# SamSweere/xmm-superres-denoise

Hardware: NVIDIA B200
Metric: RRDB SR-2x inference images/sec (F=32, nb=4, 416x416 -> 832x832, batch 64 per GPU) (higher is better)
Workload: dtype bf16

## Files before the change

### include/xmm_b200.h

```cpp
#ifndef XMM_B200_H_
#define XMM_B200_H_

#include <stddef.h>
#include <stdint.h>

#ifdef __cplusplus
extern "C" {
#endif

#define XMM_OK 0
#define XMM_ERR_INVALID_ARGUMENT 1
#define XMM_ERR_UNSUPPORTED_DEVICE 2
#define XMM_ERR_CUDA 3
#define XMM_ERR_UNSUPPORTED_SHAPE 4

const char* xmm_last_error(void);
int xmm_version(void);
int xmm_check_device(void);
int xmm_set_sm_reserve(int sms);

typedef struct {
  const float* src;
  int src_cin;
  int o_off, i_off;
  int transpose;
  int k_off, k_count;
  float scale;
  int n_off, n_count;
  int part;
} xmm_pack_segment;

typedef struct {
  void* dst;
  const float* bias;
  int nt;
  int kc;
  int nchunks;
  int nseg;
  int perm;
  int n_valid;
  int bias_n;
  xmm_pack_segment seg[5];
  int tap_order;
} xmm_pack_job;

size_t xmm_pack_blob_bytes(int nt, int kc, int nchunks);
int xmm_pack_weights(const xmm_pack_job* jobs_dev, int njobs, void* stream);

typedef struct {
  const void* in;
  int in_ctot, in_coff, cin;
  const void* wblob;
  int kc;
  int cout;
  int batch, height, width;
  float lrelu_slope;
  const void* mask; int mask_ctot, mask_coff; float mask_slope;
  float s0;
  const void* r1; int r1_ctot, r1_coff; float s1;
  const void* r2; int r2_ctot, r2_coff; float s2;
  void* out; int out_ctot, out_coff;
  int pixel_shuffle;
  int tap_mode;
  float* colsum;
  float colsum_scale;
  int shuffle_stride;
  const void* wblob_row;
} xmm_conv3x3_params;

int xmm_conv3x3_bf16(const xmm_conv3x3_params* p, void* stream);

#define XMM_CHAIN_SKIP_DEAD_STORES 0x100
size_t xmm_conv3x3_chain_workspace_bytes(int nlayers, int batch, int height);
int xmm_conv3x3_chain_bf16(const xmm_conv3x3_params* layers, int nlayers, int mode_flags, void* workspace,
                           size_t workspace_bytes, void* stream);
int xmm_last_chain_launches(void);

#define XMM_STRETCH_LINEAR 0
#define XMM_STRETCH_SQRT 1
#define XMM_STRETCH_ASINH 2
#define XMM_STRETCH_LOG 3

typedef struct {
  const void* in;
  int in_is_int32;
  const uint8_t* mask;
  size_t mask_n;
  float* out;
  size_t n;
  float pre_scale;
  float max_val;
  int stretch_mode;
  float* scratch;
} xmm_normalize_params;
int xmm_normalize(const xmm_normalize_params* p, void* stream);

int xmm_denormalize(const float* in, float* out, size_t n, size_t per_image, const float* max_vals_dev,
                    int max_n, int stretch_mode, void* stream);

int xmm_restretch(const float* in, float* out, size_t n, int from_mode, int to_mode, void* stream);

typedef struct {
  const void* src[3];
  int nsrc;
  int src_is_int32;
  const unsigned char* mask;
  int batch, h, w;
  int up;
  int res_h, res_w;
  float pre_scale;
  const float* pre_scale_dev;
  float max_val;
  int stretch_mode;
  float* out;
} xmm_prepare_counts_params;
int xmm_prepare_counts(const xmm_prepare_counts_params* p, void* stream);

int xmm_image_upsample(const float* in, float* out, int n_img, int h, int w, int scale, void* stream);

typedef struct {
  const float* in;
  const float* weight;
  const float* bias;
  int batch, cin, height, width, filters;
  void* out; int out_ctot, out_coff;
  void* out2; int out2_ctot, out2_coff;
  const float* gate;
  const void* mask; int mask_ctot, mask_coff; float mask_slope;
} xmm_conv_first_params;
int xmm_conv_first(const xmm_conv_first_params* p, void* stream);

typedef struct {
  const void* in; int in_ctot, in_coff;
  const float* weight;
  const float* bias;
  const float* residual;
  float* out;
  float* pre;
  int batch, cout, height, width, filters;
  int clamp;
  const void* wblob;
} xmm_conv_last_params;
int xmm_conv_last(const xmm_conv_last_params* p, void* stream);

typedef struct {
  int tap_begin, tap_count;
  int x_c0, x_boxes;
  int y_c0, n;
  int mode;
} xmm_wgrad_role;

typedef struct {
  float* dw;
  int o_count, i_total;
  int i_begin, i_end;
  int role;
  int lane0;
  int col0;
  float scale;
  int accumulate;
  int perm;
  int o_begin, o_total;
} xmm_wgrad_dst;

typedef struct {
  const void* x; int x_ctot;
  const void* dy; int dy_ctot;
  int batch, height, width;
  int nroles; xmm_wgrad_role roles[4];
  int ndst; xmm_wgrad_dst dst[16];
  float* workspace;
} xmm_wgrad_params;

size_t xmm_wgrad_workspace_bytes(void);
int xmm_conv3x3_wgrad(const xmm_wgrad_params* p, void* stream);

int xmm_colsum_bf16(const void* in, int ctot, int c0, int n, size_t npix, float* out, float scale,
                    int accumulate, void* stream);

typedef struct {
  int c0, n;
  float* out;
  float scale;
  int accumulate;
} xmm_colsum_segment;
int xmm_colsum_multi_bf16(const void* in, int ctot, size_t npix, const xmm_colsum_segment* segs, int nseg,
                          void* stream);

typedef struct {
  const float* s; const float* gate;
  const void* v; int v_ctot, v_coff;
  const void* v2; int v2_ctot, v2_coff;
  float* r;
  float* ssum;
  int batch, ns, height, width, channels;
} xmm_edge_wgrad_params;
int xmm_edge_wgrad(const xmm_edge_wgrad_params* p, void* stream);

typedef struct {
  float minp, maxp, mint, maxt;
  float nmaxp, nminp;
  float dr, c1, c2;
  float use_p;
  float d_dr;
  float pad;
} xmm_scale_stats;

size_t xmm_loss_workspace_floats(void);
int xmm_loss_reduce(const float* preds, const float* target, size_t n, float* sums_dev,
                    xmm_scale_stats* stats_dev, float* workspace, void* stream);
int xmm_loss_grad(const float* preds, const float* target, size_t n, const float* coef_dev,
                  const float* gl_dev, float* grad, int accumulate, void* stream);
int xmm_avgpool2_pair(const float* preds, const float* target, float* preds_out, float* target_out,
                      int nimg, int h, int w, void* stream);
int xmm_ssim_prepare(const float* preds, size_t n, xmm_scale_stats* stats_dev, float k1, float k2,
                     void* stream);

typedef struct {
  const float* preds; const float* target;
  int nimg, h, w;
  const xmm_scale_stats* stats_dev;
  float window[19];
  int use_sim;
  float* acc;
  const float* kimg;
  float* ga; float* gb; float* gc;
} xmm_ssim_stats_params;
int xmm_ssim_tiles(int h, int w);
int xmm_ssim_stats(const xmm_ssim_stats_params* p, void* stream);

typedef struct {
  const float* preds; const float* target;
  int nimg, h, w;
  const xmm_scale_stats* stats_dev;
  float window[19];
  const float* ga; const float* gb; const float* gc;
  const float* coarse;
  float* grad;
  int accumulate;
} xmm_ssim_grad_params;
int xmm_ssim_grad(const xmm_ssim_grad_params* p, void* stream);

typedef struct {
  const float* acc[5];
  int tiles[5];
  int nvalid[5];
  int nscales;
  int batch, channels;
  float betas[5];
  float k1, k2;
  xmm_scale_stats* stats_dev;
  float* value;
  float* img_val;
  float* kimg;
  const float* gl_dev;
  float weight;
} xmm_msssim_finalize_params;
int xmm_msssim_finalize(const xmm_msssim_finalize_params* p, void* stream);

int xmm_adam_step(float* params, const float* grads, float* exp_avg, float* exp_avg_sq, size_t n, float lr,
                  float beta1, float beta2, float eps, int step, float grad_scale, void* stream);

#ifdef __cplusplus
}
#endif
#endif
```

### xmm_superres_denoise_b200/csrc/conv3x3_rdb.cuh

```cuda
#pragma once
#include <cstdio>

#include "conv3x3_tc.cuh"

namespace xmm {

constexpr int kRdbP = 63;
constexpr int kRdbBoxPx = kRdbP + 2;
constexpr int kRdbTileData = 2 * kRdbBoxPx * 64;
constexpr int kRdbTileBytes = 17 * 512;
constexpr int kRdbThreads = 512;
constexpr int kRdbSlots = 5;
constexpr int kRdbSlotCols = kRdbSlots * 32;
constexpr int kRdbMaxRing = 8;
constexpr int kRdbMaxStages = 8;
constexpr int kRdbTapBytes = 32 * 64;

struct RdbLayerArgs {
  const void* wblob;
  uint32_t w_bytes;
  uint32_t smem_off;
  float lrelu_slope;
  int store;
  __nv_bfloat16* out;
  int out_ctot, out_coff;
};

struct RdbArgs {
  RdbLayerArgs layer[3];
  int cin_off;
  int batch, height, width, band_h, tiles_x;
  long long total_rows;
  int stages, ring0, ring1;
  uint32_t w_total;
  float s0, s1, s2;
  const __nv_bfloat16* r1;
  int r1_ctot, r1_coff;
  const __nv_bfloat16* r2;
  int r2_ctot, r2_coff;
  int backoff_ns;
  int prefetch_rows;
  int split_producers;
  long long* prof;
};

template <int NL>
__host__ __device__ inline int rdb_tile_origin(int t) {
  return t == 0 ? 0 : (kRdbP - (NL - 1)) + (t - 1) * (kRdbP - 2 * (NL - 1));
}
template <int NL>
__host__ __device__ inline int rdb_tiles_x(int width) {
  int n = 1;
  while ((n == 1 ? 0 : rdb_tile_origin<NL>(n - 1) - (NL - 1)) + kRdbP < width) ++n;
  return n;
}

struct RdbPiece {
  int b, x0;
  int own_lo, own_hi;
  int ra, rb;
};

template <int NL>
struct RdbSched {
  int band_h, tiles_x, width, c0, npieces;
  long long t0, t1;
  __device__ __forceinline__ void init(const RdbArgs& a) {
    band_h = a.band_h;
    tiles_x = a.tiles_x;
    width = a.width;
    t0 = a.total_rows * blockIdx.x / gridDim.x;
    t1 = a.total_rows * (blockIdx.x + 1) / gridDim.x;
    c0 = int(t0 / band_h);
    npieces = t1 > t0 ? int((t1 - 1) / band_h) - c0 + 1 : 0;
  }
  __device__ __forceinline__ RdbPiece get(int i) const {
    RdbPiece p;
    const int col = c0 + i;
    const long long base = (long long)col * band_h;
    p.ra = t0 > base ? int(t0 - base) : 0;
    p.rb = t1 < base + band_h ? int(t1 - base) : band_h;
    p.b = col / tiles_x;
    const int t = col - p.b * tiles_x;
    p.own_lo = rdb_tile_origin<NL>(t);
    p.x0 = t == 0 ? 0 : p.own_lo - (NL - 1);
    p.own_hi = t == tiles_x - 1 ? width : rdb_tile_origin<NL>(t + 1);
    return p;
  }
};

template <int NL, class F>
__device__ __forceinline__ void rdb_walk(const RdbSched<NL>& s, F&& f) {
  int piece[NL], r[NL], hi[NL], n[NL], seq[NL][NL];
  RdbPiece pc[NL];
  bool done[NL];
#pragma unroll
  for (int l = 0; l < NL; ++l) {
    piece[l] = 0;
    n[l] = 0;
    done[l] = s.npieces == 0;
#pragma unroll
    for (int m = 0; m < NL; ++m) seq[l][m] = 0;
    pc[l] = s.get(0);
    r[l] = pc[l].ra - (NL - 1 - l) - 1;
    hi[l] = pc[l].rb + (NL - 1 - l) + 2;
  }
  while (!done[NL - 1]) {
    uint32_t go = done[0] ? 0u : 1u;
    bool steady = !done[0];
    int reps = pc[0].rb + (NL - 1) - r[0] + 1;
#pragma unroll
    for (int l = 1; l < NL; ++l) {
      const bool ready = !done[l] && (done[l - 1] || piece[l - 1] > piece[l] || (piece[l - 1] == piece[l] && r[l - 1] > r[l] + 1));
      go |= ready ? (1u << l) : 0u;
      steady = steady && ready && piece[l] == piece[0];
      const int kl = pc[l].rb + (NL - 1 - l) - r[l] + 1;
      reps = kl < reps ? kl : reps;
    }
    if (!steady || reps < 1) reps = 1;
    for (int i = 0; i < reps; ++i) {
#pragma unroll
      for (int l = 0; l < NL; ++l) {
        if ((go >> l) & 1u) {
          const int e = NL - 1 - l;
          f(l, pc[l], r[l], r[l] > pc[l].rb + e, n[l], seq[l]);
          ++n[l];
          if (++r[l] > hi[l]) {
#pragma unroll
            for (int m = 0; m < NL; ++m) seq[l][m] += (pc[l].rb - pc[l].ra) + 2 * (NL - 1 - m);
            if (++piece[l] >= s.npieces) {
              done[l] = true;
            } else {
              pc[l] = s.get(piece[l]);
              r[l] = pc[l].ra - e - 1;
              hi[l] = pc[l].rb + e + 2;
            }
          }
        }
      }
    }
  }
}

__device__ __noinline__ void rdb_wait_timeout(int tag, int a, int b2, int c) {
  printf("conv3x3_rdb: CTA %d thread %d stuck in wait %d (layer/map %d, index %d, parity %d)\n", int(blockIdx.x),
         int(threadIdx.x), tag, a, b2, c);
  __trap();
}
__device__ __forceinline__ void rdb_wait(uint64_t* bar, uint32_t parity, int tag, int a, int b2) {
  uint32_t spins = 0;
  while (!ptx::mbar_try_wait(bar, parity)) {
    if (++spins > (1u << 26)) rdb_wait_timeout(tag, a, b2, int(parity));
  }
}

__device__ __forceinline__ void rdb_wait_backoff(uint64_t* bar, uint32_t parity, int tag, int a, int b2, uint32_t ns) {
  uint32_t spins = 0;
  while (!ptx::mbar_try_wait(bar, parity)) {
    if (ns) __nanosleep(ns);
    if (++spins > (1u << 24)) rdb_wait_timeout(tag, a, b2, int(parity));
  }
}
#ifndef XMM_RDB_PROFILE
#define XMM_RDB_PROFILE 0
#endif
__device__ __forceinline__ void rdb_wait_p(uint64_t* bar, uint32_t parity, int tag, int a, int b2, bool prof, long long& acc) {
  if (XMM_RDB_PROFILE && prof) {
    const long long t0 = clock64();
    rdb_wait(bar, parity, tag, a, b2);
    acc += clock64() - t0;
  } else {
    rdb_wait(bar, parity, tag, a, b2);
  }
}

__device__ __forceinline__ int rdb_phi(int row) { return (row + 30) % 3; }

__device__ __forceinline__ void tmem_st_zero32(uint32_t taddr) {
  const uint32_t z = 0;
  asm volatile(
      "tcgen05.st.sync.aligned.32x32b.x32.b32 [%0], "
      "{%1, %1, %1, %1, %1, %1, %1, %1, %1, %1, %1, %1, %1, %1, %1, %1, "
      "%1, %1, %1, %1, %1, %1, %1, %1, %1, %1, %1, %1, %1, %1, %1, %1};" ::"r"(taddr),
      "r"(z)
      : "memory");
}
__device__ __forceinline__ void tmem_st_32x32(uint32_t taddr, const uint32_t (&r)[32]) {
  asm volatile(
      "tcgen05.st.sync.aligned.32x32b.x32.b32 [%0], "
      "{%1, %2, %3, %4, %5, %6, %7, %8, %9, %10, %11, %12, %13, %14, %15, %16, "
      "%17, %18, %19, %20, %21, %22, %23, %24, %25, %26, %27, %28, %29, %30, %31, %32};" ::"r"(taddr),
      "r"(r[0]), "r"(r[1]), "r"(r[2]), "r"(r[3]), "r"(r[4]), "r"(r[5]), "r"(r[6]), "r"(r[7]), "r"(r[8]), "r"(r[9]), "r"(r[10]),
      "r"(r[11]), "r"(r[12]), "r"(r[13]), "r"(r[14]), "r"(r[15]), "r"(r[16]), "r"(r[17]), "r"(r[18]), "r"(r[19]), "r"(r[20]),
      "r"(r[21]), "r"(r[22]), "r"(r[23]), "r"(r[24]), "r"(r[25]), "r"(r[26]), "r"(r[27]), "r"(r[28]), "r"(r[29]), "r"(r[30]),
      "r"(r[31])
      : "memory");
}
__device__ __forceinline__ void st_global_256(void* p, const uint4& a, const uint4& b) {
  asm volatile("st.global.v8.b32 [%0], {%1, %2, %3, %4, %5, %6, %7, %8};" ::"l"(p), "r"(a.x), "r"(a.y), "r"(a.z), "r"(a.w),
               "r"(b.x), "r"(b.y), "r"(b.z), "r"(b.w)
               : "memory");
}
__device__ __forceinline__ void ld_global_nc_256(const void* p, uint4& a, uint4& b) {
  asm volatile("ld.global.nc.v8.b32 {%0, %1, %2, %3, %4, %5, %6, %7}, [%8];"
               : "=r"(a.x), "=r"(a.y), "=r"(a.z), "=r"(a.w), "=r"(b.x), "=r"(b.y), "=r"(b.z), "=r"(b.w)
               : "l"(p));
}
__device__ __forceinline__ void tmem_st_wait() { asm volatile("tcgen05.wait::st.sync.aligned;" ::: "memory"); }

struct RdbCtx {
  uint8_t* w_s;
  uint8_t* stage_s;
  uint8_t* map_s[2];
  uint64_t* lfull;
  uint64_t* empty;
  uint64_t* tfull;
  uint64_t* tdrain;
  uint64_t* mfull;
  uint64_t* mempty;
  uint64_t* w_bar;
  volatile int* lstage;
  uint32_t tmem_base;
};

template <int G, int NL, int L>
__device__ __forceinline__ void rdb_issuer(const RdbArgs& args, const RdbCtx& c, const RdbSched<NL>& sched) {
  constexpr int NM = NL - 1;
  constexpr int e = NL - 1 - L;
  constexpr int ring[2] = {NL == 3 ? 5 : 2, 3};
  rdb_wait(c.w_bar, 0, 7, L, 0);
  ptx::tc_fence_after();
  const uint64_t bdesc0 = ptx::umma_smem_desc(ptx::smem_u32(c.w_s), 16, 512, ptx::UMMA_SW64);
  const uint64_t adesc0 = ptx::umma_smem_desc(ptx::smem_u32(c.stage_s), 16, 512, ptx::UMMA_SW64);
  const uint32_t a_hi = uint32_t(adesc0 >> 32), b_hi = uint32_t(bdesc0 >> 32);
  const uint32_t a_lo0 = uint32_t(adesc0);
  const uint32_t b_l = uint32_t(bdesc0) + (args.layer[L].smem_off >> 4);
  const uint32_t a_map0[2] = {a_lo0 + uint32_t((c.map_s[0] - c.stage_s) >> 4), a_lo0 + uint32_t((c.map_s[1] - c.stage_s) >> 4)};
  constexpr uint32_t kTile16 = uint32_t(kRdbTileBytes) >> 4;
  constexpr uint32_t kTap16 = uint32_t(kRdbTapBytes) >> 4;
  constexpr uint32_t kIdesc = ptx::umma_idesc_bf16_f32(128, 96, 0, 0);
  auto issue6 = [&](uint32_t d, uint32_t a, uint32_t b) {
#pragma unroll
    for (int dx = 0; dx < 3; ++dx)
#pragma unroll
      for (int ks = 0; ks < 2; ++ks)
        ptx::umma_ss_lh<true>(d, a + uint32_t((dx * 64 + ks * 32) >> 4), a_hi, b + uint32_t(dx * 3) * kTap16 + uint32_t((ks * 32) >> 4),
                              b_hi, kIdesc);
  };
  const bool prof = XMM_RDB_PROFILE && args.prof != nullptr && L == 0;
  long long pw[3] = {0, 0, 0};
  const long long t_begin = XMM_RDB_PROFILE ? clock64() : 0;
  uint32_t fills = 0;
  uint32_t n = 0;
  int seq[2] = {0, 0};
  for (int pi = 0; pi < sched.npieces; ++pi) {
    const RdbPiece pc = sched.get(pi);
    const int r_last = pc.rb + e;
    for (int r = pc.ra - e - 1; r <= r_last + 2; ++r, ++n) {
      if (n > 0) rdb_wait_p(&c.tdrain[L], (n - 1u) & 1u, 2, L, int(n), prof, pw[0]);
      ptx::tc_fence_after();
      if (r <= r_last) {
        const uint32_t d = c.tmem_base + uint32_t(L * kRdbSlotCols + rdb_phi(r - 1) * 32);
        auto global_chunks = [&]() {
#pragma unroll
          for (int g = 0; g < G; ++g) {
            const int k = int(fills & 7u);
            rdb_wait_p(&c.lfull[L * 8 + k], (fills >> 3) & 1u, 3, L, k, prof, pw[1]);
            const int stage = c.lstage[L * 8 + k];
            ++fills;
            ptx::tc_fence_after();
            issue6(d, a_lo0 + uint32_t(stage) * kTile16, b_l + uint32_t(g * 9) * kTap16);
            ptx::umma_commit(&c.empty[stage]);
          }
        };
        auto map_chunks = [&]() {
#pragma unroll
          for (int m = 0; m < NM; ++m)
            if (m < L) {
              const int sq = seq[m] + (r - (pc.ra - (NL - 1 - m)));
              const int slot = sq % ring[m];
              rdb_wait_p(&c.mfull[m * 8 + slot], uint32_t(sq / ring[m]) & 1u, 4, L * 10 + m, sq, prof, pw[2]);
              ptx::tc_fence_after();
              issue6(d, a_map0[m] + uint32_t(slot) * kTile16, b_l + uint32_t((G + m) * 9) * kTap16);
              if (L == NL - 1 || r < pc.ra - e || r > pc.rb + e - 1) ptx::umma_commit(&c.mempty[m * 8 + slot]);
            }
        };
        if (NL == 2) {
          map_chunks();
          global_chunks();
        } else {
          global_chunks();
          map_chunks();
        }
      }
      ptx::umma_commit(&c.tfull[L]);
    }
#pragma unroll
    for (int m = 0; m < NM; ++m) seq[m] += (pc.rb - pc.ra) + 2 * (NL - 1 - m);
  }
  if (XMM_RDB_PROFILE && prof) {
    long long* o = args.prof + size_t(blockIdx.x) * 16;
    o[0] = clock64() - t_begin;
    o[1] = pw[0];
    o[2] = pw[1];
    o[3] = pw[2];
  }
}

template <int G, int NL, int L>
__device__ __forceinline__ void rdb_epilogue(const RdbArgs& args, const RdbCtx& c, const RdbSched<NL>& sched, int q, int lane) {
  constexpr int e = NL - 1 - L;
  constexpr int ring[2] = {NL == 3 ? 5 : 2, 3};
  constexpr bool last = L == NL - 1;
  const int pos = q * 32 + lane + 1;
  const int band = pos >= kRdbBoxPx ? 1 : 0;
  const int pl = band ? pos - (kRdbBoxPx + 1) : pos - 1;
  const bool lane_ok = band ? pl >= 0 : pl < kRdbP;
  const uint32_t lane_base = c.tmem_base + (uint32_t(q * 32) << 16) + uint32_t(L * kRdbSlotCols);
  const uint32_t pos_off = uint32_t(pos) * 64u;
  const uint32_t pos_xor = uint32_t(pos >> 1) & 3u;
  const uint32_t bias_a = ptx::smem_u32(c.w_s + args.layer[L].smem_off + args.layer[L].w_bytes);
  const float slope = args.layer[L].lrelu_slope;
  const bool has_r1 = last && args.r1 != nullptr, has_r2 = last && args.r2 != nullptr;
  const bool prof = XMM_RDB_PROFILE && args.prof != nullptr;
  long long pw[2] = {0, 0};
  long long ph[4] = {0, 0, 0, 0};
  long long tph = 0;
  const long long t_begin = XMM_RDB_PROFILE ? clock64() : 0;
  uint32_t n = 0;
  int seq = 0;
  for (int pi = 0; pi < sched.npieces; ++pi) {
    const RdbPiece pc = sched.get(pi);
    const int px = pc.x0 + pl;
    const bool px_ok = lane_ok && px < args.width;
    const bool px_own = px_ok && px >= pc.own_lo && px < pc.own_hi;
    for (int r = pc.ra - e - 1; r <= pc.rb + e + 2; ++r, ++n) {
      const int j = r - 1;
      const bool real = j >= pc.ra - e && j < pc.rb + e;
      const int y = band * args.band_h + j;
      const bool inimg = px_ok && y >= 0 && y < args.height;
      const bool owned = real && px_own && inimg && j >= pc.ra && j < pc.rb;
      const size_t pix = size_t((pc.b * args.height + (y < 0 ? 0 : y)) * args.width + (px_ok ? px : 0));
      uint4 res1[4], res2[4];
      if (has_r1 && owned) {
        const __nv_bfloat16* p = args.r1 + pix * args.r1_ctot + args.r1_coff;
        ld_global_nc_256(p, res1[0], res1[1]);
        ld_global_nc_256(p + 16, res1[2], res1[3]);
      }
      if (has_r2 && owned) {
        const __nv_bfloat16* p = args.r2 + pix * args.r2_ctot + args.r2_coff;
        ld_global_nc_256(p, res2[0], res2[1]);
        ld_global_nc_256(p + 16, res2[2], res2[3]);
      }
      if (XMM_RDB_PROFILE)
        rdb_wait_p(&c.tfull[L], n & 1u, 5, L, int(n), prof, pw[0]);
      else
        rdb_wait_backoff(&c.tfull[L], n & 1u, 5, L, int(n), uint32_t(args.backoff_ns));
      if (XMM_RDB_PROFILE) tph = clock64();
      ptx::tc_fence_after();
      const int phi = rdb_phi(j);
      const uint32_t t_main = lane_base + uint32_t(phi * 32);
      const uint32_t t_carry = lane_base + uint32_t((3 + phi) * 32);
      float v[32];
      {
        uint32_t accr[32];
        ptx::tmem_ld_32x32(t_main, accr);
        if (phi < 2) {
          uint32_t car[32];
          ptx::tmem_ld_32x32(t_carry, car);
          ptx::tmem_ld_wait();
#pragma unroll
          for (int k = 0; k < 32; ++k) v[k] = __uint_as_float(car[k]) + __uint_as_float(accr[k]);
          tmem_st_zero32(t_carry);
        } else {
          ptx::tmem_ld_wait();
#pragma unroll
          for (int k = 0; k < 32; ++k) v[k] = __uint_as_float(accr[k]);
        }
      }
      {
        uint32_t b32[32];
#pragma unroll
        for (int k = 0; k < 8; ++k)
          asm volatile("ld.shared.v4.u32 {%0, %1, %2, %3}, [%4];"
                       : "=r"(b32[4 * k]), "=r"(b32[4 * k + 1]), "=r"(b32[4 * k + 2]), "=r"(b32[4 * k + 3])
                       : "r"(bias_a + 16u * k));
        tmem_st_32x32(t_main, b32);
      }
      tmem_st_wait();
      ptx::tc_fence_before();
      __syncwarp();
      if (lane == 0) ptx::mbar_arrive(&c.tdrain[L]);
      if (XMM_RDB_PROFILE) {
        const long long t = clock64();
        ph[0] += t - tph;
        tph = t;
      }
      if (!real) continue;

      if (slope != 1.f) {
#pragma unroll
        for (int k = 0; k < 32; ++k) v[k] = fmaxf(v[k], v[k] * slope);
      }
      if (last) {
        const float s0 = args.s0;
        if (s0 != 1.f) {
#pragma unroll
          for (int k = 0; k < 32; ++k) v[k] *= s0;
        }
        if (has_r1 && owned) {
          const float s1 = args.s1;
#pragma unroll
          for (int k = 0; k < 4; ++k) {
            float m8[8];
            unpack8(res1[k], m8);
#pragma unroll
            for (int i = 0; i < 8; ++i) v[8 * k + i] = fmaf(s1, m8[i], v[8 * k + i]);
          }
        }
        if (has_r2 && owned) {
          const float s2 = args.s2;
#pragma unroll
          for (int k = 0; k < 4; ++k) {
            float m8[8];
            unpack8(res2[k], m8);
#pragma unroll
            for (int i = 0; i < 8; ++i) v[8 * k + i] = fmaf(s2, m8[i], v[8 * k + i]);
          }
        }
      }
      uint4 o[4];
#pragma unroll
      for (int k = 0; k < 4; ++k) o[k] = pack8(v + 8 * k);
      if (XMM_RDB_PROFILE) {
        const long long t = clock64();
        ph[1] += t - tph;
        tph = t;
      }
      if (args.layer[L].store && owned) {
        __nv_bfloat16* gp = args.layer[L].out + pix * args.layer[L].out_ctot + args.layer[L].out_coff;
        st_global_256(gp, o[0], o[1]);
        st_global_256(gp + 16, o[2], o[3]);
      }
      if (!last) {
        const int sq = seq + (j - (pc.ra - e));
        const int slot = sq % ring[L];
        rdb_wait_p(&c.mempty[L * 8 + slot], (uint32_t(sq / ring[L]) & 1u) ^ 1u, 6, L, sq, prof, pw[1]);
        if (XMM_RDB_PROFILE) tph = clock64();
        uint8_t* dst = c.map_s[L] + size_t(slot) * kRdbTileBytes + pos_off;
        const uint4 zero = make_uint4(0, 0, 0, 0);
#pragma unroll
        for (int k = 0; k < 4; ++k) *reinterpret_cast<uint4*>(dst + ((uint32_t(k) ^ pos_xor) << 4)) = inimg ? o[k] : zero;
        ptx::fence_proxy_async();
        __syncwarp();
        if (lane == 0) ptx::mbar_arrive(&c.mfull[L * 8 + slot]);
        if (XMM_RDB_PROFILE) {
          const long long t = clock64();
          ph[2] += t - tph;
          tph = t;
        }
      }
      if (XMM_RDB_PROFILE) {
        const long long t = clock64();
        ph[3] += t - tph;
        tph = t;
      }
    }
    seq += (pc.rb - pc.ra) + 2 * e;
  }
  if (XMM_RDB_PROFILE && prof && q == 0 && lane == 0 && L < 2) {
    long long* o = args.prof + size_t(blockIdx.x) * 16 + 4 + 4 * L;
    o[0] = clock64() - t_begin;
    o[1] = pw[0];
    o[2] = pw[1];
    o[3] = (long long)n;
    if (L == 0) {
      long long* o2 = args.prof + size_t(blockIdx.x) * 16 + 12;
      o2[0] = ph[0];
      o2[1] = ph[1];
      o2[2] = ph[2];
      o2[3] = ph[3];
    }
  }
}

template <int G, int NL, int L>
__device__ __forceinline__ void rdb_layer_producer(const CUtensorMap* tmap_in, const RdbArgs& args, const RdbCtx& c,
                                                   const RdbSched<NL>& sched, int s0, int ns) {
  constexpr int e = NL - 1 - L;
  int idx = 0;
  uint32_t phase = 0;
  uint32_t fills = 0;
  for (int pi = 0; pi < sched.npieces; ++pi) {
    const RdbPiece pc = sched.get(pi);
    for (int r = pc.ra - e - 1; r <= pc.rb + e; ++r) {
      int row = r, band0 = 0;
      if (r < 0) {
        row = r + args.band_h;
        band0 = -1;
      } else if (r >= args.band_h) {
        row = r - args.band_h;
        band0 = 1;
      }
#pragma unroll
      for (int g = 0; g < G; ++g) {
        const int stage = s0 + idx;
        rdb_wait_backoff(&c.empty[stage], phase ^ 1u, 1, L, stage, uint32_t(args.backoff_ns));
        const int k = int(fills++ & 7u);
        c.lstage[L * 8 + k] = stage;
        uint64_t* fb = &c.lfull[L * 8 + k];
        ptx::mbar_expect_tx(fb, kRdbTileData);
        ptx::tma_load_5d(c.stage_s + size_t(stage) * kRdbTileBytes, tmap_in, fb, args.cin_off + 32 * g, pc.x0 - 1, row, band0, pc.b);
        if (++idx == ns) {
          idx = 0;
          phase ^= 1u;
        }
      }
      if (L == 0 && args.prefetch_rows > 0) {
        const int rp = r + args.prefetch_rows;
        if (rp <= pc.rb + e) {
          int prow = rp, pband = 0;
          if (rp < 0) {
            prow = rp + args.band_h;
            pband = -1;
          } else if (rp >= args.band_h) {
            prow = rp - args.band_h;
            pband = 1;
          }
#pragma unroll
          for (int g = 0; g < G; ++g)
            asm volatile("cp.async.bulk.prefetch.tensor.5d.L2.global.tile [%0, {%1, %2, %3, %4, %5}];" ::"l"(
                             reinterpret_cast<uint64_t>(tmap_in)),
                         "r"(args.cin_off + 32 * g), "r"(pc.x0 - 1), "r"(prow), "r"(pband), "r"(pc.b)
                         : "memory");
        }
      }
    }
  }
}

template <int G, int NL>
__global__ void __launch_bounds__(kRdbThreads, 1)
conv3x3_rdb_kernel(const __grid_constant__ CUtensorMap tmap_in, const RdbArgs args) {
  static_assert(NL == 2 || NL == 3, "two or three fused layers");
  static_assert(NL * kRdbSlotCols <= 512, "accumulators exceed TMEM");
  constexpr int NM = NL - 1;
  extern __shared__ uint8_t smem_raw[];
  uint8_t* smem = reinterpret_cast<uint8_t*>((reinterpret_cast<uintptr_t>(smem_raw) + 1023) & ~uintptr_t(1023));
  RdbCtx c;
  c.w_s = smem;
  c.stage_s = smem + args.w_total;
  c.map_s[0] = c.stage_s + size_t(args.stages) * kRdbTileBytes;
  c.map_s[1] = c.map_s[0] + size_t(args.ring0) * kRdbTileBytes;
  uint8_t* after = c.map_s[1] + size_t(NM > 1 ? args.ring1 : 0) * kRdbTileBytes;
  uint64_t* bars = reinterpret_cast<uint64_t*>(after);
  c.lfull = bars;
  c.empty = c.lfull + 24;
  c.tfull = c.empty + 8;
  c.tdrain = c.tfull + 3;
  c.mfull = c.tdrain + 3;
  c.mempty = c.mfull + 16;
  c.w_bar = c.mempty + 16;
  c.lstage = reinterpret_cast<volatile int*>(c.w_bar + 1);
  uint32_t* tmem_ptr_s = reinterpret_cast<uint32_t*>(const_cast<int*>(c.lstage) + 24);

  const int warp = threadIdx.x >> 5;
  const int lane = threadIdx.x & 31;

  if (warp == 0 && lane == 0) {
    ptx::prefetch_tmap(&tmap_in);
    for (int s = 0; s < NL * 8; ++s) ptx::mbar_init(&c.lfull[s], 1);
    for (int s = 0; s < args.stages; ++s) ptx::mbar_init(&c.empty[s], 1);
    for (int l = 0; l < NL; ++l) {
      ptx::mbar_init(&c.tfull[l], 1);
      ptx::mbar_init(&c.tdrain[l], 4);
    }
    for (int s = 0; s < 16; ++s) {
      ptx::mbar_init(&c.mfull[s], 4);
      ptx::mbar_init(&c.mempty[s], 1);
    }
    ptx::mbar_init(c.w_bar, 1);
    ptx::fence_mbar_init();
  }
  if (warp == 1) ptx::tmem_alloc<512>(tmem_ptr_s);
  ptx::tc_fence_before();
  __syncthreads();
  ptx::tc_fence_after();
  c.tmem_base = *tmem_ptr_s;

  if (warp == 0 && ptx::elect_one()) {
    uint32_t wtot = 0;
    for (int l = 0; l < NL; ++l) wtot += args.layer[l].w_bytes + 128u;
    ptx::mbar_expect_tx(c.w_bar, wtot);
    for (int l = 0; l < NL; ++l) {
      const uint8_t* gsrc = static_cast<const uint8_t*>(args.layer[l].wblob);
      const uint32_t n_l = args.layer[l].w_bytes + 128u;
      for (uint32_t off = 0; off < n_l; off += 32768u)
        ptx::bulk_load(c.w_s + args.layer[l].smem_off + off, gsrc + off, n_l - off < 32768u ? n_l - off : 32768u, c.w_bar);
    }
  }
  const int egroup = (warp - 4) >> 2;
  if (warp >= 4) {
    uint4* z = reinterpret_cast<uint4*>(c.map_s[0]);
    const int nz = (args.ring0 + (NM > 1 ? args.ring1 : 0)) * (kRdbTileBytes / 16);
    for (int i = int(threadIdx.x) - 128; i < nz; i += kRdbThreads - 128) z[i] = make_uint4(0, 0, 0, 0);
    ptx::fence_proxy_async();
    if (egroup < NL) {
      rdb_wait(c.w_bar, 0, 9, 0, 0);
      const uint32_t lane_base = c.tmem_base + (uint32_t((warp & 3) * 32) << 16) + uint32_t(egroup * kRdbSlotCols);
      const float* bias_s = reinterpret_cast<const float*>(c.w_s + args.layer[egroup].smem_off + args.layer[egroup].w_bytes);
      uint32_t b32[32];
#pragma unroll
      for (int k = 0; k < 32; ++k) b32[k] = __float_as_uint(bias_s[k]);
      for (int sl = 0; sl < 3; ++sl) tmem_st_32x32(lane_base + uint32_t(sl * 32), b32);
      for (int sl = 3; sl < kRdbSlots; ++sl) tmem_st_zero32(lane_base + uint32_t(sl * 32));
      tmem_st_wait();
    }
  }
  ptx::tc_fence_before();
  __syncthreads();
  ptx::tc_fence_after();

  RdbSched<NL> sched;
  sched.init(args);

  if (NL == 2 && args.split_producers && (warp == 0 || warp == 3)) {
    if (ptx::elect_one()) {
      const int ns0 = (args.stages + 1) / 2;
      if (warp == 0) rdb_layer_producer<G, NL, 0>(&tmap_in, args, c, sched, 0, ns0);
      if (warp == 3) rdb_layer_producer<G, NL, 1>(&tmap_in, args, c, sched, ns0, args.stages - ns0);
    }
  } else if (warp == 0) {
    if (ptx::elect_one()) {
      int stage = 0;
      uint32_t phase = 0;
      uint32_t fills[NL];
#pragma unroll
      for (int l = 0; l < NL; ++l) fills[l] = 0;
      rdb_walk<NL>(sched, [&](int l, const RdbPiece& pc, int r, bool flush, int, const int*) {
        if (flush) return;
        int row = r, band0 = 0;
        if (r < 0) {
          row = r + args.band_h;
          band0 = -1;
        } else if (r >= args.band_h) {
          row = r - args.band_h;
          band0 = 1;
        }
#pragma unroll
        for (int g = 0; g < G; ++g) {
          rdb_wait_backoff(&c.empty[stage], phase ^ 1u, 1, l, stage, uint32_t(args.backoff_ns));
          const int k = int(fills[l]++ & 7u);
          c.lstage[l * 8 + k] = stage;
          uint64_t* fb = &c.lfull[l * 8 + k];
          ptx::mbar_expect_tx(fb, kRdbTileData);
          ptx::tma_load_5d(c.stage_s + size_t(stage) * kRdbTileBytes, &tmap_in, fb, args.cin_off + 32 * g, pc.x0 - 1, row, band0,
                           pc.b);
          if (++stage == args.stages) {
            stage = 0;
            phase ^= 1u;
          }
        }
        if (l == 0 && args.prefetch_rows > 0) {
          const int rp = r + args.prefetch_rows;
          if (rp <= pc.rb + (NL - 1)) {
            int prow = rp, pband = 0;
            if (rp < 0) {
              prow = rp + args.band_h;
              pband = -1;
            } else if (rp >= args.band_h) {
              prow = rp - args.band_h;
              pband = 1;
            }
#pragma unroll
            for (int g = 0; g < G; ++g)
              asm volatile("cp.async.bulk.prefetch.tensor.5d.L2.global.tile [%0, {%1, %2, %3, %4, %5}];" ::"l"(
                               reinterpret_cast<uint64_t>(&tmap_in)),
                           "r"(args.cin_off + 32 * g), "r"(pc.x0 - 1), "r"(prow), "r"(pband), "r"(pc.b)
                           : "memory");
          }
        }
      });
    }
  } else if (warp <= 3) {
    if (warp - 1 < NL && ptx::elect_one()) {
      if (warp == 1) rdb_issuer<G, NL, 0>(args, c, sched);
      if (warp == 2) rdb_issuer<G, NL, 1>(args, c, sched);
      if constexpr (NL == 3) {
        if (warp == 3) rdb_issuer<G, NL, 2>(args, c, sched);
      }
    }
  } else if (egroup < NL) {
    const int q = warp & 3;
    if (egroup == 0) rdb_epilogue<G, NL, 0>(args, c, sched, q, lane);
    if (egroup == 1) rdb_epilogue<G, NL, 1>(args, c, sched, q, lane);
    if constexpr (NL == 3) {
      if (egroup == 2) rdb_epilogue<G, NL, 2>(args, c, sched, q, lane);
    }
  }

  ptx::tc_fence_before();
  __syncthreads();
  if (warp == 1) {
    ptx::tc_fence_after();
    ptx::tmem_dealloc<512>(c.tmem_base);
  }
}

}
```

### xmm_superres_denoise_b200/csrc/ptx_sm100.cuh

```cuda
#pragma once
#include <cstdint>
#include <cuda.h>
#include <cuda_runtime.h>

namespace xmm {
namespace ptx {

__device__ __forceinline__ uint32_t smem_u32(const void* p) {
  return static_cast<uint32_t>(__cvta_generic_to_shared(p));
}

__device__ __forceinline__ bool elect_one() {
  uint32_t pred;
  asm volatile(
      "{\n\t"
      ".reg .pred p;\n\t"
      "elect.sync _|p, 0xffffffff;\n\t"
      "selp.u32 %0, 1, 0, p;\n\t"
      "}\n"
      : "=r"(pred));
  return pred != 0;
}

__device__ __forceinline__ void mbar_init(uint64_t* bar, uint32_t count) {
  asm volatile("mbarrier.init.shared::cta.b64 [%0], %1;" ::"r"(smem_u32(bar)), "r"(count));
}
__device__ __forceinline__ void fence_mbar_init() {
  asm volatile("fence.mbarrier_init.release.cluster;" ::: "memory");
}
__device__ __forceinline__ void fence_proxy_async() {
  asm volatile("fence.proxy.async.shared::cta;" ::: "memory");
}
__device__ __forceinline__ void mbar_expect_tx(uint64_t* bar, uint32_t bytes) {
  asm volatile("mbarrier.arrive.expect_tx.shared::cta.b64 _, [%0], %1;" ::"r"(smem_u32(bar)),
               "r"(bytes)
               : "memory");
}
__device__ __forceinline__ void mbar_arrive(uint64_t* bar) {
  asm volatile("mbarrier.arrive.shared::cta.b64 _, [%0];" ::"r"(smem_u32(bar)) : "memory");
}
__device__ __forceinline__ bool mbar_try_wait(uint64_t* bar, uint32_t parity) {
  uint32_t ok;
  asm volatile(
      "{\n\t"
      ".reg .pred p;\n\t"
      "mbarrier.try_wait.parity.shared::cta.b64 p, [%1], %2;\n\t"
      "selp.u32 %0, 1, 0, p;\n\t"
      "}\n"
      : "=r"(ok)
      : "r"(smem_u32(bar)), "r"(parity)
      : "memory");
  return ok != 0;
}
__device__ __forceinline__ void mbar_wait(uint64_t* bar, uint32_t parity) {
  while (!mbar_try_wait(bar, parity)) {
  }
}

__device__ __forceinline__ void prefetch_tmap(const CUtensorMap* m) {
  asm volatile("prefetch.tensormap [%0];" ::"l"(reinterpret_cast<uint64_t>(m)) : "memory");
}
__device__ __forceinline__ void tma_load_4d(void* smem_dst, const CUtensorMap* m, uint64_t* bar,
                                            int c0, int c1, int c2, int c3) {
  asm volatile(
      "cp.async.bulk.tensor.4d.shared::cluster.global.tile.mbarrier::complete_tx::bytes "
      "[%0], [%1, {%3, %4, %5, %6}], [%2];"
      ::"r"(smem_u32(smem_dst)),
      "l"(reinterpret_cast<uint64_t>(m)), "r"(smem_u32(bar)), "r"(c0), "r"(c1), "r"(c2), "r"(c3)
      : "memory");
}
__device__ __forceinline__ void tma_store_4d(const CUtensorMap* m, const void* smem_src, int c0, int c1, int c2, int c3) {
  asm volatile(
      "cp.async.bulk.tensor.4d.global.shared::cta.bulk_group [%0, {%2, %3, %4, %5}], [%1];"
      ::"l"(reinterpret_cast<uint64_t>(m)), "r"(smem_u32(smem_src)), "r"(c0), "r"(c1), "r"(c2), "r"(c3)
      : "memory");
}
__device__ __forceinline__ void tma_load_5d(void* smem_dst, const CUtensorMap* m, uint64_t* bar, int c0, int c1, int c2,
                                            int c3, int c4) {
  asm volatile(
      "cp.async.bulk.tensor.5d.shared::cluster.global.tile.mbarrier::complete_tx::bytes "
      "[%0], [%1, {%3, %4, %5, %6, %7}], [%2];"
      ::"r"(smem_u32(smem_dst)),
      "l"(reinterpret_cast<uint64_t>(m)), "r"(smem_u32(bar)), "r"(c0), "r"(c1), "r"(c2), "r"(c3), "r"(c4)
      : "memory");
}
__device__ __forceinline__ void tma_store_5d(const CUtensorMap* m, const void* smem_src, int c0, int c1, int c2, int c3,
                                             int c4) {
  asm volatile(
      "cp.async.bulk.tensor.5d.global.shared::cta.bulk_group [%0, {%2, %3, %4, %5, %6}], [%1];"
      ::"l"(reinterpret_cast<uint64_t>(m)), "r"(smem_u32(smem_src)), "r"(c0), "r"(c1), "r"(c2), "r"(c3), "r"(c4)
      : "memory");
}
__device__ __forceinline__ void bulk_commit() { asm volatile("cp.async.bulk.commit_group;" ::: "memory"); }
template <int N>
__device__ __forceinline__ void bulk_wait_read() { asm volatile("cp.async.bulk.wait_group.read %0;" ::"n"(N) : "memory"); }
template <int N>
__device__ __forceinline__ void bulk_wait() { asm volatile("cp.async.bulk.wait_group %0;" ::"n"(N) : "memory"); }
__device__ __forceinline__ void named_bar_sync(int id, int nthreads) {
  asm volatile("bar.sync %0, %1;" ::"r"(id), "r"(nthreads) : "memory");
}
__device__ __forceinline__ void bulk_load(void* smem_dst, const void* gsrc, uint32_t bytes,
                                          uint64_t* bar) {
  asm volatile(
      "cp.async.bulk.shared::cluster.global.mbarrier::complete_tx::bytes [%0], [%1], %2, [%3];"
      ::"r"(smem_u32(smem_dst)),
      "l"(reinterpret_cast<uint64_t>(gsrc)), "r"(bytes), "r"(smem_u32(bar))
      : "memory");
}

template <int kCols>
__device__ __forceinline__ void tmem_alloc(uint32_t* smem_result) {
  asm volatile("tcgen05.alloc.cta_group::1.sync.aligned.shared::cta.b32 [%0], %1;" ::"r"(
                   smem_u32(smem_result)),
               "n"(kCols)
               : "memory");
  asm volatile("tcgen05.relinquish_alloc_permit.cta_group::1.sync.aligned;" ::: "memory");
}
template <int kCols>
__device__ __forceinline__ void tmem_dealloc(uint32_t taddr) {
  asm volatile("tcgen05.dealloc.cta_group::1.sync.aligned.b32 %0, %1;" ::"r"(taddr), "n"(kCols)
               : "memory");
}
__device__ __forceinline__ void tc_fence_before() {
  asm volatile("tcgen05.fence::before_thread_sync;" ::: "memory");
}
__device__ __forceinline__ void tc_fence_after() {
  asm volatile("tcgen05.fence::after_thread_sync;" ::: "memory");
}
__device__ __forceinline__ void umma_ss(uint32_t tmem_d, uint64_t adesc, uint64_t bdesc,
                                        uint32_t idesc, uint32_t accumulate) {
  asm volatile(
      "{\n\t"
      ".reg .pred p;\n\t"
      "setp.ne.b32 p, %4, 0;\n\t"
      "tcgen05.mma.cta_group::1.kind::f16 [%0], %1, %2, %3, p;\n\t"
      "}\n" ::"r"(tmem_d),
      "l"(adesc), "l"(bdesc), "r"(idesc), "r"(accumulate)
      : "memory");
}
template <bool ACC>
__device__ __forceinline__ void umma_ss_lh(uint32_t tmem_d, uint32_t a_lo, uint32_t a_hi, uint32_t b_lo, uint32_t b_hi,
                                           uint32_t idesc) {
  asm volatile(
      "{\n\t"
      ".reg .pred p;\n\t"
      ".reg .b64 da, db;\n\t"
      "setp.ne.b32 p, %6, 0;\n\t"
      "mov.b64 da, {%1, %2};\n\t"
      "mov.b64 db, {%3, %4};\n\t"
      "tcgen05.mma.cta_group::1.kind::f16 [%0], da, db, %5, p;\n\t"
      "}\n" ::"r"(tmem_d),
      "r"(a_lo), "r"(a_hi), "r"(b_lo), "r"(b_hi), "r"(idesc), "n"(ACC ? 1 : 0)
      : "memory");
}
__device__ __forceinline__ void umma_ts(uint32_t tmem_d, uint32_t tmem_a, uint64_t bdesc,
                                        uint32_t idesc, uint32_t accumulate) {
  asm volatile(
      "{\n\t"
      ".reg .pred p;\n\t"
      "setp.ne.b32 p, %4, 0;\n\t"
      "tcgen05.mma.cta_group::1.kind::f16 [%0], [%1], %2, %3, p;\n\t"
      "}\n" ::"r"(tmem_d),
      "r"(tmem_a), "l"(bdesc), "r"(idesc), "r"(accumulate)
      : "memory");
}
__device__ __forceinline__ void umma_commit(uint64_t* bar) {
  asm volatile("tcgen05.commit.cta_group::1.mbarrier::arrive::one.shared::cluster.b64 [%0];" ::"r"(
                   smem_u32(bar))
               : "memory");
}
__device__ __forceinline__ void tmem_ld_32x32(uint32_t taddr, uint32_t (&r)[32]) {
  asm volatile(
      "tcgen05.ld.sync.aligned.32x32b.x32.b32 "
      "{%0, %1, %2, %3, %4, %5, %6, %7, %8, %9, %10, %11, %12, %13, %14, %15, "
      "%16, %17, %18, %19, %20, %21, %22, %23, %24, %25, %26, %27, %28, %29, %30, %31}, [%32];"
      : "=r"(r[0]), "=r"(r[1]), "=r"(r[2]), "=r"(r[3]), "=r"(r[4]), "=r"(r[5]), "=r"(r[6]),
        "=r"(r[7]), "=r"(r[8]), "=r"(r[9]), "=r"(r[10]), "=r"(r[11]), "=r"(r[12]), "=r"(r[13]),
        "=r"(r[14]), "=r"(r[15]), "=r"(r[16]), "=r"(r[17]), "=r"(r[18]), "=r"(r[19]), "=r"(r[20]),
        "=r"(r[21]), "=r"(r[22]), "=r"(r[23]), "=r"(r[24]), "=r"(r[25]), "=r"(r[26]), "=r"(r[27]),
        "=r"(r[28]), "=r"(r[29]), "=r"(r[30]), "=r"(r[31])
      : "r"(taddr)
      : "memory");
}
__device__ __forceinline__ void tmem_ld_32x16(uint32_t taddr, uint32_t (&r)[16]) {
  asm volatile(
      "tcgen05.ld.sync.aligned.32x32b.x16.b32 "
      "{%0, %1, %2, %3, %4, %5, %6, %7, %8, %9, %10, %11, %12, %13, %14, %15}, [%16];"
      : "=r"(r[0]), "=r"(r[1]), "=r"(r[2]), "=r"(r[3]), "=r"(r[4]), "=r"(r[5]), "=r"(r[6]),
        "=r"(r[7]), "=r"(r[8]), "=r"(r[9]), "=r"(r[10]), "=r"(r[11]), "=r"(r[12]), "=r"(r[13]),
        "=r"(r[14]), "=r"(r[15])
      : "r"(taddr)
      : "memory");
}
__device__ __forceinline__ void tmem_ld_32x8(uint32_t taddr, uint32_t (&r)[8]) {
  asm volatile(
      "tcgen05.ld.sync.aligned.32x32b.x8.b32 {%0, %1, %2, %3, %4, %5, %6, %7}, [%8];"
      : "=r"(r[0]), "=r"(r[1]), "=r"(r[2]), "=r"(r[3]), "=r"(r[4]), "=r"(r[5]), "=r"(r[6]), "=r"(r[7])
      : "r"(taddr)
      : "memory");
}
template <int N>
__device__ __forceinline__ void tmem_ld_cols(uint32_t taddr, uint32_t (&r)[N]);
template <>
__device__ __forceinline__ void tmem_ld_cols<8>(uint32_t taddr, uint32_t (&r)[8]) { tmem_ld_32x8(taddr, r); }
template <>
__device__ __forceinline__ void tmem_ld_cols<16>(uint32_t taddr, uint32_t (&r)[16]) { tmem_ld_32x16(taddr, r); }
__device__ __forceinline__ void tmem_ld_wait() {
  asm volatile("tcgen05.wait::ld.sync.aligned;" ::: "memory");
}

__device__ __forceinline__ uint32_t cluster_ctarank() {
  uint32_t r;
  asm volatile("mov.u32 %0, %%cluster_ctarank;" : "=r"(r));
  return r;
}
__device__ __forceinline__ void cluster_sync() {
  asm volatile("barrier.cluster.arrive.release.aligned;\n\tbarrier.cluster.wait.acquire.aligned;" ::: "memory");
}
__device__ __forceinline__ uint32_t mapa(uint32_t saddr, uint32_t rank) {
  uint32_t r;
  asm volatile("mapa.shared::cluster.u32 %0, %1, %2;" : "=r"(r) : "r"(saddr), "r"(rank));
  return r;
}
__device__ __forceinline__ void mbar_arrive_cluster(uint32_t cluster_addr) {
  asm volatile("mbarrier.arrive.relaxed.cluster.shared::cluster.b64 _, [%0];" ::"r"(cluster_addr) : "memory");
}
__device__ __forceinline__ void tma_load_4d_pair(void* smem_dst, const CUtensorMap* m, uint32_t bar_cluster_addr,
                                                 int c0, int c1, int c2, int c3) {
  asm volatile(
      "cp.async.bulk.tensor.4d.cta_group::2.shared::cluster.global.tile.mbarrier::complete_tx::bytes "
      "[%0], [%1, {%3, %4, %5, %6}], [%2];"
      ::"r"(smem_u32(smem_dst)),
      "l"(reinterpret_cast<uint64_t>(m)), "r"(bar_cluster_addr), "r"(c0), "r"(c1), "r"(c2), "r"(c3)
      : "memory");
}
template <int kCols>
__device__ __forceinline__ void tmem_alloc_pair(uint32_t* smem_result) {
  asm volatile("tcgen05.alloc.cta_group::2.sync.aligned.shared::cta.b32 [%0], %1;" ::"r"(smem_u32(smem_result)),
               "n"(kCols)
               : "memory");
  asm volatile("tcgen05.relinquish_alloc_permit.cta_group::2.sync.aligned;" ::: "memory");
}
template <int kCols>
__device__ __forceinline__ void tmem_dealloc_pair(uint32_t taddr) {
  asm volatile("tcgen05.dealloc.cta_group::2.sync.aligned.b32 %0, %1;" ::"r"(taddr), "n"(kCols) : "memory");
}
__device__ __forceinline__ void umma_ss_pair(uint32_t tmem_d, uint64_t adesc, uint64_t bdesc, uint32_t idesc,
                                             uint32_t accumulate) {
  asm volatile(
      "{\n\t"
      ".reg .pred p;\n\t"
      "setp.ne.b32 p, %4, 0;\n\t"
      "tcgen05.mma.cta_group::2.kind::f16 [%0], %1, %2, %3, p;\n\t"
      "}\n" ::"r"(tmem_d),
      "l"(adesc), "l"(bdesc), "r"(idesc), "r"(accumulate)
      : "memory");
}
__device__ __forceinline__ void umma_commit_pair(uint64_t* bar) {
  asm volatile(
      "tcgen05.commit.cta_group::2.mbarrier::arrive::one.shared::cluster.multicast::cluster.b64 [%0], %1;" ::"r"(
          smem_u32(bar)),
      "h"(uint16_t(3))
      : "memory");
}

enum : uint32_t { UMMA_SW_NONE = 0, UMMA_SW128 = 2, UMMA_SW64 = 4, UMMA_SW32 = 6 };

__device__ __forceinline__ uint64_t umma_smem_desc(uint32_t saddr, uint32_t lbo_bytes,
                                                   uint32_t sbo_bytes, uint32_t layout_type,
                                                   uint32_t base_offset = 0) {
  uint64_t d = 0;
  d |= static_cast<uint64_t>((saddr & 0x3FFFFu) >> 4);
  d |= static_cast<uint64_t>((lbo_bytes >> 4) & 0x3FFFu) << 16;
  d |= static_cast<uint64_t>((sbo_bytes >> 4) & 0x3FFFu) << 32;
  d |= 1ull << 46;
  d |= static_cast<uint64_t>(base_offset & 7u) << 49;
  d |= static_cast<uint64_t>(layout_type & 7u) << 61;
  return d;
}

__host__ __device__ constexpr uint32_t umma_idesc_bf16_f32(int m, int n, int a_mn_major,
                                                           int b_mn_major) {
  return (1u << 4) | (1u << 7) | (1u << 10) | (static_cast<uint32_t>(a_mn_major) << 15) |
         (static_cast<uint32_t>(b_mn_major) << 16) | (static_cast<uint32_t>(n >> 3) << 17) |
         (static_cast<uint32_t>(m >> 4) << 24);
}

}
}
```

### xmm_superres_denoise_b200/csrc/xmm_b200.cu

```cuda
#include "../../include/xmm_b200.h"

#include <unordered_map>
#include <vector>

#include "conv3x3_chain.cuh"
#include "conv3x3_dx.cuh"
#include "conv3x3_row.cuh"
#include "conv3x3_rdb.cuh"
#include "conv3x3_tc.cuh"
#include "edge_kernels.cuh"
#include "host_common.cuh"
#include "loss_kernels.cuh"
#include "pack_weights.cuh"
#include "wgrad_tc.cuh"

#ifndef XMM_DEFAULT_TAP_MODE
#define XMM_DEFAULT_TAP_MODE 0
#endif

using namespace xmm;

extern "C" const char* xmm_last_error(void) { return last_error_ref().c_str(); }
extern "C" int xmm_version(void) { return 100; }
extern "C" int xmm_check_device(void) {
  DeviceInfo d;
  return require_sm100(&d);
}

extern "C" size_t xmm_pack_blob_bytes(int nt, int kc, int nchunks) {
  return size_t(nchunks) * 9 * nt * kc * 2 + size_t(nt) * 4;
}

extern "C" int xmm_pack_weights(const xmm_pack_job* jobs_dev, int njobs, void* stream) {
  DeviceInfo d;
  int rc = require_sm100(&d);
  if (rc != XMM_OK) return rc;
  XMM_REQUIRE(jobs_dev != nullptr && njobs > 0, "xmm_pack_weights: empty job table");
  dim3 grid(45, njobs);
  pack_jobs_kernel<<<grid, 256, 0, static_cast<cudaStream_t>(stream)>>>(jobs_dev);
  XMM_CUDA_OK(cudaGetLastError());
  return XMM_OK;
}

namespace {

struct TmapKey {
  const void* base;
  int batch, height, width, ctot, box_c, box_w, box_h;
  bool operator==(const TmapKey& o) const {
    return base == o.base && batch == o.batch && height == o.height && width == o.width && ctot == o.ctot &&
           box_c == o.box_c && box_w == o.box_w && box_h == o.box_h;
  }
};
struct TmapKeyHash {
  size_t operator()(const TmapKey& k) const {
    size_t h = reinterpret_cast<size_t>(k.base);
    auto mix = [&h](size_t v) { h ^= v + 0x9e3779b97f4a7c15ull + (h << 6) + (h >> 2); };
    mix(k.batch); mix(k.height); mix(k.width); mix(k.ctot); mix(k.box_c); mix(k.box_w); mix(k.box_h);
    return h;
  }
};


int ensure_max_smem(const void* kernel, const DeviceInfo& dev, int reserve = 0) {
  static std::mutex mu;
  static std::unordered_map<const void*, unsigned long long> done;
  {
    std::lock_guard<std::mutex> lk(mu);
    unsigned long long& bits = done[kernel];
    if (bits & (1ull << dev.device)) return XMM_OK;
    bits |= 1ull << dev.device;
  }
  XMM_CUDA_OK(cudaFuncSetAttribute(kernel, cudaFuncAttributeMaxDynamicSharedMemorySize, dev.max_smem_optin - reserve));
  return XMM_OK;
}

int cached_tmap(CUtensorMap* out, const void* base, int batch, int height, int width, int ctot, int box_c,
                int box_w, int box_h) {
  static std::mutex mu;
  static std::unordered_map<TmapKey, CUtensorMap, TmapKeyHash> cache;
  TmapKey key{base, batch, height, width, ctot, box_c, box_w, box_h};
  std::lock_guard<std::mutex> lk(mu);
  auto it = cache.find(key);
  if (it != cache.end()) {
    *out = it->second;
    return XMM_OK;
  }
  int rc = make_nhwc_tmap(out, base, batch, height, width, ctot, box_c, box_w, box_h, false);
  if (rc != XMM_OK) return rc;
  if (cache.size() > 4096) cache.clear();
  cache.emplace(key, *out);
  return XMM_OK;
}

void fill_epilogue(ConvEpilogue& e, const xmm_conv3x3_params& p) {
  e.lrelu_slope = p.lrelu_slope;
  e.mask_slope = p.mask_slope;
  e.s0 = p.s0; e.s1 = p.s1; e.s2 = p.s2;
  e.mask = static_cast<const __nv_bfloat16*>(p.mask); e.mask_ctot = p.mask_ctot; e.mask_coff = p.mask_coff;
  e.r1 = static_cast<const __nv_bfloat16*>(p.r1); e.r1_ctot = p.r1_ctot; e.r1_coff = p.r1_coff;
  e.r2 = static_cast<const __nv_bfloat16*>(p.r2); e.r2_ctot = p.r2_ctot; e.r2_coff = p.r2_coff;
  e.out = static_cast<__nv_bfloat16*>(p.out); e.out_ctot = p.out_ctot; e.out_coff = p.out_coff;
  e.pixel_shuffle = p.pixel_shuffle;
  e.shuffle_stride = p.shuffle_stride > 0 ? p.shuffle_stride : p.cout;
  e.img_out = nullptr; e.img_res = nullptr; e.img_pre = nullptr; e.img_cout = 0; e.img_clamp = 0;
  e.colsum = p.colsum; e.colsum_scale = p.colsum_scale;
}

struct ImageOut {
  float* out;
  const float* res;
  float* pre;
  int cout, clamp;
};

constexpr bool kTcTwoGroupsDefault = true;
template <int KC, int NT, int MODE, int EG>
int launch_conv_impl(const xmm_conv3x3_params& p, const DeviceInfo& dev, cudaStream_t stream, const ImageOut* img) {
  using Cfg = ConvCfg<KC, NT, MODE, EG>;
  ConvArgs a{};
  a.wblob = p.wblob;
  a.nchunks = p.cin / KC;
  a.w_bytes = uint32_t(a.nchunks) * 9u * Cfg::kTapBytes;
  a.cin_off = p.in_coff;
  a.batch = p.batch;
  a.height = p.height;
  a.width = p.width;
  a.tiles_x = (p.width + kTileW - 1) / kTileW;
  a.tiles_y = (p.height + kTileH - 1) / kTileH;
  a.num_tiles = a.tiles_x * a.tiles_y * p.batch;
  static const int tma_env = [] { const char* e = getenv("XMM_TC_TMA_STORE"); return e ? atoi(e) : 1; }();
  const size_t fixed_plain = Cfg::smem_bytes(a.w_bytes, 0, false), fixed_out = Cfg::smem_bytes(a.w_bytes, 0, true);
  if (fixed_plain + 2 * size_t(Cfg::kStageBytes) > size_t(dev.max_smem_optin))
    return fail(XMM_ERR_UNSUPPORTED_SHAPE,
                "conv3x3: weights of cin=%d cout=%d (%u B) do not fit in shared memory next to 2 pipeline stages",
                p.cin, p.cout, a.w_bytes);
  auto stages_for = [&](size_t fixed) {
    const int st = size_t(dev.max_smem_optin) > fixed ? int((size_t(dev.max_smem_optin) - fixed) / Cfg::kStageBytes) : 0;
    return st > kMaxStages ? kMaxStages : st;
  };
  const int st_plain = stages_for(fixed_plain), st_out = stages_for(fixed_out);
  a.tma_store = (Cfg::kOutBytes > 0 && p.pixel_shuffle == 0 && img == nullptr && st_out >= 2 &&
                 (tma_env == 2 || (tma_env == 1 && (st_out >= 6 || st_out == st_plain))))
                    ? 1 : 0;
  const int stages = a.tma_store ? st_out : st_plain;
  a.stages = stages;
  const size_t smem = Cfg::smem_bytes(a.w_bytes, stages, a.tma_store != 0);

  fill_epilogue(a.epi, p);
  if (img != nullptr) {
    a.epi.img_out = img->out; a.epi.img_res = img->res; a.epi.img_pre = img->pre;
    a.epi.img_cout = img->cout; a.epi.img_clamp = img->clamp;
  }

  CUtensorMap tmap;
  int rc = cached_tmap(&tmap, p.in, p.batch, p.height, p.width, p.in_ctot, KC, Cfg::kPitchPx, kHaloH);
  if (rc != XMM_OK) return rc;
  CUtensorMap tmap_out = tmap;
  if (a.tma_store) {
    rc = cached_tmap(&tmap_out, p.out, p.batch, p.height, p.width, p.out_ctot, NT, kTileW, 4);
    if (rc != XMM_OK) return rc;
  }

  rc = ensure_max_smem(reinterpret_cast<const void*>(conv3x3_tc_kernel<KC, NT, MODE, EG>), dev);
  if (rc != XMM_OK) return rc;
  const int grid = a.num_tiles < dev.sm_count ? a.num_tiles : dev.sm_count;
  conv3x3_tc_kernel<KC, NT, MODE, EG><<<grid, Cfg::kThreads, smem, stream>>>(tmap, tmap_out, a);
  XMM_CUDA_OK(cudaGetLastError());
  return XMM_OK;
}

template <int KC, int NT, int MODE>
int launch_conv(const xmm_conv3x3_params& p, const DeviceInfo& dev, cudaStream_t stream, const ImageOut* img = nullptr) {
  static const int eg_env = [] { const char* e = getenv("XMM_TC_EG"); return e ? atoi(e) : 0; }();
  if constexpr (4 * NT <= 512) {
    const long long ntiles = (long long)((p.width + kTileW - 1) / kTileW) * ((p.height + kTileH - 1) / kTileH) * p.batch;
    if (eg_env == 2 || (eg_env == 0 && kTcTwoGroupsDefault && ntiles >= 4LL * dev.sm_count))
      return launch_conv_impl<KC, NT, MODE, 2>(p, dev, stream, img);
  }
  return launch_conv_impl<KC, NT, MODE, 1>(p, dev, stream, img);
}

template <int KC, int NT, bool G2>
int launch_conv_dx_impl(const xmm_conv3x3_params& p, const DeviceInfo& dev, cudaStream_t stream) {
  using Cfg = DxCfg<KC, NT, G2>;
  ConvArgs a{};
  a.wblob = p.wblob;
  a.nchunks = p.cin / KC;
  a.w_bytes = uint32_t(a.nchunks) * 9u * Cfg::kTapBytes;
  a.cin_off = p.in_coff;
  a.batch = p.batch;
  a.height = p.height;
  a.width = p.width;
  a.tiles_x = (p.width + kDxTileW - 1) / kDxTileW;
  a.tiles_y = (p.height + kDxTileH - 1) / kDxTileH;
  a.num_tiles = a.tiles_x * a.tiles_y * p.batch;
  static const int sides_env = [] { const char* e = getenv("XMM_DX_SIDES"); return e ? atoi(e) : 1; }();
  const void* side_ptr[3] = {p.mask, p.r1, p.r2};
  const int side_ctot[3] = {p.mask_ctot, p.r1_ctot, p.r2_ctot};
  int nside = 0;
  if (p.pixel_shuffle == 0 && sides_env)
    for (int k = 0; k < 3; ++k)
      if (side_ptr[k] != nullptr) { a.side_mask |= 1 << k; ++nside; }
  size_t fixed = Cfg::smem_bytes(a.w_bytes, 0, nside);
  if (nside > 0 && fixed + 4 * size_t(Cfg::kStageBytes) > size_t(dev.max_smem_optin)) {
    a.side_mask = 0;
    nside = 0;
    fixed = Cfg::smem_bytes(a.w_bytes, 0, 0);
  }
  if (fixed + 2 * size_t(Cfg::kStageBytes) > size_t(dev.max_smem_optin))
    return fail(XMM_ERR_UNSUPPORTED_SHAPE,
                "conv3x3: weights of cin=%d cout=%d (%u B) do not fit in shared memory next to 2 pipeline stages",
                p.cin, p.cout, a.w_bytes);
  int stages = int((size_t(dev.max_smem_optin) - fixed) / Cfg::kStageBytes);
  if (stages > kMaxStages) stages = kMaxStages;
  a.stages = stages;
  const size_t smem = Cfg::smem_bytes(a.w_bytes, stages, nside);
  fill_epilogue(a.epi, p);
  CUtensorMap tmap;
  int rc = cached_tmap(&tmap, p.in, p.batch, p.height, p.width, p.in_ctot, KC, kDxTileW, kDxPatchH);
  if (rc != XMM_OK) return rc;
  CUtensorMap tmap_out = tmap;
  if (p.pixel_shuffle == 0) {
    rc = cached_tmap(&tmap_out, p.out, p.batch, p.height, p.width, p.out_ctot, Cfg::kWarpCols, kDxTileW, 2);
    if (rc != XMM_OK) return rc;
  }
  DxSideMaps sides;
  for (int k = 0; k < 3; ++k) {
    sides.m[k] = tmap;
    if (a.side_mask & (1 << k)) {
      rc = cached_tmap(&sides.m[k], side_ptr[k], p.batch, p.height, p.width, side_ctot[k], NT, kDxTileW, kDxTileH);
      if (rc != XMM_OK) return rc;
    }
  }
  rc = ensure_max_smem(reinterpret_cast<const void*>(conv3x3_dx_kernel<KC, NT, false, G2>), dev);
  if (rc != XMM_OK) return rc;
  const int grid = a.num_tiles < dev.sm_count ? a.num_tiles : dev.sm_count;
  static const int rr_env = [] { const char* e = getenv("XMM_DX_RR"); return e ? atoi(e) : -1; }();
  const long long nstrips = (long long)a.tiles_y * p.batch;
  a.strip_rr = rr_env >= 0 ? (rr_env != 0) : (nstrips >= 4LL * grid && (a.nchunks >= 3 || nstrips >= 16LL * grid));
  static const int pair_env = [] { const char* e = getenv("XMM_DX_PAIR"); return e ? atoi(e) : 0; }();
  if constexpr (!G2)
  if (KC == 32 && NT == 32 && (pair_env || p.tap_mode == 6) && p.tap_mode != 5 && a.strip_rr && grid % 2 == 0 &&
      nstrips >= grid) {
    rc = ensure_max_smem(reinterpret_cast<const void*>(conv3x3_dx_kernel<KC, NT, true>), dev);
    if (rc != XMM_OK) return rc;
    cudaLaunchConfig_t cfg{};
    cfg.gridDim = dim3(unsigned(grid));
    cfg.blockDim = dim3(kDxThreads);
    cfg.dynamicSmemBytes = smem;
    cfg.stream = stream;
    cudaLaunchAttribute attr[1];
    attr[0].id = cudaLaunchAttributeClusterDimension;
    attr[0].val.clusterDim.x = 2;
    attr[0].val.clusterDim.y = 1;
    attr[0].val.clusterDim.z = 1;
    cfg.attrs = attr;
    cfg.numAttrs = 1;
    XMM_CUDA_OK(cudaLaunchKernelEx(&cfg, conv3x3_dx_kernel<KC, NT, true>, tmap, tmap_out, sides, a));
    return XMM_OK;
  }
  conv3x3_dx_kernel<KC, NT, false, G2><<<grid, kDxThreads, smem, stream>>>(tmap, tmap_out, sides, a);
  XMM_CUDA_OK(cudaGetLastError());
  return XMM_OK;
}

template <int KC, int NT>
int launch_conv_dx(const xmm_conv3x3_params& p, const DeviceInfo& dev, cudaStream_t stream) {
  if constexpr (NT == 32) {
    static const int g2_env = [] { const char* e = getenv("XMM_DX_G2"); return e ? atoi(e) : 1; }();
    static const int rr_env = [] { const char* e = getenv("XMM_DX_RR"); return e ? atoi(e) : -1; }();
    const int tiles_x = (p.width + kDxTileW - 1) / kDxTileW, tiles_y = (p.height + kDxTileH - 1) / kDxTileH;
    const long long ntiles = (long long)tiles_x * tiles_y * p.batch, nstrips = (long long)tiles_y * p.batch;
    const long long grid = ntiles < dev.sm_count ? ntiles : dev.sm_count;
    const int nchunks = p.cin / KC;
    const bool rr = rr_env >= 0 ? (rr_env != 0) : (nstrips >= 4LL * grid && (nchunks >= 3 || nstrips >= 16LL * grid));
    const bool g2 = (p.tap_mode == 8) || (g2_env && rr && nstrips >= 16LL * grid && (p.tap_mode <= 0 || p.tap_mode == 4));
    if (g2 && DxCfg<KC, NT, true>::smem_bytes(uint32_t(nchunks) * 9u * DxCfg<KC, NT, true>::kTapBytes,
                                               p.tap_mode == 8 ? 2 : 6,
                                               (p.mask != nullptr) + (p.r1 != nullptr) + (p.r2 != nullptr)) <=
                  size_t(dev.max_smem_optin))
      return launch_conv_dx_impl<KC, NT, true>(p, dev, stream);
  }
  return launch_conv_dx_impl<KC, NT, false>(p, dev, stream);
}


struct BandTmapKey {
  const void* base;
  int batch, height, width, ctot, band_h, nbands, box_c, box_w, box_bands;
  bool operator==(const BandTmapKey& o) const {
    return base == o.base && batch == o.batch && height == o.height && width == o.width && ctot == o.ctot &&
           band_h == o.band_h && nbands == o.nbands && box_c == o.box_c && box_w == o.box_w && box_bands == o.box_bands;
  }
};
struct BandTmapKeyHash {
  size_t operator()(const BandTmapKey& k) const {
    size_t h = reinterpret_cast<size_t>(k.base);
    auto mix = [&h](size_t v) { h ^= v + 0x9e3779b97f4a7c15ull + (h << 6) + (h >> 2); };
    mix(k.batch); mix(k.height); mix(k.width); mix(k.ctot); mix(k.band_h); mix(k.nbands); mix(k.box_c); mix(k.box_w);
    mix(k.box_bands);
    return h;
  }
};
int cached_band_tmap(CUtensorMap* out, const void* base, int batch, int height, int width, int ctot, int band_h,
                     int nbands, int box_c, int box_w, int box_bands) {
  static std::mutex mu;
  static std::unordered_map<BandTmapKey, CUtensorMap, BandTmapKeyHash> cache;
  BandTmapKey key{base, batch, height, width, ctot, band_h, nbands, box_c, box_w, box_bands};
  std::lock_guard<std::mutex> lk(mu);
  auto it = cache.find(key);
  if (it != cache.end()) {
    *out = it->second;
    return XMM_OK;
  }
  int rc = make_band_tmap(out, base, batch, height, width, ctot, band_h, nbands, box_c, box_w, box_bands);
  if (rc != XMM_OK) return rc;
  if (cache.size() > 4096) cache.clear();
  cache.emplace(key, *out);
  return XMM_OK;
}

bool row_bands(int height, int* nbands, int* band_h) {
  for (int n = kRowBands; n >= kRowBands / 2; --n)
    if (height % n == 0) {
      *nbands = n;
      *band_h = height / n;
      return true;
    }
  return false;
}

int row_epi_flags(const xmm_conv3x3_params& p) {
  return (p.lrelu_slope != 1.0f ? kRowLrelu : 0) | (p.mask ? kRowMask : 0) | (p.r1 ? kRowR1 : 0) | (p.r2 ? kRowR2 : 0) |
         (p.colsum ? kRowCsum : 0);
}
bool row_epi_built(int f) {
  switch (f) {
    case 0: case kRowLrelu: case kRowR1: case kRowR1 | kRowR2: case kRowMask: case kRowMask | kRowCsum: case kRowCsum:
    case kRowR1 | kRowCsum: case kRowR1 | kRowR2 | kRowCsum:
      return true;
    default:
      return false;
  }
}

template <int KC, int NT>
const char* row_blocker(const xmm_conv3x3_params& p, const DeviceInfo& dev, int* stages_out) {
  using Cfg = RowCfg<KC, NT>;
  if (p.wblob_row == nullptr) return "no row-hop weight image (wblob_row)";
  if (p.pixel_shuffle != 0) return "pixel shuffle";
  int nbands, band_h;
  if (!row_bands(p.height, &nbands, &band_h)) return "height has no divisor in 8..16";
  const int flags = row_epi_flags(p);
  if (!row_epi_built(flags)) return "epilogue combination not instantiated";
  if ((flags & kRowCsum) && NT != 32) return "fused column sums need cout = 32";
  const int nside = (p.mask != nullptr) + (p.r1 != nullptr) + (p.r2 != nullptr);
  const uint32_t w_bytes = uint32_t(p.cin / KC) * 9u * Cfg::kTapBytes;
  const size_t fixed = Cfg::smem_bytes(w_bytes, 0, nside);
  if (fixed + 3 * size_t(Cfg::kStageBytes) > size_t(dev.max_smem_optin)) return "weights do not fit next to 3 pipeline stages";
  int stages = int((size_t(dev.max_smem_optin) - fixed) / Cfg::kStageBytes);
  if (stages > kMaxStages) stages = kMaxStages;
  *stages_out = stages;
  return nullptr;
}

template <int KC, int NT, int EPI>
int launch_conv_row_epi(const xmm_conv3x3_params& p, const DeviceInfo& dev, cudaStream_t stream, int stages) {
  using Cfg = RowCfg<KC, NT>;
  RowArgs a{};
  a.wblob = p.wblob_row;
  a.nchunks = p.cin / KC;
  a.w_bytes = uint32_t(a.nchunks) * 9u * Cfg::kTapBytes;
  a.cin_off = p.in_coff;
  a.batch = p.batch;
  a.height = p.height;
  a.width = p.width;
  row_bands(p.height, &a.nbands, &a.band_h);
  a.tiles_x = (p.width + kRowPx - 1) / kRowPx;
  a.ncols = a.tiles_x * p.batch;
  a.stages = stages;
  const void* side_ptr[3] = {p.mask, p.r1, p.r2};
  const int side_ctot[3] = {p.mask_ctot, p.r1_ctot, p.r2_ctot};
  int nside = 0;
  for (int k = 0; k < 3; ++k)
    if (side_ptr[k] != nullptr) { a.side_mask |= 1 << k; ++nside; }
  fill_epilogue(a.epi, p);
  const long long total_rows = (long long)a.ncols * a.band_h;
  const int grid = total_rows < dev.sm_count ? int(total_rows) : dev.sm_count;
  static const int rr_env = [] { const char* e = getenv("XMM_ROW_RR"); return e ? atoi(e) : 1; }();
  a.rr_rounds = (rr_env && a.ncols >= 2 * grid) ? a.ncols / grid : 0;
  CUtensorMap tmap, tmap_out;
  int rc = cached_band_tmap(&tmap, p.in, p.batch, p.height, p.width, p.in_ctot, a.band_h, a.nbands, KC, kRowPitch, kRowBands);
  if (rc != XMM_OK) return rc;
  rc = cached_band_tmap(&tmap_out, p.out, p.batch, p.height, p.width, p.out_ctot, a.band_h, a.nbands, NT, kRowPx, 4);
  if (rc != XMM_OK) return rc;
  RowSideMaps sides;
  for (int k = 0; k < 3; ++k) {
    sides.m[k] = tmap;
    if (a.side_mask & (1 << k)) {
      rc = cached_band_tmap(&sides.m[k], side_ptr[k], p.batch, p.height, p.width, side_ctot[k], a.band_h, a.nbands, NT,
                            kRowPx, kRowBands);
      if (rc != XMM_OK) return rc;
    }
  }
  rc = ensure_max_smem(reinterpret_cast<const void*>(conv3x3_row_kernel<KC, NT, EPI>), dev);
  if (rc != XMM_OK) return rc;
  const size_t smem = Cfg::smem_bytes(a.w_bytes, stages, nside);
  conv3x3_row_kernel<KC, NT, EPI><<<grid, kRowThreads, smem, stream>>>(tmap, tmap_out, sides, a);
  XMM_CUDA_OK(cudaGetLastError());
  return XMM_OK;
}

template <int KC, int NT>
int launch_conv_row(const xmm_conv3x3_params& p, const DeviceInfo& dev, cudaStream_t stream, int stages) {
  switch (row_epi_flags(p)) {
#define XMM_ROW_CASE(F_) case (F_): return launch_conv_row_epi<KC, NT, (F_)>(p, dev, stream, stages);
    XMM_ROW_CASE(0)
    XMM_ROW_CASE(kRowLrelu)
    XMM_ROW_CASE(kRowR1)
    XMM_ROW_CASE(kRowR1 | kRowR2)
    XMM_ROW_CASE(kRowMask)
    default: break;
  }
  if constexpr (NT == 32) {
    switch (row_epi_flags(p)) {
      XMM_ROW_CASE(kRowCsum)
      XMM_ROW_CASE(kRowMask | kRowCsum)
      XMM_ROW_CASE(kRowR1 | kRowCsum)
      XMM_ROW_CASE(kRowR1 | kRowR2 | kRowCsum)
#undef XMM_ROW_CASE
      default: break;
    }
  }
  return fail(XMM_ERR_INVALID_ARGUMENT, "conv3x3 (row-hop): epilogue combination %d is not instantiated", row_epi_flags(p));
}

template <int KC, int NT>
int launch_conv_mode(const xmm_conv3x3_params& p, const DeviceInfo& dev, cudaStream_t stream) {
  const int mode = p.tap_mode <= 0 ? XMM_DEFAULT_TAP_MODE : p.tap_mode - 1;
  switch (mode) {
    case kTapHalo: return launch_conv<KC, NT, kTapHalo>(p, dev, stream);
    case kTapHaloBaseOff: return launch_conv<KC, NT, kTapHaloBaseOff>(p, dev, stream);
    case kTapDx3: return launch_conv<KC, NT, kTapDx3>(p, dev, stream);
    default: return fail(XMM_ERR_INVALID_ARGUMENT, "conv3x3: unknown tap_mode %d", mode);
  }
}

}

namespace {
int check_conv_params(const xmm_conv3x3_params& p) {
  XMM_REQUIRE(p.in && p.out && p.wblob, "conv3x3: null tensor pointer");
  XMM_REQUIRE(p.batch > 0 && p.height > 0 && p.width > 0, "conv3x3: bad shape %dx%dx%d", p.batch, p.height, p.width);
  XMM_REQUIRE(p.kc == 32 || p.kc == 64, "conv3x3: kc must be 32 or 64 (got %d)", p.kc);
  XMM_REQUIRE(p.cin > 0 && p.cin % p.kc == 0, "conv3x3: cin=%d is not a multiple of kc=%d", p.cin, p.kc);
  XMM_REQUIRE(p.in_ctot % 8 == 0 && p.in_coff % 8 == 0 && p.in_coff + p.cin <= p.in_ctot,
              "conv3x3: input channel window [%d,%d) of %d", p.in_coff, p.in_coff + p.cin, p.in_ctot);
  XMM_REQUIRE(p.shuffle_stride == 0 || (p.pixel_shuffle == 2 && p.shuffle_stride >= p.cout && p.shuffle_stride % 8 == 0),
              "conv3x3: shuffle_stride is the inverse pixel shuffle's block distance (>= cout)");
  const int out_c = p.pixel_shuffle == 1 ? p.cout / 4
                    : (p.pixel_shuffle == 2 ? 3 * (p.shuffle_stride > 0 ? p.shuffle_stride : p.cout) + p.cout : p.cout);
  XMM_REQUIRE(p.pixel_shuffle >= 0 && p.pixel_shuffle <= 2, "conv3x3: pixel_shuffle must be 0, 1 or 2");
  XMM_REQUIRE(p.pixel_shuffle != 2 || (p.height % 2 == 0 && p.width % 2 == 0 && !p.r1 && !p.r2),
              "conv3x3: inverse pixel shuffle needs even height/width and no residual");
  XMM_REQUIRE(p.out_ctot % 8 == 0 && p.out_coff % 8 == 0 && p.out_coff + out_c <= p.out_ctot,
              "conv3x3: output channel window [%d,%d) of %d", p.out_coff, p.out_coff + out_c, p.out_ctot);
  XMM_REQUIRE(!p.mask || (p.mask_ctot % 8 == 0 && p.mask_coff % 8 == 0), "conv3x3: mask window alignment");
  XMM_REQUIRE(!p.r1 || (p.r1_ctot % 8 == 0 && p.r1_coff % 8 == 0), "conv3x3: r1 window alignment");
  XMM_REQUIRE(!p.r2 || (p.r2_ctot % 8 == 0 && p.r2_coff % 8 == 0), "conv3x3: r2 window alignment");
  XMM_REQUIRE(!p.colsum || (p.cout == 32 && p.pixel_shuffle == 0), "conv3x3: fused column sums need cout = 32");
  XMM_REQUIRE(p.pixel_shuffle != 1 || (!p.mask && !p.r1 && !p.r2 && p.cout % 128 == 0),
              "conv3x3: pixel_shuffle needs cout %% 128 == 0 and no mask/residual");
  XMM_REQUIRE((reinterpret_cast<uintptr_t>(p.in) & 15) == 0 && (reinterpret_cast<uintptr_t>(p.out) & 15) == 0 &&
                  (reinterpret_cast<uintptr_t>(p.wblob) & 15) == 0,
              "conv3x3: pointers must be 16-byte aligned");
  return XMM_OK;
}
}

extern "C" int xmm_conv3x3_bf16(const xmm_conv3x3_params* pp, void* stream) {
  XMM_REQUIRE(pp != nullptr, "conv3x3: null params");
  const xmm_conv3x3_params& p = *pp;
  DeviceInfo dev;
  int rc = require_sm100(&dev);
  if (rc != XMM_OK) return rc;
  rc = check_conv_params(p);
  if (rc != XMM_OK) return rc;
  cudaStream_t s = static_cast<cudaStream_t>(stream);
  static const int row_env = [] { const char* e = getenv("XMM_ROW"); return e ? atoi(e) : 1; }();
  const bool row_narrow = p.cin <= 2 * p.kc || row_env == 2;
  if ((p.tap_mode <= 0 && row_env && row_narrow && p.wblob_row != nullptr) || p.tap_mode == 9) {
    const char* why = "cout must equal kc (32 or 64)";
    int stages = 0;
    if (p.kc == 32 && p.cout == 32) {
      why = row_blocker<32, 32>(p, dev, &stages);
      if (why == nullptr) return launch_conv_row<32, 32>(p, dev, s, stages);
    } else if (p.kc == 64 && p.cout == 64) {
      why = row_blocker<64, 64>(p, dev, &stages);
      if (why == nullptr) return launch_conv_row<64, 64>(p, dev, s, stages);
    }
    if (p.tap_mode == 9) return fail(XMM_ERR_UNSUPPORTED_SHAPE, "conv3x3: the row-hop form does not qualify (%s)", why);
  }
  const bool dx_auto = p.tap_mode <= 0 && p.kc == 32 && p.cout == 32 && p.cin >= 64 &&
                       DxCfg<32, 32>::smem_bytes(uint32_t(p.cin / 32) * 9u * DxCfg<32, 32>::kTapBytes, 4) <=
                           size_t(dev.max_smem_optin);
  if ((p.tap_mode >= 4 && p.tap_mode <= 8) || dx_auto) {
    if (p.kc == 32 && p.cout == 32) return launch_conv_dx<32, 32>(p, dev, s);
    if (p.kc == 64 && p.cout == 64) return launch_conv_dx<64, 64>(p, dev, s);
    return fail(XMM_ERR_INVALID_ARGUMENT, "conv3x3: the column-scatter form is built for cout = kc = 32 or 64");
  }
#define XMM_CONV_CASE(KC_, NT_) \
  if (p.kc == KC_ && p.cout == NT_) return launch_conv_mode<KC_, NT_>(p, dev, s);
  XMM_CONV_CASE(32, 32)
  XMM_CONV_CASE(32, 128)
  XMM_CONV_CASE(64, 64)
  XMM_CONV_CASE(64, 256)
#undef XMM_CONV_CASE
  return fail(XMM_ERR_UNSUPPORTED_SHAPE, "conv3x3: no kernel for kc=%d cout=%d", p.kc, p.cout);
}

namespace {

struct Window {
  const void* base;
  int ctot, c0, c1;
};
bool overlaps(const Window& a, const Window& b) {
  return a.base && b.base && a.base == b.base && a.ctot == b.ctot && a.c0 < b.c1 && b.c0 < a.c1;
}
bool same(const Window& a, const Window& b) { return a.base == b.base && a.ctot == b.ctot && a.c0 == b.c0 && a.c1 == b.c1; }

const char* chain_blocker(const xmm_conv3x3_params* L, int n) {
  if (n < 2 || n > kChainMaxLayers) return "2..5 layers";
  for (int l = 0; l < n; ++l) {
    const xmm_conv3x3_params& p = L[l];
    if (p.kc != 32 || p.cout != 32) return "kc = cout = 32 layers only";
    if (p.pixel_shuffle != 0) return "no pixel shuffle inside a chain";
    if (p.batch != L[0].batch || p.height != L[0].height || p.width != L[0].width) return "one image geometry";
    if (uint32_t(p.cin / 32) * 9u * DxCfg<32, 32>::kTapBytes > 160u * 1024u) return "weights must stay resident";
  }
  for (int l = 0; l < n; ++l) {
    const Window in{L[l].in, L[l].in_ctot, L[l].in_coff, L[l].in_coff + L[l].cin};
    const Window out{L[l].out, L[l].out_ctot, L[l].out_coff, L[l].out_coff + L[l].cout};
    const Window side[3] = {{L[l].mask, L[l].mask_ctot, L[l].mask_coff, L[l].mask_coff + L[l].cout},
                            {L[l].r1, L[l].r1_ctot, L[l].r1_coff, L[l].r1_coff + L[l].cout},
                            {L[l].r2, L[l].r2_ctot, L[l].r2_coff, L[l].r2_coff + L[l].cout}};
    if (overlaps(in, out)) return "a layer may not write its own input window";
    for (int m = 0; m < n; ++m) {
      const Window om{L[m].out, L[m].out_ctot, L[m].out_coff, L[m].out_coff + L[m].cout};
      if (m > l && overlaps(in, om)) return "a later layer overwrites an earlier layer's input";
      if (m != l && overlaps(out, om)) return "two layers write the same window";
      for (const Window& sd : side) {
        if (!sd.base) continue;
        if (m == l ? (overlaps(sd, om) && !same(sd, om)) : overlaps(sd, om))
          return "an epilogue input (mask / residual) is produced inside the chain";
      }
    }
  }
  return nullptr;
}

int env_int(const char* name, int dflt) {
  const char* e = getenv(name);
  return e && *e ? atoi(e) : dflt;
}

int launch_chain(const xmm_conv3x3_params* L, int n, const DeviceInfo& dev, int* done, cudaStream_t stream) {
  using Cfg = DxCfg<32, 32>;
  ChainArgs a{};
  ChainTmaps tm{};
  a.nlayers = n;
  a.batch = L[0].batch;
  a.height = L[0].height;
  a.width = L[0].width;
  a.tiles_x = (a.width + kDxTileW - 1) / kDxTileW;
  a.tiles_y = (a.height + kDxTileH - 1) / kDxTileH;
  int segs = env_int("XMM_CHAIN_SEGS", 2);
  if (segs < 1) segs = 1;
  if (segs > a.tiles_x) segs = a.tiles_x;
  a.segs = segs;
  a.done = done;
  const int nstrips = a.batch * a.tiles_y;
  const int grid = dev.sm_count;

  double cost[kChainMaxLayers], total = 0;
  for (int l = 0; l < n; ++l) {
    const int nch = L[l].cin / 32;
    cost[l] = 60.0 + 340.0 * nch;
    if (cost[l] < 850.0) cost[l] = 850.0;
    total += cost[l];
  }
  int cnt[kChainMaxLayers], used = 0;
  for (int l = 0; l < n; ++l) {
    cnt[l] = int(grid * cost[l] / total);
    if (cnt[l] < 1) cnt[l] = 1;
    used += cnt[l];
  }
  for (int l = n - 1; used < grid; l = (l + n - 1) % n) { ++cnt[l]; ++used; }
  for (int l = 0; used > grid; l = (l + 1) % n) if (cnt[l] > 1) { --cnt[l]; --used; }
  if (const char* e = getenv("XMM_CHAIN_SPLIT")) {
    int v[kChainMaxLayers], k = 0, sum = 0;
    for (const char* q = e; *q && k < n; ++k) {
      v[k] = atoi(q);
      sum += v[k];
      while (*q && *q != ',') ++q;
      if (*q == ',') ++q;
    }
    if (k == n && sum <= grid) {
      bool ok = true;
      for (int l = 0; l < n; ++l) ok = ok && v[l] >= 1;
      if (ok) for (int l = 0; l < n; ++l) cnt[l] = v[l];
    }
  }
  size_t smem = 0;
  int begin = 0;
  for (int l = 0; l < n; ++l) {
    ChainLayer& c = a.layer[l];
    c.wblob = L[l].wblob;
    c.nchunks = L[l].cin / 32;
    c.w_bytes = uint32_t(c.nchunks) * 9u * Cfg::kTapBytes;
    c.cin_off = L[l].in_coff;
    c.cta_begin = begin;
    c.cta_count = cnt[l];
    begin += cnt[l];
    const size_t fixed = Cfg::smem_bytes(c.w_bytes, 0);
    int stages = int((size_t(dev.max_smem_optin) - fixed) / Cfg::kStageBytes);
    if (stages > kMaxStages) stages = kMaxStages;
    c.stages = stages;
    const size_t need = Cfg::smem_bytes(c.w_bytes, stages);
    if (need > smem) smem = need;
    fill_epilogue(c.epi, L[l]);
    int rc = cached_tmap(&tm.m[l], L[l].in, a.batch, a.height, a.width, L[l].in_ctot, 32, kDxTileW, kDxPatchH);
    if (rc != XMM_OK) return rc;
    rc = cached_tmap(&tm.out[l], L[l].out, a.batch, a.height, a.width, L[l].out_ctot, Cfg::kWarpCols, kDxTileW, 2);
    if (rc != XMM_OK) return rc;
  }
  const int total_ctas = begin;
  XMM_CUDA_OK(cudaMemsetAsync(done, 0, size_t(n) * nstrips * sizeof(int), stream));
  {
    const int rc_attr = ensure_max_smem(reinterpret_cast<const void*>(conv3x3_chain_kernel<32, 32>), dev);
    if (rc_attr != XMM_OK) return rc_attr;
  }
  static const bool prof_on = env_int("XMM_CHAIN_PROF", 0) != 0;
  long long* prof_d = nullptr;
  if (prof_on) {
    XMM_CUDA_OK(cudaMalloc(&prof_d, size_t(total_ctas) * 4 * sizeof(long long)));
    XMM_CUDA_OK(cudaMemsetAsync(prof_d, 0, size_t(total_ctas) * 4 * sizeof(long long), stream));
    a.prof = prof_d;
  }
  void* kargs[2] = {&tm, &a};
  XMM_CUDA_OK(cudaLaunchCooperativeKernel(reinterpret_cast<const void*>(conv3x3_chain_kernel<32, 32>), dim3(total_ctas),
                                          dim3(kDxThreads), kargs, smem, stream));
  if (prof_on) {
    XMM_CUDA_OK(cudaStreamSynchronize(stream));
    std::vector<long long> h(size_t(total_ctas) * 4);
    XMM_CUDA_OK(cudaMemcpy(h.data(), prof_d, h.size() * sizeof(long long), cudaMemcpyDeviceToHost));
    cudaFree(prof_d);
    for (int l = 0; l < n; ++l) {
      double tot = 0, dep = 0, idle = 0, tiles = 0;
      for (int c = a.layer[l].cta_begin; c < a.layer[l].cta_begin + a.layer[l].cta_count; ++c) {
        tot += double(h[size_t(c) * 4]); dep += double(h[size_t(c) * 4 + 1]);
        idle += double(h[size_t(c) * 4 + 2]); tiles += double(h[size_t(c) * 4 + 3]);
      }
      const double nc = a.layer[l].cta_count;
      fprintf(stderr, "chain layer %d: %3d CTAs, nchunks %d, stages %d | per CTA: total %.0f cyc, dependency wait %.0f, "
              "epilogue idle %.0f, tiles %.1f -> %.0f cyc/tile all-in, %.0f cyc/tile busy\n", l, a.layer[l].cta_count,
              a.layer[l].nchunks, a.layer[l].stages, tot / nc, dep / nc, idle / nc, tiles / nc, tot / tiles,
              (tot - idle) / tiles);
    }
  }
  return XMM_OK;
}

}

extern "C" size_t xmm_conv3x3_chain_workspace_bytes(int nlayers, int batch, int height) {
  if (nlayers < 1 || batch < 1 || height < 1) return 0;
  return size_t(nlayers) * size_t(batch) * size_t((height + kDxTileH - 1) / kDxTileH) * sizeof(int);
}

const char* rdb_blocker(const xmm_conv3x3_params* L, int n, const DeviceInfo& dev) {
  if (n != 5) return "five layers";
  const xmm_conv3x3_params& p0 = L[0];
  if (p0.height < 8 || (p0.height & 1)) return "image height must be even (two bands) and >= 8";
  for (int k = 0; k < 5; ++k) {
    const xmm_conv3x3_params& p = L[k];
    if (p.kc != 32 || p.cout != 32) return "kc = cout = 32 layers only";
    if (p.pixel_shuffle != 0 || p.mask != nullptr || p.colsum != nullptr) return "no pixel shuffle / mask / column sums";
    if (p.wblob_row == nullptr) return "no row-hop weight image (wblob_row)";
    if (p.tap_mode > 0) return "a kernel form is forced (tap_mode)";
    if (p.batch != p0.batch || p.height != p0.height || p.width != p0.width) return "one image geometry";
    if (p.in != p0.in || p.in_ctot != p0.in_ctot || p.in_coff != p0.in_coff || p.cin != 32 * (k + 1))
      return "layer k must read channels [c0, c0 + 32 (k+1)) of one buffer";
    if (k < 4) {
      if (p.out != p0.in || p.out_ctot != p0.in_ctot || p.out_coff != p0.in_coff + 32 * (k + 1))
        return "layer k < 5 must write channels [c0 + 32 k, c0 + 32 (k+1)) of the same buffer";
      if (p.r1 != nullptr || p.r2 != nullptr || p.s0 != 1.0f) return "residuals only on the last layer";
    } else {
      if (p.out == p0.in && p.out_coff < p0.in_coff + 160 && p.out_coff + 32 > p0.in_coff)
        return "the last layer may not overwrite the block's own feature maps";
    }
  }
  if ((long long)p0.batch * p0.height * p0.width >= (1LL << 31)) return "more than 2^31 pixels";
  if (size_t(dev.max_smem_optin) < 232448) return "needs 227 KB of shared memory per CTA";
  return nullptr;
}

template <int G, int NL>
int launch_rdb(const xmm_conv3x3_params* L, const bool* store, const DeviceInfo& dev, cudaStream_t stream) {
  RdbArgs a{};
  uint32_t off = 0;
  for (int l = 0; l < NL; ++l) {
    const xmm_conv3x3_params& p = L[l];
    a.layer[l].wblob = p.wblob_row;
    a.layer[l].w_bytes = uint32_t(p.cin / 32) * 9u * uint32_t(kRdbTapBytes);
    a.layer[l].smem_off = off;
    off += (a.layer[l].w_bytes + 128u + 1023u) & ~1023u;
    a.layer[l].lrelu_slope = p.lrelu_slope;
    a.layer[l].store = store[l] ? 1 : 0;
    a.layer[l].out = static_cast<__nv_bfloat16*>(p.out);
    a.layer[l].out_ctot = p.out_ctot;
    a.layer[l].out_coff = p.out_coff;
  }
  a.w_total = off;
  const xmm_conv3x3_params& pl = L[NL - 1];
  a.cin_off = L[0].in_coff;
  a.batch = L[0].batch;
  a.height = L[0].height;
  a.width = L[0].width;
  a.band_h = a.height / 2;
  a.tiles_x = rdb_tiles_x<NL>(a.width);
  a.total_rows = (long long)a.batch * a.tiles_x * a.band_h;
  a.s0 = pl.s0; a.s1 = pl.s1; a.s2 = pl.s2;
  a.r1 = static_cast<const __nv_bfloat16*>(pl.r1); a.r1_ctot = pl.r1_ctot; a.r1_coff = pl.r1_coff;
  a.r2 = static_cast<const __nv_bfloat16*>(pl.r2); a.r2_ctot = pl.r2_ctot; a.r2_coff = pl.r2_coff;
  static const int backoff_env = env_int("XMM_RDB_BACKOFF_NS", 0);
  static const int prefetch_env = env_int("XMM_RDB_PREFETCH_ROWS", 3);
  a.backoff_ns = backoff_env;
  a.prefetch_rows = prefetch_env;
  constexpr int kBarBytes = 1024;
  const long long room = (long long)dev.max_smem_optin - 1024 - kBarBytes - (long long)a.w_total;
  int tiles = int(room / kRdbTileBytes);
  a.ring0 = NL == 3 ? 5 : 2;
  a.ring1 = NL == 3 ? 3 : 0;
  a.stages = tiles - a.ring0 - a.ring1;
  if (a.stages > kRdbMaxStages) a.stages = kRdbMaxStages;
  static const int stages_env = env_int("XMM_RDB_STAGES", 0);
  if (stages_env > 0 && stages_env < a.stages) a.stages = stages_env;
  if (a.stages < 3) return fail(XMM_ERR_UNSUPPORTED_SHAPE, "conv3x3 (fused dense block): %d pipeline stages fit", a.stages);
  static const int split_env = env_int("XMM_RDB_SPLIT_PRODUCERS", 0);
  a.split_producers = (NL == 2 && split_env && a.stages >= 4) ? 1 : 0;
  CUtensorMap tmap;
  int rc = cached_band_tmap(&tmap, L[0].in, a.batch, a.height, a.width, L[0].in_ctot, a.band_h, 2, 32, kRdbBoxPx, 2);
  if (rc != XMM_OK) return rc;
  rc = ensure_max_smem(reinterpret_cast<const void*>(conv3x3_rdb_kernel<G, NL>), dev);
  if (rc != XMM_OK) return rc;
  const size_t smem = 1024 + size_t(a.w_total) + size_t(a.stages + a.ring0 + a.ring1) * kRdbTileBytes + kBarBytes;
  static const int max_ctas = env_int("XMM_RDB_MAX_CTAS", 0);
  int grid = a.total_rows < dev.sm_count ? int(a.total_rows) : dev.sm_count;
  if (max_ctas > 0 && grid > max_ctas) grid = max_ctas;
  static const int prof_env = XMM_RDB_PROFILE ? env_int("XMM_RDB_PROF", 0) : 0;
  static long long* prof_dev = nullptr;
  if (prof_env) {
    if (prof_dev == nullptr) XMM_CUDA_OK(cudaMalloc(&prof_dev, 16 * sizeof(long long) * 1024));
    XMM_CUDA_OK(cudaMemsetAsync(prof_dev, 0, 16 * sizeof(long long) * 1024, stream));
    a.prof = prof_dev;
  }
  conv3x3_rdb_kernel<G, NL><<<grid, kRdbThreads, smem, stream>>>(tmap, a);
  XMM_CUDA_OK(cudaGetLastError());
  if (prof_env) {
    XMM_CUDA_OK(cudaStreamSynchronize(stream));
    std::vector<long long> h(size_t(grid) * 16);
    XMM_CUDA_OK(cudaMemcpy(h.data(), prof_dev, h.size() * sizeof(long long), cudaMemcpyDeviceToHost));
    static const char* names[16] = {"issuer total", "issuer wait drained", "issuer wait TMA", "issuer wait map row",
                                    "epi0 total", "epi0 wait row complete", "epi0 wait map slot", "epi0 rows",
                                    "epi1 total", "epi1 wait row complete", "epi1 wait map slot", "epi1 rows",
                                    "epi0 drain (ld+st+arrive)", "epi0 math+pack", "epi0 map write+fence+arrive", "epi0 global store"};
    fprintf(stderr, "conv3x3_rdb<%d,%d> grid %d stages %d:", G, NL, grid, a.stages);
    for (int k = 0; k < 16; ++k) {
      double sum = 0;
      for (int c = 0; c < grid; ++c) sum += double(h[size_t(c) * 16 + k]);
      fprintf(stderr, " %s %.0f;", names[k], sum / grid);
    }
    fprintf(stderr, "\n");
  }
  return XMM_OK;
}

int launch_rdb_block(const xmm_conv3x3_params* L, bool skip_dead, const DeviceInfo& dev, cudaStream_t stream) {
  const bool store_a[3] = {true, true, true};
  int rc = launch_rdb<1, 3>(L, store_a, dev, stream);
  if (rc != XMM_OK) return rc;
  const bool store_b[2] = {!skip_dead, true};
  return launch_rdb<4, 2>(L + 3, store_b, dev, stream);
}

extern "C" int xmm_set_sm_reserve(int sms) {
  if (sms < 0) sms = 0;
  return sm_reserve().exchange(sms);
}

namespace {
thread_local int g_last_chain_launches = 0;
}
extern "C" int xmm_last_chain_launches(void) { return g_last_chain_launches; }

extern "C" int xmm_conv3x3_chain_bf16(const xmm_conv3x3_params* layers, int nlayers, int mode_flags, void* workspace,
                                      size_t workspace_bytes, void* stream) {
  XMM_REQUIRE(layers != nullptr && nlayers >= 1, "conv3x3_chain: no layers");
  g_last_chain_launches = 0;
  const int mode = mode_flags & 0xff;
  const bool skip_dead = (mode_flags & XMM_CHAIN_SKIP_DEAD_STORES) != 0;
  XMM_REQUIRE(mode >= 0 && mode <= 3 && (mode_flags & ~(0xff | XMM_CHAIN_SKIP_DEAD_STORES)) == 0,
              "conv3x3_chain: mode must be 0 (auto), 1 (pipelined), 2 (layer by layer) or 3 (fused dense block)");
  DeviceInfo dev;
  int rc = require_sm100(&dev);
  if (rc != XMM_OK) return rc;
  for (int l = 0; l < nlayers; ++l) {
    rc = check_conv_params(layers[l]);
    if (rc != XMM_OK) return rc;
  }
  cudaStream_t s = static_cast<cudaStream_t>(stream);
  static const int rdb_env = env_int("XMM_RDB", 1);
  if (mode == 3 || (mode == 0 && rdb_env)) {
    const char* why_not = rdb_blocker(layers, nlayers, dev);
    if (why_not == nullptr) {
      g_last_chain_launches = 2;
      return launch_rdb_block(layers, skip_dead, dev, s);
    }
    if (mode == 3) return fail(XMM_ERR_UNSUPPORTED_SHAPE, "conv3x3_chain: cannot fuse the dense block (%s)", why_not);
  }
  const char* why = chain_blocker(layers, nlayers);
  bool pipelined = mode == 1 && why == nullptr;
  if (mode == 1 && why != nullptr) return fail(XMM_ERR_UNSUPPORTED_SHAPE, "conv3x3_chain: cannot pipeline (%s)", why);
  if (pipelined) {
    const size_t need = xmm_conv3x3_chain_workspace_bytes(nlayers, layers[0].batch, layers[0].height);
    XMM_REQUIRE(workspace != nullptr && workspace_bytes >= need && (reinterpret_cast<uintptr_t>(workspace) & 3) == 0,
                "conv3x3_chain: workspace of %zu bytes needed (got %zu)", need, workspace_bytes);
    g_last_chain_launches = 1;
    return launch_chain(layers, nlayers, dev, static_cast<int*>(workspace), s);
  }
  for (int l = 0; l < nlayers; ++l) {
    rc = xmm_conv3x3_bf16(&layers[l], stream);
    if (rc != XMM_OK) return rc;
  }
  g_last_chain_launches = nlayers;
  return XMM_OK;
}

extern "C" int xmm_normalize(const xmm_normalize_params* pp, void* stream) {
  XMM_REQUIRE(pp != nullptr, "normalize: null params");
  const xmm_normalize_params& p = *pp;
  DeviceInfo dev;
  int rc = require_sm100(&dev);
  if (rc != XMM_OK) return rc;
  if (p.n == 0) return XMM_OK;
  XMM_REQUIRE(p.in && p.out, "normalize: null tensor pointer");
  XMM_REQUIRE(p.stretch_mode >= 0 && p.stretch_mode <= 3, "normalize: Stretching function %d is not implemented",
              p.stretch_mode);
  XMM_REQUIRE((reinterpret_cast<uintptr_t>(p.in) & 15) == 0 && (reinterpret_cast<uintptr_t>(p.out) & 15) == 0,
              "normalize: pointers must be 16-byte aligned");
  XMM_REQUIRE(!p.mask || p.mask_n > 0, "normalize: mask_n must be > 0 with a mask");
  cudaStream_t s = static_cast<cudaStream_t>(stream);
  NormalizeArgs a{};
  a.in = p.in; a.mask = p.mask; a.out = p.out; a.n = p.n; a.mask_n = p.mask_n; a.in_is_int32 = p.in_is_int32;
  a.pre_scale = p.pre_scale; a.max_val = p.max_val; a.mode = p.stretch_mode; a.dyn_max = p.scratch;
  if (!(p.max_val > 0.0f)) {
    XMM_REQUIRE(p.scratch != nullptr && !p.in_is_int32 && p.mask == nullptr,
                "normalize: the max_val <= 0 branch needs fp32 input, no mask and a scratch float");
    XMM_CUDA_OK(cudaMemsetAsync(p.scratch, 0, sizeof(float), s));
    max_kernel<<<dev.sm_count * 4, 256, 0, s>>>(static_cast<const float*>(p.in), p.n, p.pre_scale, p.scratch);
    XMM_CUDA_OK(cudaGetLastError());
  }
  const size_t threads = (p.n + 3) / 4;
  normalize_kernel<<<unsigned((threads + 255) / 256), 256, 0, s>>>(a);
  XMM_CUDA_OK(cudaGetLastError());
  return XMM_OK;
}

extern "C" int xmm_denormalize(const float* in, float* out, size_t n, size_t per_image, const float* max_vals_dev,
                               int max_n, int stretch_mode, void* stream) {
  DeviceInfo dev;
  int rc = require_sm100(&dev);
  if (rc != XMM_OK) return rc;
  if (n == 0) return XMM_OK;
  XMM_REQUIRE(in && out && max_vals_dev, "denormalize: null tensor pointer");
  XMM_REQUIRE(stretch_mode >= 0 && stretch_mode <= 3, "denormalize: Stretching function %d is not implemented",
              stretch_mode);
  XMM_REQUIRE(max_n == 1 || (per_image > 0 && size_t(max_n) * per_image == n),
              "denormalize: %d max values do not match %zu elements of %zu per image", max_n, n, per_image);
  denormalize_kernel<<<unsigned((n + 255) / 256), 256, 0, static_cast<cudaStream_t>(stream)>>>(
      in, out, n, per_image ? per_image : n, max_vals_dev, max_n, stretch_mode);
  XMM_CUDA_OK(cudaGetLastError());
  return XMM_OK;
}

extern "C" int xmm_restretch(const float* in, float* out, size_t n, int from_mode, int to_mode, void* stream) {
  DeviceInfo dev;
  int rc = require_sm100(&dev);
  if (rc != XMM_OK) return rc;
  if (n == 0) return XMM_OK;
  XMM_REQUIRE(in && out, "restretch: null tensor pointer");
  XMM_REQUIRE(from_mode >= 0 && from_mode <= 3 && to_mode >= 0 && to_mode <= 3,
              "restretch: Stretching function %d -> %d is not implemented", from_mode, to_mode);
  XMM_REQUIRE((reinterpret_cast<uintptr_t>(in) & 15) == 0 && (reinterpret_cast<uintptr_t>(out) & 15) == 0,
              "restretch: pointers must be 16-byte aligned");
  const size_t threads = (n + 3) / 4;
  restretch_kernel<<<unsigned((threads + 255) / 256), 256, 0, static_cast<cudaStream_t>(stream)>>>(in, out, n, from_mode,
                                                                                                  to_mode);
  XMM_CUDA_OK(cudaGetLastError());
  return XMM_OK;
}

extern "C" int xmm_prepare_counts(const xmm_prepare_counts_params* pp, void* stream) {
  XMM_REQUIRE(pp != nullptr, "prepare_counts: null params");
  const xmm_prepare_counts_params& p = *pp;
  DeviceInfo dev;
  int rc = require_sm100(&dev);
  if (rc != XMM_OK) return rc;
  XMM_REQUIRE(p.nsrc >= 1 && p.nsrc <= 3 && p.src[0] && p.out, "prepare_counts: 1..3 source planes and an output");
  for (int k = 0; k < p.nsrc; ++k) XMM_REQUIRE(p.src[k] != nullptr, "prepare_counts: source plane %d is null", k);
  XMM_REQUIRE(p.batch > 0 && p.h > 0 && p.w > 0 && p.res_h > 0 && p.res_w > 0 && p.up >= 1,
              "prepare_counts: bad shape %dx%dx%d (x%d) -> %dx%d", p.batch, p.h, p.w, p.up, p.res_h, p.res_w);
  XMM_REQUIRE(p.max_val > 0.0f, "prepare_counts: max_val must be positive");
  XMM_REQUIRE(p.stretch_mode >= 0 && p.stretch_mode <= 3, "prepare_counts: Stretching function %d is not implemented",
              p.stretch_mode);
  PrepareCountsArgs a{};
  for (int k = 0; k < 3; ++k) a.src[k] = k < p.nsrc ? p.src[k] : nullptr;
  a.nsrc = p.nsrc; a.src_is_int32 = p.src_is_int32; a.mask = p.mask;
  a.batch = p.batch; a.h = p.h; a.w = p.w; a.up = p.up; a.res_h = p.res_h; a.res_w = p.res_w;
  a.pre_scale = p.pre_scale; a.pre_scale_dev = p.pre_scale_dev; a.max_val = p.max_val; a.mode = p.stretch_mode;
  a.out = p.out;
  const size_t n = size_t(p.batch) * p.res_h * p.res_w;
  prepare_counts_kernel<<<unsigned((n + 255) / 256), 256, 0, static_cast<cudaStream_t>(stream)>>>(a);
  XMM_CUDA_OK(cudaGetLastError());
  return XMM_OK;
}

extern "C" int xmm_image_upsample(const float* in, float* out, int n_img, int h, int w, int scale, void* stream) {
  DeviceInfo dev;
  int rc = require_sm100(&dev);
  if (rc != XMM_OK) return rc;
  XMM_REQUIRE(scale >= 1, "image_upsample: scale factor %d must be a positive integer", scale);
  const size_t n_out = size_t(n_img) * h * w * scale * scale;
  if (n_out == 0) return XMM_OK;
  XMM_REQUIRE(in && out, "image_upsample: null tensor pointer");
  image_upsample_kernel<<<unsigned((n_out + 255) / 256), 256, 0, static_cast<cudaStream_t>(stream)>>>(in, out, n_out,
                                                                                                   h, w, scale);
  XMM_CUDA_OK(cudaGetLastError());
  return XMM_OK;
}

extern "C" int xmm_conv_first(const xmm_conv_first_params* pp, void* stream) {
  XMM_REQUIRE(pp != nullptr, "conv_first: null params");
  const xmm_conv_first_params& p = *pp;
  DeviceInfo dev;
  int rc = require_sm100(&dev);
  if (rc != XMM_OK) return rc;
  XMM_REQUIRE(p.in && p.weight && p.out, "conv_first: null tensor pointer");
  XMM_REQUIRE(p.cin >= 1 && p.cin <= 4, "conv_first: in_channels=%d not in 1..4", p.cin);
  XMM_REQUIRE(p.batch > 0 && p.height > 0 && p.width > 0, "conv_first: bad shape");
  XMM_REQUIRE(p.out_ctot % 8 == 0 && p.out_coff % 8 == 0 && p.out_coff + p.filters <= p.out_ctot,
              "conv_first: output channel window");
  XMM_REQUIRE(!p.out2 || (p.out2_ctot % 8 == 0 && p.out2_coff % 8 == 0 && p.out2_coff + p.filters <= p.out2_ctot),
              "conv_first: second output channel window");
  ConvFirstArgs a{};
  a.in = p.in; a.w = p.weight; a.bias = p.bias;
  a.out = static_cast<__nv_bfloat16*>(p.out); a.out_ctot = p.out_ctot; a.out_coff = p.out_coff;
  a.out2 = static_cast<__nv_bfloat16*>(p.out2); a.out2_ctot = p.out2_ctot; a.out2_coff = p.out2_coff;
  a.batch = p.batch; a.cin = p.cin; a.height = p.height; a.width = p.width;
  a.gate = p.gate;
  a.mask = static_cast<const __nv_bfloat16*>(p.mask); a.mask_ctot = p.mask_ctot; a.mask_coff = p.mask_coff;
  a.mask_slope = p.mask_slope;
  XMM_REQUIRE(!p.mask || (p.mask_ctot % 8 == 0 && p.mask_coff % 8 == 0), "conv_first: mask window alignment");
  const size_t npix = size_t(p.batch) * p.height * p.width;
  const unsigned grid = unsigned((npix + 127) / 128);
  const size_t smem = (size_t(p.cin) * 9 + 1) * p.filters * sizeof(float);
  cudaStream_t s = static_cast<cudaStream_t>(stream);
  if (p.filters == 32) conv_first_kernel<32><<<grid, 128, smem, s>>>(a);
  else if (p.filters == 64) conv_first_kernel<64><<<grid, 128, smem, s>>>(a);
  else return fail(XMM_ERR_UNSUPPORTED_SHAPE, "conv_first: filters=%d (supported: 32, 64)", p.filters);
  XMM_CUDA_OK(cudaGetLastError());
  return XMM_OK;
}

extern "C" int xmm_conv_last(const xmm_conv_last_params* pp, void* stream) {
  XMM_REQUIRE(pp != nullptr, "conv_last: null params");
  const xmm_conv_last_params& p = *pp;
  DeviceInfo dev;
  int rc = require_sm100(&dev);
  if (rc != XMM_OK) return rc;
  XMM_REQUIRE(p.in && p.weight && p.out, "conv_last: null tensor pointer");
  XMM_REQUIRE(p.cout >= 1 && p.cout <= 4, "conv_last: out_channels=%d not in 1..4", p.cout);
  XMM_REQUIRE(p.batch > 0 && p.height > 0 && p.width > 0, "conv_last: bad shape");
  XMM_REQUIRE(p.in_ctot % 8 == 0 && p.in_coff % 8 == 0 && p.in_coff + p.filters <= p.in_ctot,
              "conv_last: input channel window");
  if (p.wblob != nullptr) {
    XMM_REQUIRE(p.filters % 32 == 0 && p.in_ctot % 8 == 0 && p.in_coff % 8 == 0 &&
                    (reinterpret_cast<uintptr_t>(p.wblob) & 15) == 0 && (reinterpret_cast<uintptr_t>(p.in) & 15) == 0,
                "conv_last: tensor-core path needs filters %% 32 == 0 and 16-byte aligned buffers");
    xmm_conv3x3_params c{};
    c.in = p.in; c.in_ctot = p.in_ctot; c.in_coff = p.in_coff; c.cin = p.filters;
    c.wblob = p.wblob; c.kc = 32; c.cout = 32;
    c.batch = p.batch; c.height = p.height; c.width = p.width;
    c.lrelu_slope = 1.0f; c.s0 = 1.0f;
    c.out = p.out; c.out_ctot = 32; c.out_coff = 0;
    ImageOut img{p.out, p.residual, p.pre, p.cout, p.clamp};
    return launch_conv<32, 32, kTapHalo>(c, dev, static_cast<cudaStream_t>(stream), &img);
  }
  ConvLastArgs a{};
  a.in = static_cast<const __nv_bfloat16*>(p.in); a.in_ctot = p.in_ctot; a.in_coff = p.in_coff;
  a.w = p.weight; a.bias = p.bias; a.residual = p.residual; a.out = p.out; a.pre = p.pre;
  a.batch = p.batch; a.cout = p.cout; a.height = p.height; a.width = p.width; a.clamp = p.clamp;
  const size_t npix = size_t(p.batch) * p.height * p.width;
  const unsigned grid = unsigned((npix + 127) / 128);
  const size_t smem = size_t(p.cout) * 9 * p.filters * sizeof(float);
  cudaStream_t s = static_cast<cudaStream_t>(stream);
  if (p.filters == 32) conv_last_kernel<32><<<grid, 128, smem, s>>>(a);
  else if (p.filters == 64) conv_last_kernel<64><<<grid, 128, smem, s>>>(a);
  else return fail(XMM_ERR_UNSUPPORTED_SHAPE, "conv_last: filters=%d (supported: 32, 64)", p.filters);
  XMM_CUDA_OK(cudaGetLastError());
  return XMM_OK;
}

extern "C" size_t xmm_wgrad_workspace_bytes(void) {
  DeviceInfo d;
  int sms = 160;
  if (device_info(&d) == XMM_OK && d.sm_count > 0) sms = d.sm_count;
  return size_t(sms) * kWgWsFloatsPerCta * sizeof(float);
}

static double wg_stacked_cost_scale() {
  static const double v = [] {
    const char* e = getenv("XMM_WG_STACKED_COST");
    return e ? atof(e) : 1.3;
  }();
  return v;
}

extern "C" int xmm_conv3x3_wgrad(const xmm_wgrad_params* pp, void* stream) {
  XMM_REQUIRE(pp != nullptr, "wgrad: null params");
  const xmm_wgrad_params& p = *pp;
  DeviceInfo dev;
  int rc = require_sm100(&dev);
  if (rc != XMM_OK) return rc;
  XMM_REQUIRE(p.x && p.dy && p.workspace, "wgrad: null tensor pointer");
  XMM_REQUIRE(p.batch > 0 && p.height > 0 && p.width > 0, "wgrad: bad shape");
  XMM_REQUIRE(p.x_ctot % 8 == 0 && p.dy_ctot % 8 == 0, "wgrad: channel counts must be multiples of 8");
  XMM_REQUIRE(p.nroles >= 1 && p.nroles <= kWgMaxRoles && p.ndst >= 1 && p.ndst <= 16, "wgrad: %d roles / %d dsts",
              p.nroles, p.ndst);
  XMM_REQUIRE(dev.sm_count >= p.nroles, "wgrad: fewer SMs than roles");
  static const int max_ctas_env = [] {
    const char* e = getenv("XMM_WG_MAX_CTAS");
    return e ? atoi(e) : 0;
  }();
  if (max_ctas_env >= p.nroles && max_ctas_env < dev.sm_count) dev.sm_count = max_ctas_env;
  WgradArgs a{};
  WgradReduceArgs ra{};
  a.nroles = ra.nroles = p.nroles;
  double cost[kWgMaxRoles], total = 0;
  size_t max_stage = 0;
  for (int r = 0; r < p.nroles; ++r) {
    const xmm_wgrad_role& q = p.roles[r];
    XMM_REQUIRE(q.tap_begin >= 0 && q.tap_count >= 1 && q.tap_begin + q.tap_count <= 9, "wgrad: role %d taps", r);
    XMM_REQUIRE(q.n >= 16 && q.n % 16 == 0 && q.n <= 192 && q.tap_count * q.n <= 512,
                "wgrad: role %d needs %d x %d TMEM columns (max 512)", r, q.tap_count, q.n);
    XMM_REQUIRE(q.mode == 0 || q.mode == 1, "wgrad: role %d mode %d", r, q.mode);
    if (q.mode == 1)
      XMM_REQUIRE(q.tap_begin == 0 && q.tap_count == 3 && q.n == 96 && q.x_c0 + 32 <= p.x_ctot && q.y_c0 < p.dy_ctot,
                  "wgrad: stacked role %d must be 3 filter rows x (3 dx x 32 X channels)", r);
    XMM_REQUIRE((q.x_boxes == 1 || q.x_boxes == 2) && q.x_c0 % 8 == 0 && q.y_c0 % 8 == 0 && q.x_c0 < p.x_ctot &&
                    (q.mode == 1 || q.y_c0 + q.n <= ((p.dy_ctot + 63) / 64) * 64 + 64),
                "wgrad: role %d channel windows", r);
    WgradRole& w = a.roles[r];
    w.tap_begin = q.tap_begin; w.tap_count = q.tap_count; w.x_c0 = q.x_c0; w.x_boxes = q.x_boxes;
    w.y_c0 = q.y_c0; w.n = q.n; w.y_boxes = (q.n + 63) / 64; w.mode = q.mode;
    static const int rows8_env = [] { const char* e = getenv("XMM_WG_ROWS8"); return e ? atoi(e) : 1; }();
    w.rows8 = (q.mode == 0 && rows8_env && q.tap_begin / 3 == (q.tap_begin + q.tap_count - 1) / 3) ? 1 : 0;
    const double per_mma = q.n / 2.0 > 47.0 ? q.n / 2.0 : 47.0;
    cost[r] = q.tap_count * per_mma * (q.mode == 1 ? wg_stacked_cost_scale() : 1.0);
    total += cost[r];
    const size_t st = q.mode == 1 ? size_t(w.x_boxes) * kWgBoxYBytes + size_t(kWgBoxX32Bytes)
                                  : size_t(w.x_boxes) * (w.rows8 ? kWgBoxX8Bytes : kWgBoxXBytes) +
                                        size_t(w.y_boxes) * kWgBoxYBytes;
    if (st > max_stage) max_stage = st;
  }
  int assigned = 0;
  for (int r = 0; r < p.nroles; ++r) {
    int c = int(dev.sm_count * cost[r] / total);
    if (c < 1) c = 1;
    a.roles[r].cta_count = c;
    assigned += c;
  }
  for (int r = 0; assigned != dev.sm_count; r = (r + 1) % p.nroles) {
    if (assigned < dev.sm_count) { ++a.roles[r].cta_count; ++assigned; }
    else if (a.roles[r].cta_count > 1) { --a.roles[r].cta_count; --assigned; }
  }
  int begin = 0;
  for (int r = 0; r < p.nroles; ++r) {
    a.roles[r].cta_begin = begin;
    begin += a.roles[r].cta_count;
    ra.roles[r] = a.roles[r];
  }
  a.batch = p.batch; a.height = p.height; a.width = p.width;
  a.tiles_x = (p.width + kTileW - 1) / kTileW;
  a.tiles_y = (p.height + kWgTileH - 1) / kWgTileH;
  a.num_tiles = a.tiles_x * a.tiles_y * p.batch;
  a.ws = p.workspace;
  int wg_stages = int((size_t(dev.max_smem_optin) - 2048) / max_stage);
  if (wg_stages > kWgMaxStages) wg_stages = kWgMaxStages;
  XMM_REQUIRE(wg_stages >= 2, "wgrad: stage of %zu B does not fit twice in shared memory", max_stage);
  a.stages = wg_stages;
  const size_t smem = 1024 + size_t(wg_stages) * max_stage;

  ra.ws = p.workspace;
  ra.ndst = p.ndst;
  for (int i = 0; i < p.ndst; ++i) {
    const xmm_wgrad_dst& q = p.dst[i];
    XMM_REQUIRE(q.dw && q.role >= 0 && q.role < p.nroles && q.i_begin >= 0 && q.i_end > q.i_begin &&
                    q.i_end <= q.i_total && q.lane0 >= 0 && q.col0 >= 0,
                "wgrad: destination %d is inconsistent with its role", i);
    if (p.roles[q.role].mode == 1)
      XMM_REQUIRE(q.lane0 + q.o_count <= 64 * p.roles[q.role].x_boxes && q.col0 + (q.i_end - q.i_begin) <= 32,
                  "wgrad: destination %d does not fit its stacked role", i);
    else
      XMM_REQUIRE(q.lane0 + (q.i_end - q.i_begin) <= 128 && q.col0 + q.o_count <= p.roles[q.role].n,
                  "wgrad: destination %d is inconsistent with its role", i);
    WgradDst& d = ra.dst[i];
    d.dw = q.dw; d.o_count = q.o_count; d.i_total = q.i_total; d.i_begin = q.i_begin; d.i_end = q.i_end;
    d.role = q.role; d.lane0 = q.lane0; d.col0 = q.col0; d.scale = q.scale; d.accumulate = q.accumulate; d.perm = q.perm;
    d.o_begin = q.o_begin; d.o_total = q.o_total > 0 ? q.o_total : q.o_count;
    XMM_REQUIRE(q.o_begin >= 0 && q.o_begin + q.o_count <= d.o_total, "wgrad: destination %d output-channel window", i);
  }

  CUtensorMap tx, ty, tx32, tx8;
  rc = cached_tmap(&tx, p.x, p.batch, p.height, p.width, p.x_ctot, 64, kTileW + 2, kWgTileH + 2);
  if (rc != XMM_OK) return rc;
  rc = cached_tmap(&tx32, p.x, p.batch, p.height, p.width, p.x_ctot, 32, kTileW + 2, kWgTileH + 2);
  if (rc != XMM_OK) return rc;
  rc = cached_tmap(&tx8, p.x, p.batch, p.height, p.width, p.x_ctot, 64, kTileW + 2, kWgTileH);
  if (rc != XMM_OK) return rc;
  rc = cached_tmap(&ty, p.dy, p.batch, p.height, p.width, p.dy_ctot, 64, kTileW, kWgTileH);
  if (rc != XMM_OK) return rc;
  rc = ensure_max_smem(reinterpret_cast<const void*>(wgrad_tc_kernel), dev, 1024);
  if (rc != XMM_OK) return rc;
  cudaStream_t s = static_cast<cudaStream_t>(stream);
  wgrad_tc_kernel<<<dev.sm_count, kWgThreads, smem, s>>>(tx, ty, tx32, tx8, a);
  XMM_CUDA_OK(cudaGetLastError());
  wgrad_reduce_kernel<<<dim3(24, p.ndst), 256, 0, s>>>(ra, a.num_tiles);
  XMM_CUDA_OK(cudaGetLastError());
  return XMM_OK;
}

extern "C" int xmm_colsum_multi_bf16(const void* in, int ctot, size_t npix, const xmm_colsum_segment* segs, int nseg,
                                     void* stream) {
  DeviceInfo dev;
  int rc = require_sm100(&dev);
  if (rc != XMM_OK) return rc;
  XMM_REQUIRE(in && segs && nseg >= 1 && nseg <= kColsumMaxSeg, "colsum: 1..%d segments", kColsumMaxSeg);
  XMM_REQUIRE(ctot % 8 == 0 && (reinterpret_cast<uintptr_t>(in) & 15) == 0, "colsum: input alignment");
  ColsumArgs a{};
  a.in = static_cast<const __nv_bfloat16*>(in);
  a.ctot = ctot;
  a.npix = npix;
  a.nseg = nseg;
  cudaStream_t s = static_cast<cudaStream_t>(stream);
  int groups = 0;
  for (int i = 0; i < nseg; ++i) {
    const xmm_colsum_segment& g = segs[i];
    XMM_REQUIRE(g.out != nullptr && g.n > 0 && g.n % 8 == 0 && g.c0 % 8 == 0 && g.c0 >= 0 && g.c0 + g.n <= ctot,
                "colsum: channel window [%d,%d) of %d", g.c0, g.c0 + g.n, ctot);
    a.seg[i].c0 = g.c0; a.seg[i].n = g.n; a.seg[i].out = g.out; a.seg[i].scale = g.scale;
    a.seg[i].group0 = groups;
    groups += g.n / 8;
    if (!g.accumulate) XMM_CUDA_OK(cudaMemsetAsync(g.out, 0, size_t(g.n) * sizeof(float), s));
  }
  XMM_REQUIRE(groups <= kColsumThreads, "colsum: %d channels in one call (max %d)", groups * 8, kColsumThreads * 8);
  a.ngroups = groups;
  if (npix == 0) return XMM_OK;
  const int ppb = kColsumThreads / groups;
  size_t want = (npix + size_t(ppb) * 8 - 1) / (size_t(ppb) * 8);
  const size_t cap = size_t(dev.sm_count) * 8;
  const unsigned grid = unsigned(want < 1 ? 1 : (want > cap ? cap : want));
  colsum_multi_kernel<<<grid, kColsumThreads, 0, s>>>(a);
  XMM_CUDA_OK(cudaGetLastError());
  return XMM_OK;
}

extern "C" int xmm_colsum_bf16(const void* in, int ctot, int c0, int n, size_t npix, float* out, float scale,
                               int accumulate, void* stream) {
  xmm_colsum_segment g{c0, n, out, scale, accumulate};
  return xmm_colsum_multi_bf16(in, ctot, npix, &g, 1, stream);
}

extern "C" int xmm_edge_wgrad(const xmm_edge_wgrad_params* pp, void* stream) {
  XMM_REQUIRE(pp != nullptr, "edge_wgrad: null params");
  const xmm_edge_wgrad_params& p = *pp;
  DeviceInfo dev;
  int rc = require_sm100(&dev);
  if (rc != XMM_OK) return rc;
  XMM_REQUIRE(p.s && p.v && p.r, "edge_wgrad: null tensor pointer");
  XMM_REQUIRE(p.ns >= 1 && p.ns <= 4 && p.batch > 0 && p.height > 0 && p.width > 0, "edge_wgrad: bad shape");
  EdgeWgradArgs a{};
  a.s = p.s; a.gate = p.gate;
  a.v = static_cast<const __nv_bfloat16*>(p.v); a.v_ctot = p.v_ctot; a.v_coff = p.v_coff;
  a.v2 = static_cast<const __nv_bfloat16*>(p.v2); a.v2_ctot = p.v2_ctot; a.v2_coff = p.v2_coff;
  a.r = p.r; a.ssum = p.ssum; a.batch = p.batch; a.ns = p.ns; a.height = p.height; a.width = p.width;
  XMM_REQUIRE(p.v_ctot % 8 == 0 && p.v_coff % 8 == 0 && (!p.v2 || (p.v2_ctot % 8 == 0 && p.v2_coff % 8 == 0)),
              "edge_wgrad: channel windows must be 8-channel aligned");
  XMM_REQUIRE(p.channels == 32 || p.channels == 64, "edge_wgrad: channels=%d (supported: 32, 64)", p.channels);
  const size_t red_bytes = size_t(kEdgeWgradThreads / 32) * p.channels * 9 * sizeof(float);
  int rows = int((40 * 1024) / (size_t(p.width + 2) * sizeof(float))) - 2;
  if (rows > 8) rows = 8;
  if (rows > p.height) rows = p.height;
  XMM_REQUIRE(rows >= 1, "edge_wgrad: image width %d too large for the shared-memory row staging", p.width);
  a.rows = rows;
  const size_t smem = size_t(rows + 2) * (p.width + 2) * sizeof(float) + red_bytes;
  const dim3 grid(unsigned((p.height + rows - 1) / rows), unsigned(p.batch));
  cudaStream_t s = static_cast<cudaStream_t>(stream);
  if (p.channels == 32) {
    static bool attr32 = false;
    if (!attr32) {
      XMM_CUDA_OK(cudaFuncSetAttribute(edge_wgrad_kernel<32>, cudaFuncAttributeMaxDynamicSharedMemorySize, 96 * 1024));
      attr32 = true;
    }
    edge_wgrad_kernel<32><<<grid, kEdgeWgradThreads, smem, s>>>(a);
  } else {
    static bool attr64 = false;
    if (!attr64) {
      XMM_CUDA_OK(cudaFuncSetAttribute(edge_wgrad_kernel<64>, cudaFuncAttributeMaxDynamicSharedMemorySize, 96 * 1024));
      attr64 = true;
    }
    edge_wgrad_kernel<64><<<grid, kEdgeWgradThreads, smem, s>>>(a);
  }
  XMM_CUDA_OK(cudaGetLastError());
  return XMM_OK;
}

static_assert(sizeof(xmm_scale_stats) == sizeof(ScaleStats), "xmm_scale_stats mirrors ScaleStats");
static const int kLossBlocks = 592;

extern "C" size_t xmm_loss_workspace_floats(void) { return size_t(kLossBlocks) * 8; }

extern "C" int xmm_loss_reduce(const float* preds, const float* target, size_t n, float* sums_dev,
                               xmm_scale_stats* stats_dev, float* workspace, void* stream) {
  DeviceInfo dev;
  int rc = require_sm100(&dev);
  if (rc != XMM_OK) return rc;
  XMM_REQUIRE(preds && target && workspace && n > 0, "loss_reduce: null pointer or empty input");
  XMM_REQUIRE((reinterpret_cast<uintptr_t>(preds) & 15) == 0 && (reinterpret_cast<uintptr_t>(target) & 15) == 0,
              "loss_reduce: pointers must be 16-byte aligned");
  cudaStream_t s = static_cast<cudaStream_t>(stream);
  size_t need = (n + 1023) / 1024;
  const int blocks = int(need < size_t(kLossBlocks) ? need : size_t(kLossBlocks));
  loss_reduce_kernel<<<blocks, 256, 0, s>>>(preds, target, n, workspace);
  XMM_CUDA_OK(cudaGetLastError());
  loss_reduce_finalize_kernel<<<1, 32, 0, s>>>(workspace, blocks, sums_dev, reinterpret_cast<ScaleStats*>(stats_dev));
  XMM_CUDA_OK(cudaGetLastError());
  return XMM_OK;
}

extern "C" int xmm_loss_grad(const float* preds, const float* target, size_t n, const float* coef_dev,
                             const float* gl_dev, float* grad, int accumulate, void* stream) {
  DeviceInfo dev;
  int rc = require_sm100(&dev);
  if (rc != XMM_OK) return rc;
  XMM_REQUIRE(preds && target && coef_dev && grad, "loss_grad: null pointer");
  if (n == 0) return XMM_OK;
  loss_grad_kernel<<<unsigned((n + 255) / 256), 256, 0, static_cast<cudaStream_t>(stream)>>>(preds, target, n, coef_dev,
                                                                                            gl_dev, grad, accumulate);
  XMM_CUDA_OK(cudaGetLastError());
  return XMM_OK;
}

extern "C" int xmm_avgpool2_pair(const float* preds, const float* target, float* preds_out, float* target_out,
                                 int nimg, int h, int w, void* stream) {
  DeviceInfo dev;
  int rc = require_sm100(&dev);
  if (rc != XMM_OK) return rc;
  XMM_REQUIRE(preds && target && preds_out && target_out, "avgpool2: null pointer");
  const size_t n = size_t(nimg) * (h / 2) * (w / 2);
  if (n == 0) return XMM_OK;
  avgpool2_pair_kernel<<<unsigned((n + 255) / 256), 256, 0, static_cast<cudaStream_t>(stream)>>>(
      preds, target, preds_out, target_out, nimg, h, w);
  XMM_CUDA_OK(cudaGetLastError());
  return XMM_OK;
}

extern "C" int xmm_ssim_prepare(const float* preds, size_t n, xmm_scale_stats* stats_dev, float k1, float k2,
                                void* stream) {
  DeviceInfo dev;
  int rc = require_sm100(&dev);
  if (rc != XMM_OK) return rc;
  XMM_REQUIRE(preds && stats_dev && n > 0, "ssim_prepare: null pointer or empty input");
  cudaStream_t s = static_cast<cudaStream_t>(stream);
  ssim_constants_kernel<<<1, 32, 0, s>>>(reinterpret_cast<ScaleStats*>(stats_dev), k1, k2);
  XMM_CUDA_OK(cudaGetLastError());
  size_t need = (n + 255) / 256;
  const int blocks = int(need < size_t(kLossBlocks) ? need : size_t(kLossBlocks));
  count_ties_kernel<<<blocks, 256, 0, s>>>(preds, n, reinterpret_cast<ScaleStats*>(stats_dev));
  XMM_CUDA_OK(cudaGetLastError());
  return XMM_OK;
}

extern "C" int xmm_ssim_tiles(int h, int w) {
  const int vh = h - 2 * kSsimPad, vw = w - 2 * kSsimPad;
  if (vh <= 0 || vw <= 0) return 0;
  return ((vh + kSsimTileH - 1) / kSsimTileH) * ((vw + kSsimTileW - 1) / kSsimTileW);
}

extern "C" int xmm_ssim_stats(const xmm_ssim_stats_params* pp, void* stream) {
  XMM_REQUIRE(pp != nullptr, "ssim_stats: null params");
  const xmm_ssim_stats_params& p = *pp;
  DeviceInfo dev;
  int rc = require_sm100(&dev);
  if (rc != XMM_OK) return rc;
  XMM_REQUIRE(p.preds && p.target && p.stats_dev, "ssim_stats: null pointer");
  XMM_REQUIRE(p.h > 2 * kSsimPad && p.w > 2 * kSsimPad && p.nimg > 0 && p.nimg <= 65535,
              "ssim_stats: image %dx%d is not larger than the %d-tap Gaussian window", p.h, p.w, kSsimTaps);
  XMM_REQUIRE((p.kimg == nullptr) == (p.acc != nullptr), "ssim_stats: give acc (forward) or kimg+ga/gb/gc (backward)");
  XMM_REQUIRE(p.kimg == nullptr || (p.ga && p.gb && p.gc), "ssim_stats: backward needs ga, gb, gc");
  SsimArgs a{};
  a.p = p.preds; a.t = p.target; a.nimg = p.nimg; a.h = p.h; a.w = p.w;
  a.st = reinterpret_cast<const ScaleStats*>(p.stats_dev);
  for (int i = 0; i < kSsimTaps; ++i) a.win.w[i] = p.window[i];
  a.acc = p.acc; a.use_sim = p.use_sim; a.kimg = p.kimg; a.ga = p.ga; a.gb = p.gb; a.gc = p.gc;
  const int vh = p.h - 2 * kSsimPad, vw = p.w - 2 * kSsimPad;
  dim3 grid((vw + kSsimTileW - 1) / kSsimTileW, (vh + kSsimTileH - 1) / kSsimTileH, p.nimg);
  ssim_stats_kernel<<<grid, 256, 0, static_cast<cudaStream_t>(stream)>>>(a);
  XMM_CUDA_OK(cudaGetLastError());
  return XMM_OK;
}

extern "C" int xmm_ssim_grad(const xmm_ssim_grad_params* pp, void* stream) {
  XMM_REQUIRE(pp != nullptr, "ssim_grad: null params");
  const xmm_ssim_grad_params& p = *pp;
  DeviceInfo dev;
  int rc = require_sm100(&dev);
  if (rc != XMM_OK) return rc;
  XMM_REQUIRE(p.preds && p.target && p.stats_dev && p.ga && p.gb && p.gc && p.grad, "ssim_grad: null pointer");
  XMM_REQUIRE(p.h > 2 * kSsimPad && p.w > 2 * kSsimPad && p.nimg > 0 && p.nimg <= 65535, "ssim_grad: bad shape");
  SsimGradArgs a{};
  a.p = p.preds; a.t = p.target; a.nimg = p.nimg; a.h = p.h; a.w = p.w;
  a.st = reinterpret_cast<const ScaleStats*>(p.stats_dev);
  for (int i = 0; i < kSsimTaps; ++i) a.win.w[i] = p.window[i];
  a.ga = p.ga; a.gb = p.gb; a.gc = p.gc; a.coarse = p.coarse; a.grad = p.grad; a.accumulate = p.accumulate;
  dim3 grid((p.w + kSsimTileW - 1) / kSsimTileW, (p.h + kSsimTileH - 1) / kSsimTileH, p.nimg);
  ssim_grad_kernel<<<grid, 256, 0, static_cast<cudaStream_t>(stream)>>>(a);
  XMM_CUDA_OK(cudaGetLastError());
  return XMM_OK;
}

extern "C" int xmm_msssim_finalize(const xmm_msssim_finalize_params* pp, void* stream) {
  XMM_REQUIRE(pp != nullptr, "msssim_finalize: null params");
  const xmm_msssim_finalize_params& p = *pp;
  DeviceInfo dev;
  int rc = require_sm100(&dev);
  if (rc != XMM_OK) return rc;
  XMM_REQUIRE(p.nscales >= 1 && p.nscales <= kMaxScales && p.batch >= 1 && p.batch <= 1024 && p.channels >= 1,
              "msssim_finalize: %d scales, batch %d", p.nscales, p.batch);
  XMM_REQUIRE(p.stats_dev && p.value && p.img_val && p.kimg, "msssim_finalize: null pointer");
  MsFinalizeArgs a{};
  for (int s = 0; s < p.nscales; ++s) {
    XMM_REQUIRE(p.acc[s] && p.tiles[s] > 0 && p.nvalid[s] > 0, "msssim_finalize: scale %d is empty", s);
    a.acc[s] = p.acc[s]; a.tiles[s] = p.tiles[s]; a.nvalid[s] = p.nvalid[s]; a.betas[s] = p.betas[s];
  }
  a.nscales = p.nscales; a.batch = p.batch; a.channels = p.channels; a.k1 = p.k1; a.k2 = p.k2;
  a.st = reinterpret_cast<ScaleStats*>(p.stats_dev);
  a.value = p.value; a.img_val = p.img_val; a.kimg = p.kimg; a.gl = p.gl_dev; a.weight = p.weight;
  const size_t fin_smem = size_t(3) * p.nscales * p.batch * p.channels * sizeof(float);
  XMM_REQUIRE(fin_smem <= 40 * 1024, "msssim_finalize: batch*channels=%d too large for the single-block reduction",
              p.batch * p.channels);
  msssim_finalize_kernel<<<1, 256, fin_smem, static_cast<cudaStream_t>(stream)>>>(a);
  XMM_CUDA_OK(cudaGetLastError());
  return XMM_OK;
}

extern "C" int xmm_adam_step(float* params, const float* grads, float* exp_avg, float* exp_avg_sq, size_t n, float lr,
                             float beta1, float beta2, float eps, int step, float grad_scale, void* stream) {
  DeviceInfo dev;
  int rc = require_sm100(&dev);
  if (rc != XMM_OK) return rc;
  XMM_REQUIRE(params && grads && exp_avg && exp_avg_sq, "adam: null pointer");
  XMM_REQUIRE(step >= 1, "adam: step count starts at 1 (got %d)", step);
  if (n == 0) return XMM_OK;
  const double bc1 = 1.0 - pow(double(beta1), double(step));
  const double bc2 = 1.0 - pow(double(beta2), double(step));
  adam_kernel<<<unsigned((n + 255) / 256), 256, 0, static_cast<cudaStream_t>(stream)>>>(
      params, grads, exp_avg, exp_avg_sq, n, lr, beta1, beta2, eps, float(bc1), float(sqrt(bc2)), grad_scale);
  XMM_CUDA_OK(cudaGetLastError());
  return XMM_OK;
}
```

### xmm_superres_denoise_b200/ops.py

```python
from __future__ import annotations

import ctypes
import os
from typing import Optional

import torch

from . import _lib
from ._lib import (Conv3x3Params, ConvFirstParams, ConvLastParams, EdgeWgradParams, NormalizeParams, WgradDst,
                   WgradParams, WgradRole)


LAST_CHAIN_LAUNCHES = 0
LAUNCHES = 0


def _count(n: int = 1) -> None:
    global LAUNCHES
    LAUNCHES += n


def _ptr(t: Optional[torch.Tensor]) -> Optional[int]:
    return None if t is None else t.data_ptr()


def _nhwc(t: torch.Tensor, name: str) -> None:
    _lib.require_cuda_tensor(t, torch.bfloat16, name)
    if t.dim() != 4:
        raise RuntimeError(f"{name}: expected [B,H,W,C], got {tuple(t.shape)}")


def _conv3x3_params(p: Conv3x3Params, inp: torch.Tensor, in_coff: int, cin: int, wblob_ptr: int, kc: int, cout: int,
                    out: torch.Tensor, out_coff: int, *, lrelu: float = 1.0, s0: float = 1.0,
                    r1: Optional[torch.Tensor] = None, r1_coff: int = 0, s1: float = 0.0,
                    r2: Optional[torch.Tensor] = None, r2_coff: int = 0, s2: float = 0.0,
                    mask: Optional[torch.Tensor] = None, mask_coff: int = 0, mask_slope: float = 1.0,
                    pixel_shuffle: int = 0, tap_mode: int = 0, colsum: Optional[torch.Tensor] = None,
                    colsum_scale: float = 1.0, shuffle_stride: int = 0, wblob_row: Optional[int] = None) -> None:
    _nhwc(inp, "conv3x3 input")
    _nhwc(out, "conv3x3 output")
    b, h, w, ctot = inp.shape
    p.in_, p.in_ctot, p.in_coff, p.cin = inp.data_ptr(), ctot, in_coff, cin
    p.wblob, p.kc, p.cout = wblob_ptr, kc, cout
    p.wblob_row = wblob_row
    p.batch, p.height, p.width = b, h, w
    p.lrelu_slope = lrelu
    if mask is not None:
        _nhwc(mask, "conv3x3 mask")
        p.mask, p.mask_ctot, p.mask_coff = mask.data_ptr(), mask.shape[3], mask_coff
    p.mask_slope = mask_slope
    p.s0 = s0
    if r1 is not None:
        _nhwc(r1, "conv3x3 r1")
        p.r1, p.r1_ctot, p.r1_coff = r1.data_ptr(), r1.shape[3], r1_coff
    p.s1 = s1
    if r2 is not None:
        _nhwc(r2, "conv3x3 r2")
        p.r2, p.r2_ctot, p.r2_coff = r2.data_ptr(), r2.shape[3], r2_coff
    p.s2 = s2
    pixel_shuffle = int(pixel_shuffle)
    exp = {0: (b, h, w), 1: (b, 2 * h, 2 * w), 2: (b, h // 2, w // 2)}[pixel_shuffle]
    if tuple(out.shape[:3]) != exp:
        raise RuntimeError(f"conv3x3 output: expected spatial shape {exp}, got {tuple(out.shape[:3])}")
    p.out, p.out_ctot, p.out_coff = out.data_ptr(), out.shape[3], out_coff
    p.pixel_shuffle = pixel_shuffle
    p.shuffle_stride = shuffle_stride
    p.tap_mode = tap_mode
    if colsum is not None:
        _lib.require_cuda_tensor(colsum, torch.float32, "conv3x3 colsum")
        if colsum.numel() != cout:
            raise RuntimeError("conv3x3 colsum: one float per output channel")
        p.colsum, p.colsum_scale = colsum.data_ptr(), colsum_scale


def conv3x3(inp: torch.Tensor, in_coff: int, cin: int, wblob_ptr: int, kc: int, cout: int,
            out: torch.Tensor, out_coff: int, **kw) -> None:
    if _TORCH_OPS and not (kw.keys() - _TORCH_FWD_KEYS):
        from . import torch_ops

        torch_ops.load().conv3x3_fwd(inp, in_coff, cin, wblob_ptr, kc, cout, out, out_coff, kw.get("lrelu", 1.0),
                                     kw.get("s0", 1.0), kw.get("r1"), kw.get("r1_coff", 0), kw.get("s1", 0.0),
                                     kw.get("r2"), kw.get("r2_coff", 0), kw.get("s2", 0.0), kw.get("wblob_row") or 0,
                                     kw.get("tap_mode", 0))
        _count()
        return
    p = Conv3x3Params()
    _conv3x3_params(p, inp, in_coff, cin, wblob_ptr, kc, cout, out, out_coff, **kw)
    _lib.check(_lib.load().xmm_conv3x3_bf16(ctypes.byref(p), _lib.stream_ptr()))
    _count()


_TORCH_OPS = os.environ.get("XMM_TORCH_OPS", "0") == "1"
_TORCH_FWD_KEYS = {"lrelu", "s0", "r1", "r1_coff", "s1", "r2", "r2_coff", "s2", "wblob_row", "tap_mode"}


CHAIN_AUTO, CHAIN_PIPELINED, CHAIN_LAYER_BY_LAYER, CHAIN_FUSED = 0, 1, 2, 3
CHAIN_SKIP_DEAD_STORES = 0x100
_chain_ws: dict = {}
_chain_ws_retired: list = []


def conv3x3_chain(layers, mode: int = CHAIN_AUTO) -> None:
    n = len(layers)
    arr = (Conv3x3Params * n)()
    for p, (a, kw) in zip(arr, layers):
        _conv3x3_params(p, *a, **kw)
    lib = _lib.load()
    dev = layers[0][0][0].device
    need = int(lib.xmm_conv3x3_chain_workspace_bytes(n, arr[0].batch, arr[0].height))
    ws = _chain_ws.get(dev)
    if ws is None or ws.numel() < need:
        if ws is not None:
            _chain_ws_retired.append(ws)
        ws = torch.empty(max(need, 1 << 16), dtype=torch.uint8, device=dev)
        _chain_ws[dev] = ws
    _lib.check(lib.xmm_conv3x3_chain_bf16(arr, n, int(mode), ws.data_ptr(), ws.numel(), _lib.stream_ptr()))
    global LAST_CHAIN_LAUNCHES
    LAST_CHAIN_LAUNCHES = int(lib.xmm_last_chain_launches())
    _count(LAST_CHAIN_LAUNCHES)


def conv_first(x: torch.Tensor, weight: torch.Tensor, bias: Optional[torch.Tensor], out: torch.Tensor,
               out_coff: int, out2: Optional[torch.Tensor] = None, out2_coff: int = 0, *,
               gate: Optional[torch.Tensor] = None, mask: Optional[torch.Tensor] = None, mask_coff: int = 0,
               mask_slope: float = 1.0) -> None:
    _lib.require_cuda_tensor(x, torch.float32, "conv_first input")
    _lib.require_cuda_tensor(weight, torch.float32, "conv_first weight")
    _nhwc(out, "conv_first output")
    b, cin, h, w = x.shape
    p = ConvFirstParams()
    p.in_, p.weight, p.bias = x.data_ptr(), weight.data_ptr(), _ptr(bias)
    p.batch, p.cin, p.height, p.width, p.filters = b, cin, h, w, weight.shape[0]
    p.out, p.out_ctot, p.out_coff = out.data_ptr(), out.shape[3], out_coff
    if out2 is not None:
        _nhwc(out2, "conv_first output2")
        p.out2, p.out2_ctot, p.out2_coff = out2.data_ptr(), out2.shape[3], out2_coff
    if gate is not None:
        _lib.require_cuda_tensor(gate, torch.float32, "conv_first gate")
        if gate.shape != x.shape:
            raise RuntimeError("conv_first gate: shape must equal the input shape")
        p.gate = gate.data_ptr()
    if mask is not None:
        _nhwc(mask, "conv_first mask")
        p.mask, p.mask_ctot, p.mask_coff = mask.data_ptr(), mask.shape[3], mask_coff
    p.mask_slope = mask_slope
    _lib.check(_lib.load().xmm_conv_first(ctypes.byref(p), _lib.stream_ptr()))
    _count()


def conv_last(inp: torch.Tensor, in_coff: int, weight: torch.Tensor, bias: Optional[torch.Tensor],
              out: torch.Tensor, residual: Optional[torch.Tensor] = None, pre: Optional[torch.Tensor] = None,
              clamp: bool = True, wblob_ptr: Optional[int] = None) -> None:
    _nhwc(inp, "conv_last input")
    _lib.require_cuda_tensor(weight, torch.float32, "conv_last weight")
    _lib.require_cuda_tensor(out, torch.float32, "conv_last output")
    b, h, w, ctot = inp.shape
    p = ConvLastParams()
    p.in_, p.in_ctot, p.in_coff = inp.data_ptr(), ctot, in_coff
    p.weight, p.bias = weight.data_ptr(), _ptr(bias)
    if residual is not None:
        _lib.require_cuda_tensor(residual, torch.float32, "conv_last residual")
        if residual.shape != out.shape:
            raise RuntimeError("conv_last residual: shape must equal the output shape")
        p.residual = residual.data_ptr()
    if pre is not None:
        _lib.require_cuda_tensor(pre, torch.float32, "conv_last pre")
        p.pre = pre.data_ptr()
    p.out = out.data_ptr()
    p.batch, p.cout, p.height, p.width, p.filters = b, weight.shape[0], h, w, weight.shape[1]
    p.clamp = 1 if clamp else 0
    p.wblob = wblob_ptr
    _lib.check(_lib.load().xmm_conv_last(ctypes.byref(p), _lib.stream_ptr()))
    _count()


def normalize(inp: torch.Tensor, max_val: float, stretch_mode: str, *, out: Optional[torch.Tensor] = None,
              mask: Optional[torch.Tensor] = None, pre_scale: float = 1.0) -> torch.Tensor:
    if stretch_mode not in _lib.STRETCH_MODES:
        raise ValueError(f"Stretching function {stretch_mode} is not implemented")
    if not inp.is_cuda or not inp.is_contiguous() or inp.dtype not in (torch.float32, torch.int32):
        raise RuntimeError("normalize: expected a contiguous CUDA fp32 or int32 tensor")
    if out is None:
        out = torch.empty(inp.shape, dtype=torch.float32, device=inp.device)
    _lib.require_cuda_tensor(out, torch.float32, "normalize output")
    p = NormalizeParams()
    p.in_, p.in_is_int32 = inp.data_ptr(), int(inp.dtype == torch.int32)
    if mask is not None:
        _lib.require_cuda_tensor(mask, torch.uint8, "normalize mask")
        p.mask, p.mask_n = mask.data_ptr(), mask.numel()
    p.out, p.n = out.data_ptr(), inp.numel()
    p.pre_scale, p.max_val, p.stretch_mode = pre_scale, float(max_val), _lib.STRETCH_MODES[stretch_mode]
    scratch = None
    if not max_val > 0:
        scratch = torch.zeros(1, dtype=torch.float32, device=inp.device)
        p.scratch = scratch.data_ptr()
    _lib.check(_lib.load().xmm_normalize(ctypes.byref(p), _lib.stream_ptr()))
    _count(1 if max_val > 0 else 2)
    return out


def denormalize(inp: torch.Tensor, max_vals: torch.Tensor, stretch_mode: str) -> torch.Tensor:
    if stretch_mode not in _lib.STRETCH_MODES:
        raise ValueError(f"Stretching function {stretch_mode} is not implemented")
    _lib.require_cuda_tensor(inp, torch.float32, "denormalize input")
    mv = max_vals.to(device=inp.device, dtype=torch.float32).reshape(-1).contiguous()
    out = torch.empty_like(inp)
    per_image = inp.numel() // inp.shape[0] if inp.dim() > 0 and inp.shape[0] > 0 else inp.numel()
    _lib.check(_lib.load().xmm_denormalize(inp.data_ptr(), out.data_ptr(), inp.numel(), per_image, mv.data_ptr(),
                                           mv.numel(), _lib.STRETCH_MODES[stretch_mode], _lib.stream_ptr()))
    _count()
    return out


def restretch(x: torch.Tensor, from_mode: str, to_mode: str) -> torch.Tensor:
    for m in (from_mode, to_mode):
        if m not in _lib.STRETCH_MODES:
            raise ValueError(f"Stretching function {m} is not implemented")
    _lib.require_cuda_tensor(x, torch.float32, "restretch input")
    out = torch.empty_like(x)
    _lib.check(_lib.load().xmm_restretch(x.data_ptr(), out.data_ptr(), x.numel(), _lib.STRETCH_MODES[from_mode],
                                         _lib.STRETCH_MODES[to_mode], _lib.stream_ptr()))
    _count()
    return out


def prepare_counts(planes, res, max_val: float, stretch_mode: str, *, det_mask: Optional[torch.Tensor] = None,
                   exposure=1.0, upsample: int = 1, out: Optional[torch.Tensor] = None) -> torch.Tensor:
    if stretch_mode not in _lib.STRETCH_MODES:
        raise ValueError(f"Stretching function {stretch_mode} is not implemented")
    planes = [p for p in planes if p is not None]
    if not 1 <= len(planes) <= 3:
        raise RuntimeError("prepare_counts: 1..3 source planes")
    first = planes[0]
    if first.dim() == 4:
        if first.shape[1] != 1:
            raise RuntimeError("prepare_counts: single-channel count images only")
        planes = [p.reshape(p.shape[0], p.shape[2], p.shape[3]) for p in planes]
        first = planes[0]
    b, h, w = first.shape
    for p in planes:
        if not p.is_cuda or not p.is_contiguous() or p.dtype != first.dtype or p.shape != first.shape:
            raise RuntimeError("prepare_counts: planes must be contiguous CUDA tensors of one dtype and shape")
    if first.dtype not in (torch.int32, torch.float32):
        raise RuntimeError("prepare_counts: planes must be int32 or fp32")
    res_h, res_w = (res, res) if isinstance(res, int) else res
    if out is None:
        out = torch.empty(b, 1, res_h, res_w, dtype=torch.float32, device=first.device)
    _lib.require_cuda_tensor(out, torch.float32, "prepare_counts output")
    p = _lib.PrepareCountsParams()
    for k, t in enumerate(planes):
        p.src[k] = t.data_ptr()
    p.nsrc, p.src_is_int32 = len(planes), int(first.dtype == torch.int32)
    if det_mask is not None:
        _lib.require_cuda_tensor(det_mask, torch.uint8, "prepare_counts det_mask")
        if det_mask.numel() != h * w:
            raise RuntimeError("prepare_counts: det_mask must have the shape of one source image")
        p.mask = det_mask.data_ptr()
    p.batch, p.h, p.w, p.up, p.res_h, p.res_w = b, h, w, int(upsample), res_h, res_w
    keep = None
    if isinstance(exposure, torch.Tensor):
        keep = (1.0 / exposure.to(device=first.device, dtype=torch.float32)).reshape(-1).contiguous()
        if keep.numel() != b:
            raise RuntimeError("prepare_counts: one exposure per image")
        p.pre_scale, p.pre_scale_dev = 1.0, keep.data_ptr()
    else:
        p.pre_scale = 1.0 / float(exposure)
    p.max_val, p.stretch_mode, p.out = float(max_val), _lib.STRETCH_MODES[stretch_mode], out.data_ptr()
    _lib.check(_lib.load().xmm_prepare_counts(ctypes.byref(p), _lib.stream_ptr()))
    _count()
    return out


def image_upsample(x: torch.Tensor, scale: int) -> torch.Tensor:
    _lib.require_cuda_tensor(x, torch.float32, "image_upsample input")
    h, w = x.shape[-2:]
    n_img = x.numel() // (h * w) if h * w else 0
    out = torch.empty(*x.shape[:-2], h * scale, w * scale, dtype=torch.float32, device=x.device)
    _lib.check(_lib.load().xmm_image_upsample(x.data_ptr(), out.data_ptr(), n_img, h, w, scale, _lib.stream_ptr()))
    _count()
    return out


def pack_weights(jobs_dev_ptr: int, njobs: int) -> None:
    _lib.check(_lib.load().xmm_pack_weights(jobs_dev_ptr, njobs, _lib.stream_ptr()))
    _count()


_WS = {}


def wgrad_workspace(device: torch.device) -> torch.Tensor:
    ws = _WS.get(str(device))
    if ws is None:
        ws = torch.empty(_lib.load().xmm_wgrad_workspace_bytes() // 4, dtype=torch.float32, device=device)
        _WS[str(device)] = ws
    return ws


def conv3x3_wgrad(x: torch.Tensor, dy: torch.Tensor, roles, dsts) -> None:
    _nhwc(x, "wgrad x")
    _nhwc(dy, "wgrad dy")
    if x.shape[:3] != dy.shape[:3]:
        raise RuntimeError("wgrad: x and dy must have the same batch / spatial shape")
    p = WgradParams()
    p.x, p.x_ctot, p.dy, p.dy_ctot = x.data_ptr(), x.shape[3], dy.data_ptr(), dy.shape[3]
    p.batch, p.height, p.width = x.shape[0], x.shape[1], x.shape[2]
    p.nroles = len(roles)
    for dst, r in zip(p.roles, roles):
        dst.tap_begin, dst.tap_count, dst.x_c0, dst.x_boxes, dst.y_c0, dst.n = r[:6]
        dst.mode = r[6] if len(r) > 6 else 0
    p.ndst = len(dsts)
    for dst, d in zip(p.dst, dsts):
        dw = d[0]
        _lib.require_cuda_tensor(dw, torch.float32, "wgrad dw")
        (dst.o_count, dst.i_total, dst.i_begin, dst.i_end, dst.role, dst.lane0, dst.col0, dst.scale, dst.accumulate,
         dst.perm) = d[1:11]
        dst.o_begin, dst.o_total = (d[11], d[12]) if len(d) > 11 else (0, 0)
        dst.dw = dw.data_ptr()
    p.workspace = wgrad_workspace(x.device).data_ptr()
    _lib.check(_lib.load().xmm_conv3x3_wgrad(ctypes.byref(p), _lib.stream_ptr()))
    _count(2)


def colsum(inp: torch.Tensor, c0: int, n: int, out: torch.Tensor, scale: float = 1.0, accumulate: bool = False) -> None:
    _nhwc(inp, "colsum input")
    _lib.require_cuda_tensor(out, torch.float32, "colsum output")
    npix = inp.shape[0] * inp.shape[1] * inp.shape[2]
    _lib.check(_lib.load().xmm_colsum_bf16(inp.data_ptr(), inp.shape[3], c0, n, npix, out.data_ptr(), scale,
                                           int(accumulate), _lib.stream_ptr()))
    _count()


def colsum_multi(inp: torch.Tensor, segments) -> None:
    _nhwc(inp, "colsum input")
    arr = (_lib.ColsumSegment * len(segments))()
    for a, (c0, n, out, scale, accumulate) in zip(arr, segments):
        _lib.require_cuda_tensor(out, torch.float32, "colsum output")
        a.c0, a.n, a.out, a.scale, a.accumulate = c0, n, out.data_ptr(), scale, int(accumulate)
    npix = inp.shape[0] * inp.shape[1] * inp.shape[2]
    _lib.check(_lib.load().xmm_colsum_multi_bf16(inp.data_ptr(), inp.shape[3], npix, arr, len(segments),
                                                 _lib.stream_ptr()))
    _count()


def edge_wgrad(s: torch.Tensor, v: torch.Tensor, v_coff: int, channels: int, r: torch.Tensor,
               ssum: Optional[torch.Tensor] = None, gate: Optional[torch.Tensor] = None,
               v2: Optional[torch.Tensor] = None, v2_coff: int = 0) -> None:
    _lib.require_cuda_tensor(s, torch.float32, "edge_wgrad s")
    _nhwc(v, "edge_wgrad v")
    _lib.require_cuda_tensor(r, torch.float32, "edge_wgrad r")
    p = EdgeWgradParams()
    p.s, p.gate = s.data_ptr(), _ptr(gate)
    p.v, p.v_ctot, p.v_coff = v.data_ptr(), v.shape[3], v_coff
    if v2 is not None:
        _nhwc(v2, "edge_wgrad v2")
        p.v2, p.v2_ctot, p.v2_coff = v2.data_ptr(), v2.shape[3], v2_coff
    p.r, p.ssum = r.data_ptr(), _ptr(ssum)
    p.batch, p.ns, p.height, p.width, p.channels = s.shape[0], s.shape[1], s.shape[2], s.shape[3], channels
    _lib.check(_lib.load().xmm_edge_wgrad(ctypes.byref(p), _lib.stream_ptr()))
    _count()
```

Before: 1387.

## Run second fused dense-block kernel as 2-CTA cluster with paired UMMA

Adds a PAIR variant of the fused RDB conv kernel for the two-layer (G=4) half. It launches as 2-CTA clusters, issues cta_group::2 UMMA with M=256, splits each weight group's bytes between the two CTAs, multicasts TMA completion to the leader's barriers, and deepens the load ring to 16 stages. Work is scheduled as pairs of tile columns, with phantom columns padding odd counts. The pair path is on by default via XMM_RDB_PAIR. The aim is to halve per-CTA weight shared-memory footprint and B-operand traffic, freeing room for more pipeline stages. The cost is cross-CTA barrier traffic, cluster scheduling limits on grid size, and possibly wasted phantom work.

```diff
diff --git a/include/xmm_b200.h b/include/xmm_b200.h
--- a/include/xmm_b200.h
+++ b/include/xmm_b200.h
@@ -71,6 +71,8 @@
 int xmm_conv3x3_bf16(const xmm_conv3x3_params* p, void* stream);
 
 #define XMM_CHAIN_SKIP_DEAD_STORES 0x100
+#define XMM_CHAIN_RDB_PAIR 0x200
+#define XMM_CHAIN_RDB_SINGLE 0x400
 size_t xmm_conv3x3_chain_workspace_bytes(int nlayers, int batch, int height);
 int xmm_conv3x3_chain_bf16(const xmm_conv3x3_params* layers, int nlayers, int mode_flags, void* workspace,
                            size_t workspace_bytes, void* stream);
diff --git a/xmm_superres_denoise_b200/csrc/conv3x3_rdb.cuh b/xmm_superres_denoise_b200/csrc/conv3x3_rdb.cuh
--- a/xmm_superres_denoise_b200/csrc/conv3x3_rdb.cuh
+++ b/xmm_superres_denoise_b200/csrc/conv3x3_rdb.cuh
@@ -13,8 +13,12 @@
 constexpr int kRdbSlots = 5;
 constexpr int kRdbSlotCols = kRdbSlots * 32;
 constexpr int kRdbMaxRing = 8;
-constexpr int kRdbMaxStages = 8;
+constexpr int kRdbMaxStages = 16;
+template <bool PAIR>
+constexpr int kRdbLRing = PAIR ? kRdbMaxStages : 8;
 constexpr int kRdbTapBytes = 32 * 64;
+constexpr int kRdbGroupBytes = 3 * kRdbTapBytes;
+constexpr int kRdbProfSlots = 24;
 
 struct RdbLayerArgs {
   const void* wblob;
@@ -61,36 +65,51 @@
   int ra, rb;
 };
 
-template <int NL>
+template <int NL, bool PAIR = false>
 struct RdbSched {
   int band_h, tiles_x, width, c0, npieces;
+  int ncols, rank;
   long long t0, t1;
   __device__ __forceinline__ void init(const RdbArgs& a) {
     band_h = a.band_h;
     tiles_x = a.tiles_x;
     width = a.width;
-    t0 = a.total_rows * blockIdx.x / gridDim.x;
-    t1 = a.total_rows * (blockIdx.x + 1) / gridDim.x;
+    if (PAIR) {
+      ncols = a.batch * a.tiles_x;
+      rank = int(ptx::cluster_ctarank());
+      const long long unit = blockIdx.x >> 1, nunits = gridDim.x >> 1;
+      t0 = a.total_rows * unit / nunits;
+      t1 = a.total_rows * (unit + 1) / nunits;
+    } else {
+      t0 = a.total_rows * blockIdx.x / gridDim.x;
+      t1 = a.total_rows * (blockIdx.x + 1) / gridDim.x;
+    }
     c0 = int(t0 / band_h);
     npieces = t1 > t0 ? int((t1 - 1) / band_h) - c0 + 1 : 0;
   }
   __device__ __forceinline__ RdbPiece get(int i) const {
     RdbPiece p;
-    const int col = c0 + i;
+    int col = c0 + i;
     const long long base = (long long)col * band_h;
     p.ra = t0 > base ? int(t0 - base) : 0;
     p.rb = t1 < base + band_h ? int(t1 - base) : band_h;
+    bool phantom = false;
+    if (PAIR) {
+      col = 2 * col + rank;
+      phantom = col >= ncols;
+      if (phantom) col = ncols - 1;
+    }
     p.b = col / tiles_x;
     const int t = col - p.b * tiles_x;
     p.own_lo = rdb_tile_origin<NL>(t);
     p.x0 = t == 0 ? 0 : p.own_lo - (NL - 1);
-    p.own_hi = t == tiles_x - 1 ? width : rdb_tile_origin<NL>(t + 1);
+    p.own_hi = phantom ? p.own_lo : t == tiles_x - 1 ? width : rdb_tile_origin<NL>(t + 1);
     return p;
   }
 };
 
-template <int NL, class F>
-__device__ __forceinline__ void rdb_walk(const RdbSched<NL>& s, F&& f) {
+template <int NL, class S, class F>
+__device__ __forceinline__ void rdb_walk(const S& s, F&& f) {
   int piece[NL], r[NL], hi[NL], n[NL], seq[NL][NL];
   RdbPiece pc[NL];
   bool done[NL];
@@ -223,11 +242,12 @@
   uint32_t tmem_base;
 };
 
-template <int G, int NL, int L>
-__device__ __forceinline__ void rdb_issuer(const RdbArgs& args, const RdbCtx& c, const RdbSched<NL>& sched) {
+template <int G, int NL, int L, bool PAIR>
+__device__ __forceinline__ void rdb_issuer(const RdbArgs& args, const RdbCtx& c, const RdbSched<NL, PAIR>& sched) {
   constexpr int NM = NL - 1;
   constexpr int e = NL - 1 - L;
   constexpr int ring[2] = {NL == 3 ? 5 : 2, 3};
+  constexpr uint32_t kR = kRdbLRing<PAIR>;
   rdb_wait(c.w_bar, 0, 7, L, 0);
   ptx::tc_fence_after();
   const uint64_t bdesc0 = ptx::umma_smem_desc(ptx::smem_u32(c.w_s), 16, 512, ptx::UMMA_SW64);
@@ -237,15 +257,26 @@
   const uint32_t b_l = uint32_t(bdesc0) + (args.layer[L].smem_off >> 4);
   const uint32_t a_map0[2] = {a_lo0 + uint32_t((c.map_s[0] - c.stage_s) >> 4), a_lo0 + uint32_t((c.map_s[1] - c.stage_s) >> 4)};
   constexpr uint32_t kTile16 = uint32_t(kRdbTileBytes) >> 4;
-  constexpr uint32_t kTap16 = uint32_t(kRdbTapBytes) >> 4;
-  constexpr uint32_t kIdesc = ptx::umma_idesc_bf16_f32(128, 96, 0, 0);
+  constexpr uint32_t kGroup16 = uint32_t(PAIR ? kRdbGroupBytes / 2 : kRdbGroupBytes) >> 4;
+  constexpr uint32_t kChunk16 = 3 * kGroup16;
+  constexpr uint32_t kIdesc = ptx::umma_idesc_bf16_f32(PAIR ? 256 : 128, 96, 0, 0);
   auto issue6 = [&](uint32_t d, uint32_t a, uint32_t b) {
 #pragma unroll
     for (int dx = 0; dx < 3; ++dx)
 #pragma unroll
-      for (int ks = 0; ks < 2; ++ks)
-        ptx::umma_ss_lh<true>(d, a + uint32_t((dx * 64 + ks * 32) >> 4), a_hi, b + uint32_t(dx * 3) * kTap16 + uint32_t((ks * 32) >> 4),
-                              b_hi, kIdesc);
+      for (int ks = 0; ks < 2; ++ks) {
+        const uint32_t a_lo = a + uint32_t((dx * 64 + ks * 32) >> 4), b_lo = b + uint32_t(dx) * kGroup16 + uint32_t((ks * 32) >> 4);
+        if constexpr (PAIR)
+          ptx::umma_ss_lh_pair<true>(d, a_lo, a_hi, b_lo, b_hi, kIdesc);
+        else
+          ptx::umma_ss_lh<true>(d, a_lo, a_hi, b_lo, b_hi, kIdesc);
+      }
+  };
+  auto commit = [](uint64_t* bar) {
+    if constexpr (PAIR)
+      ptx::umma_commit_pair(bar);
+    else
+      ptx::umma_commit(bar);
   };
   const bool prof = XMM_RDB_PROFILE && args.prof != nullptr && L == 0;
   long long pw[3] = {0, 0, 0};
@@ -264,13 +295,13 @@
         auto global_chunks = [&]() {
 #pragma unroll
           for (int g = 0; g < G; ++g) {
-            const int k = int(fills & 7u);
-            rdb_wait_p(&c.lfull[L * 8 + k], (fills >> 3) & 1u, 3, L, k, prof, pw[1]);
-            const int stage = c.lstage[L * 8 + k];
+            const int k = int(fills % kR);
+            rdb_wait_p(&c.lfull[L * kR + k], (fills / kR) & 1u, 3, L, k, prof, pw[1]);
+            const int stage = c.lstage[L * kR + k];
             ++fills;
             ptx::tc_fence_after();
-            issue6(d, a_lo0 + uint32_t(stage) * kTile16, b_l + uint32_t(g * 9) * kTap16);
-            ptx::umma_commit(&c.empty[stage]);
+            issue6(d, a_lo0 + uint32_t(stage) * kTile16, b_l + uint32_t(g) * kChunk16);
+            commit(&c.empty[stage]);
           }
         };
         auto map_chunks = [&]() {
@@ -281,8 +312,8 @@
               const int slot = sq % ring[m];
               rdb_wait_p(&c.mfull[m * 8 + slot], uint32_t(sq / ring[m]) & 1u, 4, L * 10 + m, sq, prof, pw[2]);
               ptx::tc_fence_after();
-              issue6(d, a_map0[m] + uint32_t(slot) * kTile16, b_l + uint32_t((G + m) * 9) * kTap16);
-              if (L == NL - 1 || r < pc.ra - e || r > pc.rb + e - 1) ptx::umma_commit(&c.mempty[m * 8 + slot]);
+              issue6(d, a_map0[m] + uint32_t(slot) * kTile16, b_l + uint32_t(G + m) * kChunk16);
+              if (L == NL - 1 || r < pc.ra - e || r > pc.rb + e - 1) commit(&c.mempty[m * 8 + slot]);
             }
         };
         if (NL == 2) {
@@ -293,13 +324,13 @@
           map_chunks();
         }
       }
-      ptx::umma_commit(&c.tfull[L]);
+      commit(&c.tfull[L]);
     }
 #pragma unroll
     for (int m = 0; m < NM; ++m) seq[m] += (pc.rb - pc.ra) + 2 * (NL - 1 - m);
   }
   if (XMM_RDB_PROFILE && prof) {
-    long long* o = args.prof + size_t(blockIdx.x) * 16;
+    long long* o = args.prof + size_t(blockIdx.x) * kRdbProfSlots;
     o[0] = clock64() - t_begin;
     o[1] = pw[0];
     o[2] = pw[1];
@@ -307,8 +338,16 @@
   }
 }
 
-template <int G, int NL, int L>
-__device__ __forceinline__ void rdb_epilogue(const RdbArgs& args, const RdbCtx& c, const RdbSched<NL>& sched, int q, int lane) {
+template <int G, int NL, int L, bool PAIR>
+__device__ __forceinline__ void rdb_epilogue(const RdbArgs& args, const RdbCtx& c, const RdbSched<NL, PAIR>& sched, int q,
+                                             int lane) {
+  const bool remote = PAIR && sched.rank != 0;
+  auto arrive = [&](uint64_t* bar) {
+    if (remote)
+      ptx::mbar_arrive_cluster(ptx::mapa(ptx::smem_u32(bar), 0));
+    else
+      ptx::mbar_arrive(bar);
+  };
   constexpr int e = NL - 1 - L;
   constexpr int ring[2] = {NL == 3 ? 5 : 2, 3};
   constexpr bool last = L == NL - 1;
@@ -390,7 +429,7 @@
       tmem_st_wait();
       ptx::tc_fence_before();
       __syncwarp();
-      if (lane == 0) ptx::mbar_arrive(&c.tdrain[L]);
+      if (lane == 0) arrive(&c.tdrain[L]);
       if (XMM_RDB_PROFILE) {
         const long long t = clock64();
         ph[0] += t - tph;
@@ -453,7 +492,7 @@
         for (int k = 0; k < 4; ++k) *reinterpret_cast<uint4*>(dst + ((uint32_t(k) ^ pos_xor) << 4)) = inimg ? o[k] : zero;
         ptx::fence_proxy_async();
         __syncwarp();
-        if (lane == 0) ptx::mbar_arrive(&c.mfull[L * 8 + slot]);
+        if (lane == 0) arrive(&c.mfull[L * 8 + slot]);
         if (XMM_RDB_PROFILE) {
           const long long t = clock64();
           ph[2] += t - tph;
@@ -469,18 +508,16 @@
     seq += (pc.rb - pc.ra) + 2 * e;
   }
   if (XMM_RDB_PROFILE && prof && q == 0 && lane == 0 && L < 2) {
-    long long* o = args.prof + size_t(blockIdx.x) * 16 + 4 + 4 * L;
+    long long* o = args.prof + size_t(blockIdx.x) * kRdbProfSlots + 4 + 4 * L;
     o[0] = clock64() - t_begin;
     o[1] = pw[0];
     o[2] = pw[1];
     o[3] = (long long)n;
-    if (L == 0) {
-      long long* o2 = args.prof + size_t(blockIdx.x) * 16 + 12;
-      o2[0] = ph[0];
-      o2[1] = ph[1];
-      o2[2] = ph[2];
-      o2[3] = ph[3];
-    }
+    long long* o2 = args.prof + size_t(blockIdx.x) * kRdbProfSlots + 12 + 4 * L;
+    o2[0] = ph[0];
+    o2[1] = ph[1];
+    o2[2] = ph[2];
+    o2[3] = ph[3];
   }
 }
 
@@ -539,12 +576,14 @@
   }
 }
 
-template <int G, int NL>
+template <int G, int NL, bool PAIR = false>
 __global__ void __launch_bounds__(kRdbThreads, 1)
 conv3x3_rdb_kernel(const __grid_constant__ CUtensorMap tmap_in, const RdbArgs args) {
   static_assert(NL == 2 || NL == 3, "two or three fused layers");
   static_assert(NL * kRdbSlotCols <= 512, "accumulators exceed TMEM");
   constexpr int NM = NL - 1;
+  constexpr int kR = kRdbLRing<PAIR>;
+  static_assert((3 * kR + kR + 3 + 3 + 16 + 16 + 1) * 8 + 3 * kR * 4 + 4 <= 1024, "barrier block exceeds 1024 B");
   extern __shared__ uint8_t smem_raw[];
   uint8_t* smem = reinterpret_cast<uint8_t*>((reinterpret_cast<uintptr_t>(smem_raw) + 1023) & ~uintptr_t(1023));
   RdbCtx c;
@@ -555,36 +594,45 @@
   uint8_t* after = c.map_s[1] + size_t(NM > 1 ? args.ring1 : 0) * kRdbTileBytes;
   uint64_t* bars = reinterpret_cast<uint64_t*>(after);
   c.lfull = bars;
-  c.empty = c.lfull + 24;
-  c.tfull = c.empty + 8;
+  c.empty = c.lfull + 3 * kR;
+  c.tfull = c.empty + kR;
   c.tdrain = c.tfull + 3;
   c.mfull = c.tdrain + 3;
   c.mempty = c.mfull + 16;
   c.w_bar = c.mempty + 16;
   c.lstage = reinterpret_cast<volatile int*>(c.w_bar + 1);
-  uint32_t* tmem_ptr_s = reinterpret_cast<uint32_t*>(const_cast<int*>(c.lstage) + 24);
+  uint32_t* tmem_ptr_s = reinterpret_cast<uint32_t*>(const_cast<int*>(c.lstage) + 3 * kR);
 
   const int warp = threadIdx.x >> 5;
   const int lane = threadIdx.x & 31;
+  const uint32_t rank = PAIR ? ptx::cluster_ctarank() : 0u;
 
   if (warp == 0 && lane == 0) {
     ptx::prefetch_tmap(&tmap_in);
-    for (int s = 0; s < NL * 8; ++s) ptx::mbar_init(&c.lfull[s], 1);
+    for (int s = 0; s < NL * kR; ++s) ptx::mbar_init(&c.lfull[s], 1);
     for (int s = 0; s < args.stages; ++s) ptx::mbar_init(&c.empty[s], 1);
     for (int l = 0; l < NL; ++l) {
       ptx::mbar_init(&c.tfull[l], 1);
-      ptx::mbar_init(&c.tdrain[l], 4);
+      ptx::mbar_init(&c.tdrain[l], PAIR ? 8 : 4);
     }
     for (int s = 0; s < 16; ++s) {
-      ptx::mbar_init(&c.mfull[s], 4);
+      ptx::mbar_init(&c.mfull[s], PAIR ? 8 : 4);
       ptx::mbar_init(&c.mempty[s], 1);
     }
     ptx::mbar_init(c.w_bar, 1);
     ptx::fence_mbar_init();
   }
-  if (warp == 1) ptx::tmem_alloc<512>(tmem_ptr_s);
+  if (warp == 1) {
+    if constexpr (PAIR)
+      ptx::tmem_alloc_pair<512>(tmem_ptr_s);
+    else
+      ptx::tmem_alloc<512>(tmem_ptr_s);
+  }
   ptx::tc_fence_before();
-  __syncthreads();
+  if constexpr (PAIR)
+    ptx::cluster_sync();
+  else
+    __syncthreads();
   ptx::tc_fence_after();
   c.tmem_base = *tmem_ptr_s;
 
@@ -594,9 +642,18 @@
     ptx::mbar_expect_tx(c.w_bar, wtot);
     for (int l = 0; l < NL; ++l) {
       const uint8_t* gsrc = static_cast<const uint8_t*>(args.layer[l].wblob);
-      const uint32_t n_l = args.layer[l].w_bytes + 128u;
-      for (uint32_t off = 0; off < n_l; off += 32768u)
-        ptx::bulk_load(c.w_s + args.layer[l].smem_off + off, gsrc + off, n_l - off < 32768u ? n_l - off : 32768u, c.w_bar);
+      uint8_t* dst = c.w_s + args.layer[l].smem_off;
+      const uint32_t wb = args.layer[l].w_bytes;
+      if constexpr (PAIR) {
+        constexpr uint32_t kHalf = kRdbGroupBytes / 2;
+        for (uint32_t grp = 0; grp < wb / kHalf; ++grp)
+          ptx::bulk_load(dst + grp * kHalf, gsrc + grp * kRdbGroupBytes + rank * kHalf, kHalf, c.w_bar);
+        ptx::bulk_load(dst + wb, gsrc + 2 * wb, 128u, c.w_bar);
+      } else {
+        const uint32_t n_l = wb + 128u;
+        for (uint32_t off = 0; off < n_l; off += 32768u)
+          ptx::bulk_load(dst + off, gsrc + off, n_l - off < 32768u ? n_l - off : 32768u, c.w_bar);
+      }
     }
   }
   const int egroup = (warp - 4) >> 2;
@@ -618,17 +675,22 @@
     }
   }
   ptx::tc_fence_before();
-  __syncthreads();
+  if constexpr (PAIR)
+    ptx::cluster_sync();
+  else
+    __syncthreads();
   ptx::tc_fence_after();
 
-  RdbSched<NL> sched;
+  RdbSched<NL, PAIR> sched;
   sched.init(args);
 
-  if (NL == 2 && args.split_producers && (warp == 0 || warp == 3)) {
-    if (ptx::elect_one()) {
-      const int ns0 = (args.stages + 1) / 2;
-      if (warp == 0) rdb_layer_producer<G, NL, 0>(&tmap_in, args, c, sched, 0, ns0);
-      if (warp == 3) rdb_layer_producer<G, NL, 1>(&tmap_in, args, c, sched, ns0, args.stages - ns0);
+  if (!PAIR && NL == 2 && args.split_producers && (warp == 0 || warp == 3)) {
+    if constexpr (!PAIR) {
+      if (ptx::elect_one()) {
+        const int ns0 = (args.stages + 1) / 2;
+        if (warp == 0) rdb_layer_producer<G, NL, 0>(&tmap_in, args, c, sched, 0, ns0);
+        if (warp == 3) rdb_layer_producer<G, NL, 1>(&tmap_in, args, c, sched, ns0, args.stages - ns0);
+      }
     }
   } else if (warp == 0) {
     if (ptx::elect_one()) {
@@ -650,12 +712,18 @@
 #pragma unroll
         for (int g = 0; g < G; ++g) {
           rdb_wait_backoff(&c.empty[stage], phase ^ 1u, 1, l, stage, uint32_t(args.backoff_ns));
-          const int k = int(fills[l]++ & 7u);
-          c.lstage[l * 8 + k] = stage;
-          uint64_t* fb = &c.lfull[l * 8 + k];
-          ptx::mbar_expect_tx(fb, kRdbTileData);
-          ptx::tma_load_5d(c.stage_s + size_t(stage) * kRdbTileBytes, &tmap_in, fb, args.cin_off + 32 * g, pc.x0 - 1, row, band0,
-                           pc.b);
+          const int k = int(fills[l]++ % uint32_t(kR));
+          c.lstage[l * kR + k] = stage;
+          uint64_t* fb = &c.lfull[l * kR + k];
+          if constexpr (PAIR) {
+            if (rank == 0) ptx::mbar_expect_tx(fb, 2 * kRdbTileData);
+            ptx::tma_load_5d_pair(c.stage_s + size_t(stage) * kRdbTileBytes, &tmap_in, ptx::mapa(ptx::smem_u32(fb), 0),
+                                  args.cin_off + 32 * g, pc.x0 - 1, row, band0, pc.b);
+          } else {
+            ptx::mbar_expect_tx(fb, kRdbTileData);
+            ptx::tma_load_5d(c.stage_s + size_t(stage) * kRdbTileBytes, &tmap_in, fb, args.cin_off + 32 * g, pc.x0 - 1, row,
+                             band0, pc.b);
+          }
           if (++stage == args.stages) {
             stage = 0;
             phase ^= 1u;
@@ -683,28 +751,34 @@
       });
     }
   } else if (warp <= 3) {
-    if (warp - 1 < NL && ptx::elect_one()) {
-      if (warp == 1) rdb_issuer<G, NL, 0>(args, c, sched);
-      if (warp == 2) rdb_issuer<G, NL, 1>(args, c, sched);
+    if (warp - 1 < NL && rank == 0 && ptx::elect_one()) {
+      if (warp == 1) rdb_issuer<G, NL, 0, PAIR>(args, c, sched);
+      if (warp == 2) rdb_issuer<G, NL, 1, PAIR>(args, c, sched);
       if constexpr (NL == 3) {
-        if (warp == 3) rdb_issuer<G, NL, 2>(args, c, sched);
+        if (warp == 3) rdb_issuer<G, NL, 2, PAIR>(args, c, sched);
       }
     }
   } else if (egroup < NL) {
     const int q = warp & 3;
-    if (egroup == 0) rdb_epilogue<G, NL, 0>(args, c, sched, q, lane);
-    if (egroup == 1) rdb_epilogue<G, NL, 1>(args, c, sched, q, lane);
+    if (egroup == 0) rdb_epilogue<G, NL, 0, PAIR>(args, c, sched, q, lane);
+    if (egroup == 1) rdb_epilogue<G, NL, 1, PAIR>(args, c, sched, q, lane);
     if constexpr (NL == 3) {
-      if (egroup == 2) rdb_epilogue<G, NL, 2>(args, c, sched, q, lane);
+      if (egroup == 2) rdb_epilogue<G, NL, 2, PAIR>(args, c, sched, q, lane);
     }
   }
 
   ptx::tc_fence_before();
-  __syncthreads();
+  if constexpr (PAIR)
+    ptx::cluster_sync();
+  else
+    __syncthreads();
   if (warp == 1) {
     ptx::tc_fence_after();
-    ptx::tmem_dealloc<512>(c.tmem_base);
-  }
-}
-
-}
+    if constexpr (PAIR)
+      ptx::tmem_dealloc_pair<512>(c.tmem_base);
+    else
+      ptx::tmem_dealloc<512>(c.tmem_base);
+  }
+}
+
+}
diff --git a/xmm_superres_denoise_b200/csrc/ptx_sm100.cuh b/xmm_superres_denoise_b200/csrc/ptx_sm100.cuh
--- a/xmm_superres_denoise_b200/csrc/ptx_sm100.cuh
+++ b/xmm_superres_denoise_b200/csrc/ptx_sm100.cuh
@@ -232,6 +232,30 @@
       "[%0], [%1, {%3, %4, %5, %6}], [%2];"
       ::"r"(smem_u32(smem_dst)),
       "l"(reinterpret_cast<uint64_t>(m)), "r"(bar_cluster_addr), "r"(c0), "r"(c1), "r"(c2), "r"(c3)
+      : "memory");
+}
+__device__ __forceinline__ void tma_load_5d_pair(void* smem_dst, const CUtensorMap* m, uint32_t bar_cluster_addr,
+                                                 int c0, int c1, int c2, int c3, int c4) {
+  asm volatile(
+      "cp.async.bulk.tensor.5d.cta_group::2.shared::cluster.global.tile.mbarrier::complete_tx::bytes "
+      "[%0], [%1, {%3, %4, %5, %6, %7}], [%2];"
+      ::"r"(smem_u32(smem_dst)),
+      "l"(reinterpret_cast<uint64_t>(m)), "r"(bar_cluster_addr), "r"(c0), "r"(c1), "r"(c2), "r"(c3), "r"(c4)
+      : "memory");
+}
+template <bool ACC>
+__device__ __forceinline__ void umma_ss_lh_pair(uint32_t tmem_d, uint32_t a_lo, uint32_t a_hi, uint32_t b_lo, uint32_t b_hi,
+                                                uint32_t idesc) {
+  asm volatile(
+      "{\n\t"
+      ".reg .pred p;\n\t"
+      ".reg .b64 da, db;\n\t"
+      "setp.ne.b32 p, %6, 0;\n\t"
+      "mov.b64 da, {%1, %2};\n\t"
+      "mov.b64 db, {%3, %4};\n\t"
+      "tcgen05.mma.cta_group::2.kind::f16 [%0], da, db, %5, p;\n\t"
+      "}\n" ::"r"(tmem_d),
+      "r"(a_lo), "r"(a_hi), "r"(b_lo), "r"(b_hi), "r"(idesc), "n"(ACC ? 1 : 0)
       : "memory");
 }
 template <int kCols>
diff --git a/xmm_superres_denoise_b200/csrc/xmm_b200.cu b/xmm_superres_denoise_b200/csrc/xmm_b200.cu
--- a/xmm_superres_denoise_b200/csrc/xmm_b200.cu
+++ b/xmm_superres_denoise_b200/csrc/xmm_b200.cu
@@ -707,14 +707,14 @@
   return nullptr;
 }
 
-template <int G, int NL>
+template <int G, int NL, bool PAIR>
 int launch_rdb(const xmm_conv3x3_params* L, const bool* store, const DeviceInfo& dev, cudaStream_t stream) {
   RdbArgs a{};
   uint32_t off = 0;
   for (int l = 0; l < NL; ++l) {
     const xmm_conv3x3_params& p = L[l];
     a.layer[l].wblob = p.wblob_row;
-    a.layer[l].w_bytes = uint32_t(p.cin / 32) * 9u * uint32_t(kRdbTapBytes);
+    a.layer[l].w_bytes = uint32_t(p.cin / 32) * 9u * uint32_t(kRdbTapBytes) / (PAIR ? 2u : 1u);
     a.layer[l].smem_off = off;
     off += (a.layer[l].w_bytes + 128u + 1023u) & ~1023u;
     a.layer[l].lrelu_slope = p.lrelu_slope;
@@ -731,7 +731,8 @@
   a.width = L[0].width;
   a.band_h = a.height / 2;
   a.tiles_x = rdb_tiles_x<NL>(a.width);
-  a.total_rows = (long long)a.batch * a.tiles_x * a.band_h;
+  const long long ncols = (long long)a.batch * a.tiles_x;
+  a.total_rows = (PAIR ? (ncols + 1) / 2 : ncols) * a.band_h;
   a.s0 = pl.s0; a.s1 = pl.s1; a.s2 = pl.s2;
   a.r1 = static_cast<const __nv_bfloat16*>(pl.r1); a.r1_ctot = pl.r1_ctot; a.r1_coff = pl.r1_coff;
   a.r2 = static_cast<const __nv_bfloat16*>(pl.r2); a.r2_ctot = pl.r2_ctot; a.r2_coff = pl.r2_coff;
@@ -745,55 +746,101 @@
   a.ring0 = NL == 3 ? 5 : 2;
   a.ring1 = NL == 3 ? 3 : 0;
   a.stages = tiles - a.ring0 - a.ring1;
-  if (a.stages > kRdbMaxStages) a.stages = kRdbMaxStages;
+  if (a.stages > kRdbLRing<PAIR>) a.stages = kRdbLRing<PAIR>;
   static const int stages_env = env_int("XMM_RDB_STAGES", 0);
   if (stages_env > 0 && stages_env < a.stages) a.stages = stages_env;
   if (a.stages < 3) return fail(XMM_ERR_UNSUPPORTED_SHAPE, "conv3x3 (fused dense block): %d pipeline stages fit", a.stages);
   static const int split_env = env_int("XMM_RDB_SPLIT_PRODUCERS", 0);
-  a.split_producers = (NL == 2 && split_env && a.stages >= 4) ? 1 : 0;
+  a.split_producers = (!PAIR && NL == 2 && split_env && a.stages >= 4) ? 1 : 0;
   CUtensorMap tmap;
   int rc = cached_band_tmap(&tmap, L[0].in, a.batch, a.height, a.width, L[0].in_ctot, a.band_h, 2, 32, kRdbBoxPx, 2);
   if (rc != XMM_OK) return rc;
-  rc = ensure_max_smem(reinterpret_cast<const void*>(conv3x3_rdb_kernel<G, NL>), dev);
+  const void* kernel = reinterpret_cast<const void*>(conv3x3_rdb_kernel<G, NL, PAIR>);
+  rc = ensure_max_smem(kernel, dev);
   if (rc != XMM_OK) return rc;
   const size_t smem = 1024 + size_t(a.w_total) + size_t(a.stages + a.ring0 + a.ring1) * kRdbTileBytes + kBarBytes;
   static const int max_ctas = env_int("XMM_RDB_MAX_CTAS", 0);
-  int grid = a.total_rows < dev.sm_count ? int(a.total_rows) : dev.sm_count;
-  if (max_ctas > 0 && grid > max_ctas) grid = max_ctas;
+  cudaLaunchConfig_t cfg{};
+  cudaLaunchAttribute attr[1];
+  cfg.blockDim = dim3(kRdbThreads);
+  cfg.dynamicSmemBytes = smem;
+  cfg.stream = stream;
+  long long grid;
+  if constexpr (PAIR) {
+    attr[0].id = cudaLaunchAttributeClusterDimension;
+    attr[0].val.clusterDim.x = 2;
+    attr[0].val.clusterDim.y = 1;
+    attr[0].val.clusterDim.z = 1;
+    cfg.attrs = attr;
+    cfg.numAttrs = 1;
+    static int max_clusters = 0;
+    if (max_clusters == 0) {
+      cfg.gridDim = dim3(unsigned(2 * dev.sm_count));
+      XMM_CUDA_OK(cudaOccupancyMaxActiveClusters(&max_clusters, conv3x3_rdb_kernel<G, NL, PAIR>, &cfg));
+      if (max_clusters < 1) return fail(XMM_ERR_UNSUPPORTED_SHAPE, "conv3x3 (fused dense block): no CTA pair fits an SM pair");
+    }
+    long long pairs = a.total_rows < max_clusters ? a.total_rows : max_clusters;
+    if (max_ctas > 0 && pairs > max_ctas / 2) pairs = max_ctas / 2 > 0 ? max_ctas / 2 : 1;
+    grid = 2 * pairs;
+  } else {
+    grid = a.total_rows < dev.sm_count ? a.total_rows : dev.sm_count;
+    if (max_ctas > 0 && grid > max_ctas) grid = max_ctas;
+  }
+  cfg.gridDim = dim3(unsigned(grid));
   static const int prof_env = XMM_RDB_PROFILE ? env_int("XMM_RDB_PROF", 0) : 0;
   static long long* prof_dev = nullptr;
+  constexpr size_t kProfBytes = kRdbProfSlots * sizeof(long long) * 1024;
   if (prof_env) {
-    if (prof_dev == nullptr) XMM_CUDA_OK(cudaMalloc(&prof_dev, 16 * sizeof(long long) * 1024));
-    XMM_CUDA_OK(cudaMemsetAsync(prof_dev, 0, 16 * sizeof(long long) * 1024, stream));
+    if (prof_dev == nullptr) XMM_CUDA_OK(cudaMalloc(&prof_dev, kProfBytes));
+    XMM_CUDA_OK(cudaMemsetAsync(prof_dev, 0, kProfBytes, stream));
     a.prof = prof_dev;
   }
-  conv3x3_rdb_kernel<G, NL><<<grid, kRdbThreads, smem, stream>>>(tmap, a);
-  XMM_CUDA_OK(cudaGetLastError());
+  if constexpr (PAIR) {
+    XMM_CUDA_OK(cudaLaunchKernelEx(&cfg, conv3x3_rdb_kernel<G, NL, PAIR>, tmap, a));
+  } else {
+    conv3x3_rdb_kernel<G, NL, PAIR><<<cfg.gridDim, kRdbThreads, smem, stream>>>(tmap, a);
+    XMM_CUDA_OK(cudaGetLastError());
+  }
   if (prof_env) {
     XMM_CUDA_OK(cudaStreamSynchronize(stream));
-    std::vector<long long> h(size_t(grid) * 16);
+    std::vector<long long> h(size_t(grid) * kRdbProfSlots);
     XMM_CUDA_OK(cudaMemcpy(h.data(), prof_dev, h.size() * sizeof(long long), cudaMemcpyDeviceToHost));
-    static const char* names[16] = {"issuer total", "issuer wait drained", "issuer wait TMA", "issuer wait map row",
-                                    "epi0 total", "epi0 wait row complete", "epi0 wait map slot", "epi0 rows",
-                                    "epi1 total", "epi1 wait row complete", "epi1 wait map slot", "epi1 rows",
-                                    "epi0 drain (ld+st+arrive)", "epi0 math+pack", "epi0 map write+fence+arrive", "epi0 global store"};
-    fprintf(stderr, "conv3x3_rdb<%d,%d> grid %d stages %d:", G, NL, grid, a.stages);
-    for (int k = 0; k < 16; ++k) {
+    static const char* names[kRdbProfSlots] = {
+        "issuer total", "issuer wait drained", "issuer wait TMA", "issuer wait map row",
+        "epi0 total", "epi0 wait row complete", "epi0 wait map slot", "epi0 rows",
+        "epi1 total", "epi1 wait row complete", "epi1 wait map slot", "epi1 rows",
+        "epi0 drain (ld+st+arrive)", "epi0 math+pack", "epi0 map write+fence+arrive", "epi0 global store",
+        "epi1 drain (ld+st+arrive)", "epi1 math+residuals+pack", "epi1 map write (none)", "epi1 global store",
+        "", "", "", ""};
+    fprintf(stderr, "conv3x3_rdb<%d,%d%s> grid %lld stages %d:", G, NL, PAIR ? ",pair" : "", grid, a.stages);
+    for (int k = 0; k < 20; ++k) {
       double sum = 0;
-      for (int c = 0; c < grid; ++c) sum += double(h[size_t(c) * 16 + k]);
-      fprintf(stderr, " %s %.0f;", names[k], sum / grid);
+      int n = 0;
+      for (long long c = 0; c < grid; ++c)
+        if (k >= 4 || !PAIR || c % 2 == 0) {
+          sum += double(h[size_t(c) * kRdbProfSlots + k]);
+          ++n;
+        }
+      fprintf(stderr, " %s %.0f;", names[k], sum / n);
     }
     fprintf(stderr, "\n");
   }
   return XMM_OK;
 }
 
-int launch_rdb_block(const xmm_conv3x3_params* L, bool skip_dead, const DeviceInfo& dev, cudaStream_t stream) {
+bool rdb_pair(int mode_flags) {
+  if (mode_flags & XMM_CHAIN_RDB_PAIR) return true;
+  if (mode_flags & XMM_CHAIN_RDB_SINGLE) return false;
+  static const int pair_env = env_int("XMM_RDB_PAIR", 1);
+  return pair_env != 0;
+}
+
+int launch_rdb_block(const xmm_conv3x3_params* L, bool skip_dead, bool pair, const DeviceInfo& dev, cudaStream_t stream) {
   const bool store_a[3] = {true, true, true};
-  int rc = launch_rdb<1, 3>(L, store_a, dev, stream);
+  int rc = launch_rdb<1, 3, false>(L, store_a, dev, stream);
   if (rc != XMM_OK) return rc;
   const bool store_b[2] = {!skip_dead, true};
-  return launch_rdb<4, 2>(L + 3, store_b, dev, stream);
+  return pair ? launch_rdb<4, 2, true>(L + 3, store_b, dev, stream) : launch_rdb<4, 2, false>(L + 3, store_b, dev, stream);
 }
 
 extern "C" int xmm_set_sm_reserve(int sms) {
@@ -812,8 +859,11 @@
   g_last_chain_launches = 0;
   const int mode = mode_flags & 0xff;
   const bool skip_dead = (mode_flags & XMM_CHAIN_SKIP_DEAD_STORES) != 0;
-  XMM_REQUIRE(mode >= 0 && mode <= 3 && (mode_flags & ~(0xff | XMM_CHAIN_SKIP_DEAD_STORES)) == 0,
-              "conv3x3_chain: mode must be 0 (auto), 1 (pipelined), 2 (layer by layer) or 3 (fused dense block)");
+  constexpr int kFlags = XMM_CHAIN_SKIP_DEAD_STORES | XMM_CHAIN_RDB_PAIR | XMM_CHAIN_RDB_SINGLE;
+  XMM_REQUIRE(mode >= 0 && mode <= 3 && (mode_flags & ~(0xff | kFlags)) == 0 &&
+                  (mode_flags & (XMM_CHAIN_RDB_PAIR | XMM_CHAIN_RDB_SINGLE)) != (XMM_CHAIN_RDB_PAIR | XMM_CHAIN_RDB_SINGLE),
+              "conv3x3_chain: mode must be 0 (auto), 1 (pipelined), 2 (layer by layer) or 3 (fused dense block), with at most "
+              "one of the pair / single flags");
   DeviceInfo dev;
   int rc = require_sm100(&dev);
   if (rc != XMM_OK) return rc;
@@ -827,7 +877,7 @@
     const char* why_not = rdb_blocker(layers, nlayers, dev);
     if (why_not == nullptr) {
       g_last_chain_launches = 2;
-      return launch_rdb_block(layers, skip_dead, dev, s);
+      return launch_rdb_block(layers, skip_dead, rdb_pair(mode_flags), dev, s);
     }
     if (mode == 3) return fail(XMM_ERR_UNSUPPORTED_SHAPE, "conv3x3_chain: cannot fuse the dense block (%s)", why_not);
   }
diff --git a/xmm_superres_denoise_b200/ops.py b/xmm_superres_denoise_b200/ops.py
--- a/xmm_superres_denoise_b200/ops.py
+++ b/xmm_superres_denoise_b200/ops.py
@@ -96,6 +96,7 @@
 
 CHAIN_AUTO, CHAIN_PIPELINED, CHAIN_LAYER_BY_LAYER, CHAIN_FUSED = 0, 1, 2, 3
 CHAIN_SKIP_DEAD_STORES = 0x100
+CHAIN_RDB_PAIR, CHAIN_RDB_SINGLE = 0x200, 0x400
 _chain_ws: dict = {}
 _chain_ws_retired: list = []
 
```

New measurement: 1435, median of 6. 1.03x the previous value.
